# Yubo-Shankui/Bind-Your-Avatar-Implementation

Measured on AMD Instinct MI355X. Metric: denoise-steps/sec, higher is better.
Workload: dtype bf16; 1 GPU; BASELINE.json configs[1]: full transformer.forward, 49x480x720 (13x30x45 latent tokens + 226 text), 2 characters (2 ID + 2 audio), batch 1, random-init 8.6B-param architecture; layers=42, batch=1, launch=eager, parallelism=single GPU

## Files before the change

### bind_your_avatar_implementation_amd/_hip.py

```python
import ctypes
import os

from .build import LIB_PATH as _BUILT_LIB

LIB_PATH = os.environ.get("BYA_HIP_LIB") or _BUILT_LIB

_c = ctypes
_vp, _i32, _i64, _f32 = _c.c_void_p, _c.c_int32, _c.c_int64, _c.c_float


class GemmDesc(_c.Structure):
    _fields_ = [("M", _i32), ("N", _i32), ("K", _i32), ("batch", _i32),
                ("lda", _i32), ("ldw", _i32), ("ldc", _i32), ("ldres", _i32),
                ("a_batch_stride", _i64), ("c_batch_stride", _i64), ("res_batch_stride", _i64),
                ("gate_batch_stride", _i64), ("gate_split", _i32), ("act", _i32),
                ("n_split", _i32), ("c_split_stride", _i64), ("bias_rowscale", _vp), ("alpha", _f32)]


class GemmPlan(_c.Structure):
    _fields_ = [("path", _i32), ("m0", _i32), ("tail", _i32), ("split_k", _i32), ("row_chunks", _i32)]


class QkNormDesc(_c.Structure):
    _fields_ = [("qw", _vp), ("qb", _vp), ("kw", _vp), ("kb", _vp), ("cos", _vp), ("sin", _vp),
                ("text_rows", _i32), ("width", _i32), ("eps", _f32), ("k_scale", _f32)]


class MxGemmCall(_c.Structure):
    _fields_ = [("A", _vp), ("a_scales", _vp), ("W", _vp), ("w_scales", _vp), ("bias", _vp), ("C", _vp),
                ("res", _vp), ("gate0", _vp), ("gate1", _vp), ("q_scales", _vp), ("norm", _c.POINTER(QkNormDesc)),
                ("a_fmt", _i32), ("w_fmt", _i32), ("out_fmt", _i32), ("kernel", _i32)]


class AttnDesc(_c.Structure):
    _fields_ = [("head_dim", _i32), ("heads", _i32), ("nb1", _i32), ("nb2", _i32), ("Sq", _i32), ("Skv", _i32),
                ("q_s1", _i64), ("q_s2", _i64), ("q_row", _i64),
                ("k_s1", _i64), ("k_s2", _i64), ("k_row", _i64),
                ("v_s1", _i64), ("v_s2", _i64), ("v_row", _i64),
                ("o_s1", _i64), ("o_s2", _i64), ("o_row", _i64),
                ("scale", _f32), ("scores_prescaled", _i32), ("score_bound", _f32),
                ("bound_dev", _vp), ("bound_slots", _i32), ("bound_heads", _i32), ("bound_bh0", _i32), ("fallback_flags", _vp)]


class AttnMixDesc(_c.Structure):
    _fields_ = [("head_dim", _i32), ("heads", _i32), ("n_id", _i32), ("n_grp", _i32), ("Sq", _i32), ("Skv", _i32),
                ("q_grp", _i64), ("q_row", _i64), ("k_id", _i64), ("k_grp", _i64), ("k_row", _i64),
                ("v_id", _i64), ("v_grp", _i64), ("v_row", _i64), ("z_grp", _i64), ("z_row", _i64), ("scale", _f32)]


class AttnPlan(_c.Structure):
    _fields_ = [("variant", _i32), ("grid", _i32), ("q_tile", _i32), ("stream_k", _i32), ("sk_rem", _i32), ("sk_cut", _i32),
                ("o_wide", _i32), ("second_launch", _i32)]


class AttnMixPlan(_c.Structure):
    _fields_ = [("form", _i32), ("head_dim", _i32), ("grid", _i32), ("row_chunks", _i32), ("lds_bytes", _i32), ("big_lds", _i32)]


class AttnTinyPlan(_c.Structure):
    _fields_ = [("instance", _i32), ("grid", _i32), ("waves", _i64)]


class RowGemmPlan(_c.Structure):
    _fields_ = [("form", _i32), ("ln", _i32), ("res", _i32), ("act", _i32), ("grid", _i32), ("crosses_row_block", _i32),
                ("work_items", _i64)]


class GroupAttnPlan(_c.Structure):
    _fields_ = [("P", _i32), ("G", _i32), ("wide", _i32), ("blocks", _i32), ("tiles", _i64)]


class LayerNormPlan(_c.Structure):
    _fields_ = [("kernel", _i32), ("vec", _i32), ("nv", _i32), ("modulated", _i32), ("rows_per_wave", _i32), ("grid", _i32),
                ("waves", _i64)]


class QkNormRopePlan(_c.Structure):
    _fields_ = [("stats", _i32), ("only", _i32), ("grid", _i32), ("slots", _i32), ("pairs", _i64), ("waves", _i64)]


class RouterChainPlan(_c.Structure):
    _fields_ = [("tiles", _i32), ("tp0", _i32), ("grid", _i32), ("passes", _i32), ("tiles_last", _i32), ("wgs_last", _i32)]


class SchedCoef(_c.Structure):
    _fields_ = [("guidance", _f32), ("sqrt_alpha", _f32), ("sqrt_beta", _f32), ("k_sample", _f32),
                ("k_denoised", _f32), ("k_noise", _f32), ("k_cur", _f32), ("k_old", _f32)]


SIGNATURES = {
    "bya_abi_version": [],
    "bya_set_option": [_i32, _i32],
    "bya_get_option": [_i32, _c.POINTER(_i32)],
    "bya_mfma_calibration": [_vp, _i64, _vp, _i32, _vp],
    "bya_gemm_bf16": [_vp, _vp, _vp, _vp, _vp, _vp, _vp, _c.POINTER(GemmDesc), _vp],
    "bya_gemm_skinny_bf16": [_vp, _vp, _vp, _vp, _vp, _c.POINTER(GemmDesc), _vp],
    "bya_gemm_qkv_norm_rope": [_vp, _vp, _vp, _vp, _c.POINTER(GemmDesc), _c.POINTER(QkNormDesc), _vp],
    "bya_gemm_bf16_plan": [_vp, _vp, _vp, _vp, _vp, _vp, _vp, _c.POINTER(GemmDesc), _c.POINTER(GemmPlan)],
    "bya_gemm_qkv_norm_rope_plan": [_vp, _vp, _vp, _vp, _c.POINTER(GemmDesc), _c.POINTER(QkNormDesc), _c.POINTER(GemmPlan)],
    "bya_set_gemm_workspace": [_vp, _i64],
    "bya_gemm_workspace_bytes": [_c.POINTER(_i64)],
    "bya_gemm_workspace_status": [_c.POINTER(_i32), _vp],
    "bya_quantize_rows_fp8": [_vp, _vp, _vp, _i32, _i32, _i64, _i64, _vp],
    "bya_gemm_fp8": [_vp, _vp, _vp, _vp, _vp, _vp, _vp, _vp, _vp, _c.POINTER(GemmDesc), _vp],
    "bya_gemm_fp8_plan": [_vp, _vp, _vp, _vp, _vp, _vp, _vp, _vp, _vp, _c.POINTER(GemmDesc), _c.POINTER(GemmPlan)],
    "bya_layernorm_fp8": [_vp, _vp, _vp, _vp, _vp, _vp, _vp, _vp, _vp, _i64, _i32, _i32, _i64, _i64, _i64, _i64, _i64, _i64,
                          _f32, _vp],
    "bya_quantize_mx": [_vp, _vp, _vp, _i32, _i32, _i64, _i32, _vp],
    "bya_layernorm_mx": [_vp, _vp, _vp, _vp, _vp, _vp, _vp, _vp, _vp, _i64, _i32, _i32, _i64, _i64, _i64, _i64, _i64, _i64,
                         _f32, _i32, _vp],
    "bya_gemm_mx": [_vp, _vp, _vp, _vp, _vp, _vp, _vp, _vp, _vp, _c.POINTER(GemmDesc), _i32, _vp],
    "bya_gemm_mx_plan": [_vp, _vp, _vp, _vp, _vp, _vp, _vp, _vp, _vp, _c.POINTER(GemmDesc), _i32, _c.POINTER(GemmPlan)],
    "bya_gemm_mx_mixed": [_vp, _vp, _vp, _vp, _vp, _vp, _vp, _vp, _vp, _c.POINTER(GemmDesc), _i32, _i32, _vp],
    "bya_gemm_mx_mixed_plan": [_vp, _vp, _vp, _vp, _vp, _vp, _vp, _vp, _vp, _c.POINTER(GemmDesc), _i32, _i32,
                               _c.POINTER(GemmPlan)],
    "bya_gemm_mx_quant": [_vp, _vp, _vp, _vp, _vp, _vp, _vp, _c.POINTER(GemmDesc), _i32, _i32, _i32, _vp],
    "bya_gemm_mx_quant_plan": [_vp, _vp, _vp, _vp, _vp, _vp, _vp, _c.POINTER(GemmDesc), _i32, _i32, _i32,
                               _c.POINTER(GemmPlan)],
    "bya_gemm_mx_qkv_norm_rope": [_vp, _vp, _vp, _vp, _vp, _vp, _i32, _i32, _c.POINTER(GemmDesc), _c.POINTER(QkNormDesc), _vp],
    "bya_gemm_mx_qkv_norm_rope_plan": [_vp, _vp, _vp, _vp, _vp, _vp, _i32, _i32, _c.POINTER(GemmDesc), _c.POINTER(QkNormDesc),
                                       _c.POINTER(GemmPlan)],
    "bya_gemm_mx_qkv_norm_rope_on": [_vp, _vp, _vp, _vp, _vp, _vp, _i32, _i32, _c.POINTER(GemmDesc), _c.POINTER(QkNormDesc), _i32,
                                     _vp],
    "bya_gemm_mx_qkv_norm_rope_on_plan": [_vp, _vp, _vp, _vp, _vp, _vp, _i32, _i32, _c.POINTER(GemmDesc), _c.POINTER(QkNormDesc),
                                          _i32, _c.POINTER(GemmPlan)],
    "bya_gemm_mx_call": [_c.POINTER(MxGemmCall), _c.POINTER(GemmDesc), _vp],
    "bya_gemm_mx_call_plan": [_c.POINTER(MxGemmCall), _c.POINTER(GemmDesc), _c.POINTER(GemmPlan)],
    "bya_linear_small_m": [_vp, _vp, _vp, _vp, _i32, _i32, _i32, _i32, _i32, _vp],
    "bya_timestep_features": [_vp, _vp, _i32, _i32, _i32, _f32, _vp],
    "bya_layernorm": [_vp, _vp, _vp, _vp, _vp, _vp, _vp, _vp, _i64, _i32, _i32, _i64, _i64, _i64, _i64, _i64, _i64,
                      _f32, _vp],
    "bya_layernorm_plan": [_vp, _vp, _vp, _vp, _vp, _vp, _vp, _vp, _i64, _i32, _i32, _i64, _i64, _i64, _i64, _i64, _i64,
                           _i32, _c.POINTER(LayerNormPlan)],
    "bya_qknorm_rope_plan": [_vp, _vp, _vp, _vp, _vp, _vp, _vp, _vp, _i32, _i32, _i32, _i64, _i64, _i32, _vp, _i32,
                             _c.POINTER(QkNormRopePlan)],
    "bya_qknorm_rope": [_vp, _vp, _vp, _vp, _vp, _vp, _vp, _vp, _i32, _i32, _i32, _i64, _i64, _i32, _f32, _f32, _vp, _i32, _vp],
    "bya_attn_fwd": [_vp, _vp, _vp, _vp, _c.POINTER(AttnDesc), _vp],
    "bya_attn_variant": [_c.POINTER(AttnDesc)],
    "bya_attn_plan": [_c.POINTER(AttnDesc), _vp, _i32, _c.POINTER(AttnPlan)],
    "bya_attn_fwd_mx": [_vp, _vp, _vp, _vp, _vp, _c.POINTER(AttnDesc), _i32, _i64, _i64, _i64, _i64, _i64, _i64, _vp],
    "bya_attn_mx_plan": [_c.POINTER(AttnDesc), _vp, _vp, _i32, _i64, _i64, _i64, _i64, _i64, _i64, _i32, _c.POINTER(AttnPlan)],
    "bya_set_attn_workspace": [_vp, _i64],
    "bya_attn_workspace_bytes": [_c.POINTER(_i64)],
    "bya_attn_workspace_status": [_c.POINTER(_i32), _vp],
    "bya_attn_kv_mix": [_vp, _vp, _vp, _vp, _vp, _vp, _vp, _c.POINTER(AttnMixDesc), _vp],
    "bya_attn_kv_mix_plan": [_vp, _vp, _c.POINTER(AttnMixDesc), _c.POINTER(AttnMixPlan)],
    "bya_attn_tiny": [_vp, _vp, _vp, _vp, _i32, _i32, _i64, _i64, _i64, _i64, _i64, _i64, _f32, _vp],
    "bya_attn_tiny_plan": [_vp, _vp, _vp, _vp, _i32, _i32, _i64, _i64, _i64, _i64, _c.POINTER(AttnTinyPlan)],
    "bya_router_scores": [_vp, _vp, _vp, _vp, _vp, _vp, _i32, _i64, _i32, _i32, _f32, _vp],
    "bya_router_head": [_vp, _vp, _vp, _vp, _i32, _i64, _i32, _vp],
    "bya_forcing_max_over_frames": [_vp, _vp, _i32, _i64, _i32, _vp],
    "bya_masked_combine": [_vp, _vp, _vp, _vp, _i32, _f32, _i32, _i32, _i64, _i32, _i64, _i64, _i64, _vp],
    "bya_routed_mix": [_vp, _vp, _vp, _vp, _vp, _i32, _i32, _i32, _i64, _i32, _i64, _vp],
    "bya_patchify": [_vp, _vp, _i32, _i32, _i32, _i32, _i32, _vp],
    "bya_unpatchify": [_vp, _vp, _i32, _i32, _i32, _i32, _i32, _vp],
    "bya_act_add": [_vp, _vp, _vp, _i64, _i32, _vp],
    "bya_rowgemm512": [_vp, _vp, _vp, _vp, _vp, _vp, _i32, _i32, _i32, _i32, _i32, _i32, _f32, _i32, _i32, _vp],
    "bya_rowgemm512_plan": [_vp, _vp, _vp, _vp, _vp, _vp, _i32, _i32, _i32, _i32, _i32, _i32, _i32, _c.POINTER(RowGemmPlan)],
    "bya_router_group_attn_plan": [_vp, _vp, _vp, _vp, _vp, _i32, _i32, _i32, _i32, _i64, _i64, _i64, _i64,
                                   _c.POINTER(GroupAttnPlan)],
    "bya_router_mlp_fused_plan": [_vp, _vp, _vp, _vp, _vp, _vp, _vp, _i32, _i32, _i32, _i32, _c.POINTER(RouterChainPlan)],
    "bya_router_group_attn_out_plan": [_vp, _vp, _vp, _vp, _vp, _vp, _vp, _i32, _i32, _i32, _i32, _i64, _i64, _i64, _i64, _i32,
                                       _c.POINTER(RouterChainPlan)],
    "bya_router_group_attn": [_vp, _vp, _vp, _vp, _vp, _i32, _i32, _i32, _i32, _i64, _i64, _i64, _i64, _f32, _f32, _vp],
    "bya_router_mlp_fused": [_vp, _vp, _vp, _vp, _vp, _vp, _vp, _i32, _i32, _i32, _f32, _i32, _vp],
    "bya_router_group_attn_out": [_vp, _vp, _vp, _vp, _vp, _vp, _vp, _i32, _i32, _i32, _i32, _i64, _i64, _i64, _i64, _f32, _f32,
                                  _i32, _vp],
    "bya_masks_to_routing_logits": [_vp, _vp, _i32, _i32, _i32, _i32, _i32, _i32, _i32, _vp],
    "bya_vae_patches": [_vp, _vp, _vp] + [_i32] * 14 + [_vp],
    "bya_vae_groupnorm_stats": [_vp, _vp, _vp, _i64, _i32, _i32, _vp],
    "bya_vae_norm_act": [_vp, _vp, _vp, _vp, _vp, _vp, _vp, _i64, _i32, _i32, _i32, _f32, _i32, _i32, _i32, _i32, _i32, _i32,
                         _i32, _i64, _i32, _vp],
    "bya_vae_conv3d": [_vp, _vp, _vp, _vp, _vp, _i32, _i32, _i32, _i32, _i32, _i32, _i64, _i64, _i64, _vp],
    "bya_vae_upsample_pad": [_vp, _vp, _i32, _i32, _i32, _i32, _i32, _vp],
    "bya_allgather_kv": [_vp, _vp, _vp, _vp, _i64, _i64, _vp, _vp],
    "bya_alltoall_router": [_vp, _vp, _vp, _vp, _i32, _vp, _vp],
    "bya_p2p_push": [_vp, _i32, _i64, _vp, _i32, _i32, _vp, _vp],
    "bya_p2p_wait": [_vp, _i32, _vp, _i64, _vp],
    "bya_p2p_exchange": [_vp, _i32, _i64, _vp, _i32, _i32, _vp, _vp, _i64, _vp],
    "bya_p2p_poison": [_vp, _i32, _vp, _i64, _vp],
    "bya_p2p_alloc": [_i64, _i32, _c.POINTER(_vp)],
    "bya_p2p_free": [_vp],
    "bya_p2p_ipc_export": [_vp, _vp],
    "bya_p2p_ipc_import": [_vp, _c.POINTER(_vp)],
    "bya_p2p_ipc_release": [_vp],
    "bya_cfg_scheduler_step": [_vp, _i32, _i64, _vp, _vp, _vp, _vp, _vp, _i64, _c.POINTER(SchedCoef), _vp],
}

OPTIONS = {"gemm_splitk": 0, "gemm_splitk_min": 1, "gemm_tile": 2, "gemm_variant": 3, "attn_streamk": 4, "fp8_kernel": 5,
           "p2p_groups": 6, "reference_forms": 7, "mx_kernel": 8}
REFERENCE_FORMS = {"rowgemm_chunked": 1, "kv_mix_generic": 2, "ln_generic": 4, "router_scores_wave": 8, "attn_narrow_store": 16}
def _named_value(var, v, table):
    if v not in table:
        raise ValueError(f"{var}={v!r}: expected one of {sorted(table)}")
    return table[v]


ENV_OPTIONS = {
    "BYA_GEMM_SPLITK": ("gemm_splitk", int),
    "BYA_GEMM_SPLITK_MIN": ("gemm_splitk_min", int),
    "BYA_GEMM_TILE": ("gemm_tile", int),
    "BYA_GEMM_VARIANT": ("gemm_variant", lambda v: {"w8": 1, "no128": 2}.get(v, 0)),
    "BYA_ATTN_STREAMK": ("attn_streamk", int),
    "BYA_FP8_KERNEL": ("fp8_kernel", lambda v: 1 if v.startswith("1") else 0),
    "BYA_P2P_GROUPS": ("p2p_groups", int),
    "BYA_MX_KERNEL": ("mx_kernel", lambda v: _named_value("BYA_MX_KERNEL", v, {"0": 0, "1": 1, "p256": 1, "2": 2, "always": 2})),
}

GEMM_PATHS = {0: "t128x64", 1: "t128x128", 2: "t256x128", 3: "t256x256", 4: "p256", 5: "p128", 6: "p128s", 7: "w8_256"}

ATTN_VARIANTS = {0: "d64_running_max", 1: "d64_prescaled_running_max", 2: "d64_static_bound", 3: "d128_running_max",
                 4: "d64_static_bound_w4", 5: "d64_device_bound_w4"}
KV_MIX_FORMS = {0: "mix32", 1: "one_tile"}
TINY_INSTANCES = {0: "tiny8<2>", 1: "tiny8<3>", 2: "tiny8<13>", 3: "tiny8<25>", 4: "generic<2>", 5: "generic<4>",
                  6: "generic<16>", 7: "generic<32>"}

ROWGEMM_FORMS = {0: "chunk_balanced", 1: "w_stationary"}

LN_KERNELS = {0: "generic", 1: "rows"}
LN_OUT_KINDS = {"bf16": 0, "fp8": 1, "mxfp8": 2, "mxfp6": 3}

ERRORS = {-1: "BYA_ERR_SHAPE", -2: "BYA_ERR_ALIGN", -3: "BYA_ERR_LAUNCH", -4: "BYA_ERR_UNSUPPORTED"}

_lib = None


def load():
    global _lib
    if _lib is not None:
        return _lib
    import torch
    if not os.path.exists(LIB_PATH):
        raise RuntimeError(
            f"{LIB_PATH} is missing: the Bind-Your-Avatar MI355X engine has no fallback path. "
            "Build it with `python -m bind_your_avatar_implementation_amd.build`.")
    lib = ctypes.CDLL(LIB_PATH)
    for name, argtypes in SIGNATURES.items():
        fn = getattr(lib, name)
        fn.argtypes = argtypes
        fn.restype = _i32
    _lib = lib
    apply_env_options()
    return lib


def set_option(name, value):
    check(load().bya_set_option(OPTIONS[name], int(value)), f"bya_set_option({name}={value})")


def get_option(name):
    v = _i32(0)
    check(load().bya_get_option(OPTIONS[name], _c.byref(v)), f"bya_get_option({name})")
    return v.value


OPTION_DEFAULTS = {"gemm_splitk": 0, "gemm_splitk_min": 0, "gemm_tile": -1, "gemm_variant": 0, "attn_streamk": 1, "fp8_kernel": 0,
                   "p2p_groups": 0, "reference_forms": 0, "mx_kernel": 0}


def apply_env_options():
    for var, (name, parse) in ENV_OPTIONS.items():
        v = os.environ.get(var)
        set_option(name, parse(v) if v not in (None, "") else OPTION_DEFAULTS[name])


class ByaError(RuntimeError):
    pass


def check(rc, what):
    if rc != 0:
        raise ByaError(f"{what} failed: {ERRORS.get(rc, rc)}")
```

### bind_your_avatar_implementation_amd/csrc/gemm.hip

```cpp
#include "gemm_common.h"
#include <stdlib.h>
#include <string.h>
#include "options.h"

namespace {


template <int ROWS, int NWAVES>
__device__ __forceinline__ void stage_tile(const bf16_t* __restrict__ src, int ld, int row0, int row_max, int k0,
                                           char* lds_tile, int wave, int lane) {
    constexpr int PER_WAVE = ROWS / NWAVES;
#pragma unroll
    for (int q = 0; q < PER_WAVE / 8; ++q) {
        const int rbase = wave * PER_WAVE + q * 8;
        const int rl = rbase + (lane >> 3);
        const int chunk = (lane & 7) ^ ((rl >> 1) & 7);
        int gr = row0 + rl;
        gr = gr < row_max ? gr : row_max;
        const bf16_t* g = src + (long long)gr * ld + k0 + chunk * 8;
        __builtin_amdgcn_global_load_lds(GLOBAL_PTR(g), LDS_PTR(lds_tile + rbase * 128), 16, 0, 0);
    }
}

__device__ __forceinline__ bf16x8 lds_frag(const char* tile, int row, int chunk) {
// ... 79 lines not shown
    ds_read128<(HALF * 64 + 48) * 128>(f.v[3], addr);
}
template <int HALF>
__device__ __forceinline__ void load_frag_b(FragB& f, uint32_t addr) {
    ds_read128<(HALF * 32 + 0) * 128>(f.v[0], addr);
    ds_read128<(HALF * 32 + 16) * 128>(f.v[1], addr);
}
template <int N>
__device__ __forceinline__ void wait_frags(FragA& a, FragB& b) {
    asm volatile("s_waitcnt lgkmcnt(%6)"
                 : "+v"(a.v[0]), "+v"(a.v[1]), "+v"(a.v[2]), "+v"(a.v[3]), "+v"(b.v[0]), "+v"(b.v[1])
                 : "i"(N));
}

template <int HA, int HB>
__device__ __forceinline__ void mfma_quadrant(f32x4 (&acc)[4][8], const FragA& a, const FragB& b) {
    __builtin_amdgcn_s_setprio(1);
#pragma unroll
    for (int ni = 0; ni < 2; ++ni)
#pragma unroll
        for (int mi = 0; mi < 4; ++mi)
            acc[HB * 2 + ni][HA * 4 + mi] =
                __builtin_amdgcn_mfma_f32_16x16x32_bf16(b.v[ni], a.v[mi], acc[HB * 2 + ni][HA * 4 + mi], 0, 0, 0);
    __builtin_amdgcn_s_setprio(0);
}

__global__ __launch_bounds__(512, 2) void gemm256_kernel(GemmArgs p) {
    extern __shared__ __attribute__((aligned(16))) char smem[];
    constexpr int BM = 256, BN = 256, STAGE = (BM + BN) * BK * 2, TILE_A = BM * BK * 2;
    const int tid = threadIdx.x, lane = tid & 63;
    const int wave = __builtin_amdgcn_readfirstlane(tid >> 6);
    const int tiles_m = (p.M + BM - 1) / BM, tiles_n = (p.N + BN - 1) / BN;
    const int nwg = tiles_m * tiles_n;
    const int id = xcd_remap(blockIdx.x, nwg);
    constexpr int GM = 4;
    const int per_group = GM * tiles_n;
    const int group = id / per_group, first_m = group * GM;
    const int gsz = (tiles_m - first_m) < GM ? (tiles_m - first_m) : GM;
    const int in_g = id - group * per_group;
    const int tm = first_m + in_g % gsz, tn = in_g / gsz;
    const int m0 = tm * BM, n0 = tn * BN;
    const int z = blockIdx.z;
    const bf16_t* A = p.A + (long long)z * p.a_bs;
    const int nk = p.K / BK;
    const int wm = wave >> 2, wn = wave & 3;
    const int fr = lane & 15, fq = lane >> 4;

    const int a_row = wm * 128 + fr, w_row = wn * 64 + fr;
    const int a_sw = (a_row >> 1) & 7, w_sw = (w_row >> 1) & 7;
    const int a_off0 = ((fq ^ a_sw) << 4), a_off1 = (((4 + fq) ^ a_sw) << 4);
    const int w_off0 = ((fq ^ w_sw) << 4), w_off1 = (((4 + fq) ^ w_sw) << 4);
    const int a_lane = a_row * 128, w_lane = w_row * 128;

    const __amdgpu_buffer_rsrc_t rsA = __builtin_amdgcn_make_buffer_rsrc(
        (void*)A, 0, (int)(((long long)(p.M - 1) * p.lda + p.K) * 2), 0x00020000);
    const __amdgpu_buffer_rsrc_t rsW = __builtin_amdgcn_make_buffer_rsrc(
        (void*)p.W, 0, (int)(((long long)(p.N - 1) * p.ldw + p.K) * 2), 0x00020000);
    uint32_t voff[8];
#pragma unroll
    for (int q = 0; q < 8; ++q) {
        const int rl = wave * 32 + (q & 3) * 8 + (lane >> 3);
        const int chunk = (lane & 7) ^ ((rl >> 1) & 7);
        voff[q] = (q < 4) ? (uint32_t)(m0 + rl) * (uint32_t)(p.lda * 2) + chunk * 16
                          : (uint32_t)(n0 + rl) * (uint32_t)(p.ldw * 2) + chunk * 16;
    }
    auto piece = [&](int t, int q) {
        char* dst = smem + (t & 1) * STAGE + (q >= 4 ? TILE_A : 0) + (wave * 32 + (q & 3) * 8) * 128;
        __builtin_amdgcn_raw_ptr_buffer_load_lds(q >= 4 ? rsW : rsA, LDS_PTR(dst), 16, voff[q], t * (BK * 2), 0, 0);
    };

    f32x4 acc[4][8];
#pragma unroll
    for (int i = 0; i < 4; ++i)
#pragma unroll
        for (int j = 0; j < 8; ++j) acc[i][j] = f32x4{0.f, 0.f, 0.f, 0.f};

    piece(0, 0); piece(0, 1); piece(0, 2); piece(0, 3); piece(0, 4); piece(0, 5); piece(0, 6); piece(0, 7);
    if (nk > 1) { piece(1, 0); piece(1, 1); }
    asm volatile("s_waitcnt vmcnt(0)" ::: "memory");
    __builtin_amdgcn_s_barrier();

    const uint32_t lds0 = (uint32_t)(uintptr_t)LDS_PTR(smem);
    uint32_t cA0 = lds0 + a_lane + a_off0, cA1 = lds0 + a_lane + a_off1;
    uint32_t cW0 = lds0 + TILE_A + w_lane + w_off0, cW1 = lds0 + TILE_A + w_lane + w_off1;
    static_assert(STAGE == 65536, "stage flip uses one address bit");
    FragA a0, a1;
    FragB bx, by;
    load_frag_a<0>(a0, cA0);
    load_frag_b<0>(bx, cW0);

    for (int t = 0; t < nk; ++t) {
        const bool more = t + 1 < nk;
        load_frag_b<1>(by, cW0);
        if (more) { piece(t + 1, 2); piece(t + 1, 3); }
        __builtin_amdgcn_sched_barrier(0);
        wait_frags<2>(a0, bx);
        mfma_quadrant<0, 0>(acc, a0, bx);
        __builtin_amdgcn_sched_barrier(0);
        load_frag_a<1>(a1, cA0);
        if (more) { piece(t + 1, 4); piece(t + 1, 5); }
        __builtin_amdgcn_sched_barrier(0);
        wait_frags<4>(a0, by);
        mfma_quadrant<0, 1>(acc, a0, by);
        __builtin_amdgcn_sched_barrier(0);
        load_frag_a<0>(a0, cA1);
        if (more) { piece(t + 1, 6); piece(t + 1, 7); }
        __builtin_amdgcn_sched_barrier(0);
        wait_frags<4>(a1, by);
        mfma_quadrant<1, 1>(acc, a1, by);
        __builtin_amdgcn_sched_barrier(0);
        load_frag_b<0>(by, cW1);
        __builtin_amdgcn_sched_barrier(0);
        mfma_quadrant<1, 0>(acc, a1, bx);
        __builtin_amdgcn_sched_barrier(0);
        load_frag_b<1>(bx, cW1);
        __builtin_amdgcn_sched_barrier(0);
        wait_frags<2>(a0, by);
        mfma_quadrant<0, 0>(acc, a0, by);
        __builtin_amdgcn_sched_barrier(0);
        load_frag_a<1>(a1, cA1);
        __builtin_amdgcn_sched_barrier(0);
        wait_frags<4>(a0, bx);
        mfma_quadrant<0, 1>(acc, a0, bx);
        __builtin_amdgcn_sched_barrier(0);
        wait_frags<0>(a1, bx);
        mfma_quadrant<1, 1>(acc, a1, bx);
        __builtin_amdgcn_sched_barrier(0);
        asm volatile("s_waitcnt vmcnt(0)" ::: "memory");
        __builtin_amdgcn_s_barrier();
        cA0 ^= STAGE; cA1 ^= STAGE; cW0 ^= STAGE; cW1 ^= STAGE;
        if (more) {
            load_frag_a<0>(a0, cA0);
            load_frag_b<0>(bx, cW0);
            if (t + 2 < nk) { piece(t + 2, 0); piece(t + 2, 1); }
        }
        __builtin_amdgcn_sched_barrier(0);
        mfma_quadrant<1, 0>(acc, a1, by);
        __builtin_amdgcn_sched_barrier(0);
    }
    asm volatile("s_waitcnt lgkmcnt(0)" ::: "memory");

    auto run = [&](auto act_tag) {
        epilogue_block<decltype(act_tag)::value, 4, 8, 2>(p, z, m0 + wm * 128 + fr, n0 + wn * 64 + fq * 4, acc);
    };
    dispatch_act_big(p.act, run);
}

inline bool v4_eligible(const GemmArgs& a) {
    return a.K >= 3 * BK && a.N % 8 == 0 && a.n_split % 8 == 0 && a.ldc % 8 == 0 && (!a.res || a.ldres % 8 == 0) &&
        !(((uintptr_t)a.C | (uintptr_t)a.res | (uintptr_t)a.bias | (uintptr_t)a.gate0 | (uintptr_t)a.gate1) & 15) &&
        a.c_bs % 8 == 0 && a.res_bs % 8 == 0 && a.gate_bs % 8 == 0 && a.c_split_stride % 8 == 0;
}

inline bool p128_eligible(const GemmArgs& a) { return v4_eligible(a) && a.K >= 4 * BK && a.conv_cpg_log2 < 0 && bya_opt(BYA_OPT_GEMM_VARIANT) == 0; }

inline int path256(const GemmArgs& a) {
    return v4_eligible(a) && bya_opt(BYA_OPT_GEMM_VARIANT) != 1 ? BYA_GEMM_PATH_P256 : BYA_GEMM_PATH_W8_256;
}

int launch_w8_256(const GemmArgs& a, int batch, hipStream_t s) {
    const int tiles_m = (a.M + 255) / 256, tiles_n = (a.N + 255) / 256;
    dim3 grid(tiles_m * tiles_n, 1, batch);
    const size_t lds = 2 * 512 * BK * 2;
    static std::atomic<unsigned long long> attr_done{0};
    if (bya_allow_big_lds(reinterpret_cast<const void*>(gemm256_kernel), (int)lds, attr_done) != BYA_OK) return BYA_ERR_LAUNCH;
    BYA_LAUNCH(gemm256_kernel, grid, dim3(512), lds, s, a);
    return hipGetLastError() == hipSuccess ? BYA_OK : BYA_ERR_LAUNCH;
}

template <int BM, int BN, int WAVES_M, int WAVES_N>
int launch(const GemmArgs& a, int batch, hipStream_t s) {
    const int tiles_m = (a.M + BM - 1) / BM, tiles_n = (a.N + BN - 1) / BN;
    dim3 grid(tiles_m * tiles_n, 1, batch);
    const size_t lds = 2 * (BM + BN) * BK * 2;
    static std::atomic<unsigned long long> attr_done{0};
    if (bya_allow_big_lds(reinterpret_cast<const void*>(gemm_bf16_kernel<BM, BN, WAVES_M, WAVES_N>), (int)lds, attr_done) != BYA_OK)
        return BYA_ERR_LAUNCH;
    BYA_LAUNCH((gemm_bf16_kernel<BM, BN, WAVES_M, WAVES_N>), grid, dim3(64 * WAVES_M * WAVES_N), lds, s, a);
    return hipGetLastError() == hipSuccess ? BYA_OK : BYA_ERR_LAUNCH;
}

constexpr double REL_128S = 0.85, REL_128P = 0.80;
inline double rounds_128(int M, int N, int batch, double rel) {
    const long long t = (long long)((M + 127) / 128) * ((N + 255) / 256) * batch;
    return 0.5 * (double)((t + 255) / 256) / rel;
}
inline double rounds_256_split(int M, int N, int K, int batch) {
    const long long tiles = (long long)((M + 255) / 256) * ((N + 255) / 256) * batch, full = tiles / 256, rem = tiles % 256;
    if (rem == 0) return (double)full;
    const int R = (int)((rem + 7) / 8);
    int parts = 32 / R;
    const int by_k = (K / BK) / bya_gemm_split_min_ktiles();
    if (parts > by_k) parts = by_k;
    return (double)full + (parts > 1 ? 1.0 / parts + 0.3 : 1.0);
}
inline int hybrid_rows(int M, int N, int batch, double rel, double* cost) {
    const long long tn = (N + 255) / 256, tiles = (long long)((M + 255) / 256) * tn, full = tiles / 256;
    if (batch != 1 || full < 1 || tiles % 256 == 0) return 0;
    const int main_tm = (int)(full * 256 / tn), m0 = main_tm * 256;
    if (m0 <= 0 || m0 >= M) return 0;
    *cost = (double)(((long long)main_tm * tn + 255) / 256) + rounds_128(M - m0, N, 1, rel) + 0.05;
    return m0;
}
inline int plan_rows_qkn(int M, int N, int batch, int* m0) {
    const int forced = bya_opt(BYA_OPT_GEMM_TILE);
    if (forced >= 0) return forced == 5 || forced == 6 ? 1 : 0;
    const long long t256 = (long long)((M + 255) / 256) * ((N + 255) / 256) * batch;
    const double r256 = (double)((t256 + 255) / 256), r128 = rounds_128(M, N, batch, REL_128P);
    double best = r256, hc = 0.0;
    int plan = 0;
    if (r128 < 0.97 * best) { best = r128; plan = 1; }
    const int hm = hybrid_rows(M, N, batch, REL_128P, &hc);
    if (hm > 0 && hc < (plan == 0 ? r256 - 0.15 : 0.97 * best)) { *m0 = hm; plan = 2; }
    return plan;
}

inline int pick_tile(int M, int N, int K, int batch, int forced, int act, bool splitk, bool p128_ok) {
    if (forced >= 0) return (forced >= 4 && !act_on_big_tiles(act)) ? 1 : forced;
    if (N <= 64) return 0;
    auto rounds = [&](int bm, int bn, int per_cu) {
        const long long blocks = (long long)((M + bm - 1) / bm) * ((N + bn - 1) / bn) * batch;
        const long long slots = 256LL * per_cu;
        return (double)((blocks + slots - 1) / slots) * (bm * bn) * (double)per_cu;
    };
    const double t128 = rounds(128, 128, 2) / 0.80;
    const double t256x128 = rounds(256, 128, 1) / 0.95;
    const double frac_rounds = (double)((M + 255) / 256) * ((N + 255) / 256) * batch / 256.0;
    const double t256 = splitk ? (frac_rounds + 0.12) * 65536.0 : rounds(256, 256, 1) / 1.00;
    (void)t256x128;
#ifdef BYA_GEMM_NO_DEEP_GRID
    const bool deep_grid = false;
#else
    const bool deep_grid = frac_rounds >= 4.0 && M >= 512 && K >= 512;
#endif
    if (((M < 1024 || K < 1024) && !deep_grid) || N < 512 || !act_on_big_tiles(act)) return 1;
    if (p128_ok) {
        const double t256s = (splitk ? rounds_256_split(M, N, K, batch) * 65536.0 : t256) / 1.2;
        const double best = t256s <= t128 ? t256s : t128, r128 = rounds_128(M, N, batch, REL_128S);
        if (r128 * 65536.0 / 1.2 < 0.97 * best) {
            double hc = 0.0;
            if (!splitk && hybrid_rows(M, N, batch, REL_128S, &hc) > 0 && hc < 0.97 * r128 && t256 / 1.2 <= t128) return 4;
            return 6;
        }
    }
    return (t256 / 1.2 <= t128) ? 4 : 1;
}

}

namespace {
constexpr int MAX_DEVICES = 64;
std::atomic<void*> g_gemm_ws[MAX_DEVICES];
inline int current_device() {
    int dev = 0;
    return hipGetDevice(&dev) == hipSuccess && dev >= 0 && dev < MAX_DEVICES ? dev : -1;
}
}

extern "C" int bya_set_gemm_workspace(void* ws, int64_t bytes) {
    if (ws && (bytes < (int64_t)GEMM_WS_BYTES || ((uintptr_t)ws & 255))) return BYA_ERR_SHAPE;
    const int dev = current_device();
    if (dev < 0) return BYA_ERR_UNSUPPORTED;
    g_gemm_ws[dev].store(ws);
    return BYA_OK;
}

extern "C" int bya_gemm_workspace_status(int32_t* timeouts, hipStream_t stream) {
    if (!timeouts) return BYA_ERR_SHAPE;
    *timeouts = 0;
    const int dev = current_device();
    char* const ws = dev < 0 ? nullptr : static_cast<char*>(g_gemm_ws[dev].load());
    if (!ws) return BYA_OK;
    unsigned word = 0;
    if (hipMemcpyAsync(&word, ws + 1023 * 4, 4, hipMemcpyDeviceToHost, stream) != hipSuccess) return BYA_ERR_LAUNCH;
    if (hipStreamSynchronize(stream) != hipSuccess) return BYA_ERR_LAUNCH;
    *timeouts = (int32_t)word;
    return BYA_OK;
}

extern "C" int bya_gemm_workspace_bytes(int64_t* bytes) {
    if (!bytes) return BYA_ERR_SHAPE;
    *bytes = (int64_t)GEMM_WS_BYTES;
    return BYA_OK;
}

namespace {
int dispatch_gemm(const GemmArgs& a, int nbatch, hipStream_t stream);
void plan_gemm(const GemmArgs& a, int nbatch, bya_gemm_plan* p);

int bf16_args(const void* A, const void* W, const void* bias, const void* C, const void* res, const void* gate0,
              const void* gate1, const bya_gemm_desc* d, GemmArgs* out) {
    if (!A || !W || !C || !d) return BYA_ERR_SHAPE;
    if (d->M <= 0 || d->N <= 0 || d->K <= 0 || d->batch <= 0) return BYA_ERR_SHAPE;
    if (d->K % BK != 0 || d->N % 4 != 0) return BYA_ERR_SHAPE;
    if (d->lda % 8 || d->ldw % 8 || d->ldc % 4 || (res && d->ldres % 4)) return BYA_ERR_ALIGN;
    if (((uintptr_t)A | (uintptr_t)W) & 15) return BYA_ERR_ALIGN;
    if (((uintptr_t)C | (uintptr_t)res | (uintptr_t)bias | (uintptr_t)gate0 | (uintptr_t)gate1) & 7) return BYA_ERR_ALIGN;
    if (d->act < 0 || d->act > 6) return BYA_ERR_UNSUPPORTED;
    GemmArgs& a = *out;
    a.A = (const bf16_t*)A; a.W = (const bf16_t*)W; a.bias = (const bf16_t*)bias; a.C = (bf16_t*)C;
    a.res = (const bf16_t*)res; a.gate0 = (const bf16_t*)gate0; a.gate1 = (const bf16_t*)(gate1 ? gate1 : gate0);
    a.M = d->M; a.N = d->N; a.K = d->K;
    a.lda = d->lda; a.ldw = d->ldw; a.ldc = d->ldc; a.ldres = d->ldres;
    a.a_bs = d->a_batch_stride; a.c_bs = d->c_batch_stride; a.res_bs = d->res_batch_stride;
    a.gate_bs = d->gate_batch_stride; a.gate_split = d->gate_split; a.act = d->act; a.leaky = 0.01f;
    a.n_split = d->n_split; a.c_split_stride = d->c_split_stride;
    a.bias_rowscale = d->bias_rowscale; a.alpha = d->alpha == 0.0f ? 1.0f : d->alpha;
    const int dev = current_device();
    char* const ws = dev < 0 ? nullptr : static_cast<char*>(g_gemm_ws[dev].load());
    a.ws_counters = reinterpret_cast<unsigned*>(ws);
    a.ws_slabs = ws ? reinterpret_cast<float*>(ws + GEMM_WS_COUNTER_BYTES) : nullptr;
    if (d->n_split < 0 || (d->n_split > 0 && (d->n_split % 4 || d->c_split_stride % 4 || res))) return BYA_ERR_SHAPE;
    return BYA_OK;
}

int qkn_args(const void* A, const void* W, const void* bias, const void* C, const bya_gemm_desc* d, const bya_qknorm_desc* n,
             GemmArgs* out) {
    if (!A || !W || !C || !d || !n) return BYA_ERR_SHAPE;
    if (d->M <= 0 || d->N <= 0 || d->K <= 0 || d->batch <= 0 || d->K % BK != 0) return BYA_ERR_SHAPE;
    if (!n->qw || !n->qb || !n->kw || !n->kb || n->width <= 0 || n->text_rows < 0) return BYA_ERR_SHAPE;
    if (n->text_rows < d->M && (!n->cos || !n->sin)) return BYA_ERR_SHAPE;
    if ((d->N != 3 * n->width && d->N != 2 * n->width) || n->width % 128 != 0 || d->n_split <= 0 || d->act != 0 || d->bias_rowscale || (d->alpha != 0.0f && d->alpha != 1.0f))
        return BYA_ERR_UNSUPPORTED;
    if (d->lda % 8 || d->ldw % 8) return BYA_ERR_ALIGN;
    if (((uintptr_t)A | (uintptr_t)W | (uintptr_t)C | (uintptr_t)bias | (uintptr_t)n->qw | (uintptr_t)n->qb | (uintptr_t)n->kw |
         (uintptr_t)n->kb | (uintptr_t)n->cos | (uintptr_t)n->sin) & 15) return BYA_ERR_ALIGN;
    GemmArgs& a = *out;
    a.A = (const bf16_t*)A; a.W = (const bf16_t*)W; a.bias = (const bf16_t*)bias; a.C = (bf16_t*)C;
    a.res = nullptr; a.gate0 = nullptr; a.gate1 = nullptr;
    a.M = d->M; a.N = d->N; a.K = d->K;
    a.lda = d->lda; a.ldw = d->ldw; a.ldc = d->ldc; a.ldres = 0;
    a.a_bs = d->a_batch_stride; a.c_bs = d->c_batch_stride; a.res_bs = 0; a.gate_bs = 0; a.gate_split = 0; a.act = 0; a.leaky = 0.01f;
    a.n_split = d->n_split; a.c_split_stride = d->c_split_stride;
    a.bias_rowscale = nullptr; a.alpha = 1.0f;
    a.ws_counters = nullptr; a.ws_slabs = nullptr;
    a.qkn_w[0] = (const bf16_t*)n->qw; a.qkn_b[0] = (const bf16_t*)n->qb; a.qkn_w[1] = (const bf16_t*)n->kw; a.qkn_b[1] = (const bf16_t*)n->kb;
    a.qkn_cos = n->cos; a.qkn_sin = n->sin; a.qkn_text_rows = n->text_rows; a.qkn_width = n->width;
    a.qkn_eps = n->eps; a.qkn_kscale = n->k_scale == 0.0f ? 1.0f : n->k_scale;
    if (!v4_eligible(a) || !gemm_rows_reachable(a, a.M)) return BYA_ERR_UNSUPPORTED;
    return BYA_OK;
}

inline int qkn_plan(const GemmArgs& a, int batch, int* m0) {
    *m0 = 0;
    return p128_eligible(a) ? plan_rows_qkn(a.M, a.N, batch, m0) : 0;
}
}

extern "C" int bya_gemm_bf16(const void* A, const void* W, const void* bias, void* C, const void* res,
                             const void* gate0, const void* gate1, const bya_gemm_desc* d, hipStream_t stream) {
    GemmArgs a;
    const int rc = bf16_args(A, W, bias, C, res, gate0, gate1, d, &a);
    if (rc != BYA_OK) return rc;
    return gemm_row_chunks(a, d->batch, 2, [&](const GemmArgs& piece, int batch, long long) {
        return dispatch_gemm(piece, batch, stream);
    });
}

extern "C" int bya_gemm_bf16_plan(const void* A, const void* W, const void* bias, const void* C, const void* res,
                                  const void* gate0, const void* gate1, const bya_gemm_desc* d, bya_gemm_plan* plan) {
    if (!plan) return BYA_ERR_SHAPE;
    GemmArgs a, piece;
    int rc = bf16_args(A, W, bias, C, res, gate0, gate1, d, &a), nb = 0;
    if (rc != BYA_OK) return rc;
    const int chunks = gemm_first_chunk(a, d->batch, &piece, &nb);
    if (!chunks) return BYA_ERR_UNSUPPORTED;
    plan_gemm(piece, nb, plan);
    plan->row_chunks = chunks;
    return BYA_OK;
}

extern "C" int bya_gemm_qkv_norm_rope(const void* A, const void* W, const void* bias, void* C, const bya_gemm_desc* d,
                                      const bya_qknorm_desc* n, hipStream_t stream) {
    GemmArgs a;
    const int rc0 = qkn_args(A, W, bias, C, d, n, &a);
    if (rc0 != BYA_OK) return rc0;
    int m0 = 0;
    const int plan = qkn_plan(a, d->batch, &m0);
    if (plan == 1) return bya_launch_gemm128p_qkn(&a, d->batch, stream);
    if (plan == 2) {
        GemmArgs lo = a, hi = a;
        lo.M = m0;
        hi.M = a.M - m0;
        hi.A += (long long)m0 * a.lda;
        hi.C += (long long)m0 * a.ldc;
        hi.qkn_text_rows = a.qkn_text_rows > m0 ? a.qkn_text_rows - m0 : 0;
        if (a.qkn_cos && m0 > a.qkn_text_rows) {
            hi.qkn_cos = a.qkn_cos + (long long)(m0 - a.qkn_text_rows) * 64;
            hi.qkn_sin = a.qkn_sin + (long long)(m0 - a.qkn_text_rows) * 64;
        }
        const int rc = bya_launch_gemm256p_qkn(&lo, 1, stream);
        return rc != BYA_OK ? rc : bya_launch_gemm128p_qkn(&hi, 1, stream);
    }
    return bya_launch_gemm256p_qkn(&a, d->batch, stream);
}

extern "C" int bya_gemm_qkv_norm_rope_plan(const void* A, const void* W, const void* bias, const void* C, const bya_gemm_desc* d,
                                           const bya_qknorm_desc* n, bya_gemm_plan* p) {
    if (!p) return BYA_ERR_SHAPE;
    GemmArgs a;
    const int rc = qkn_args(A, W, bias, C, d, n, &a);
    if (rc != BYA_OK) return rc;
    int m0 = 0;
    const int plan = qkn_plan(a, d->batch, &m0);
    p->path = plan == 1 ? BYA_GEMM_PATH_P128 : BYA_GEMM_PATH_P256;
    p->m0 = plan == 2 ? m0 : 0;
    p->tail = plan == 2 ? BYA_GEMM_PATH_P128 : -1;
    p->split_k = 0;
    p->row_chunks = 1;
    return BYA_OK;
}

namespace {
template <int MT>
__global__ __launch_bounds__(1024) void gemm_skinny_kernel(GemmArgs p) {
    extern __shared__ __attribute__((aligned(16))) char smem[];
    float* red = reinterpret_cast<float*>(smem);
    const int tid = threadIdx.x, lane = tid & 63, c = lane & 15, g = lane >> 4;
    const int wave = __builtin_amdgcn_readfirstlane(tid >> 6);
    const int n0 = blockIdx.x * 16, zb = blockIdx.y, fold = p.gate_split, rows = fold > 0 ? fold * p.M : p.M;
    const int ksteps = p.K / 32;
    const int k_lo = (int)((long long)ksteps * wave / 16), k_hi = (int)((long long)ksteps * (wave + 1) / 16);
    const bf16_t* wrow = p.W + (long long)(n0 + c) * p.ldw + 8 * g;
    const bf16_t* xrow[MT];
#pragma unroll
    for (int mt = 0; mt < MT; ++mt) {
        int r = mt * 16 + c;
        r = r < rows ? r : rows - 1;
        const int z = fold > 0 ? r / p.M : zb, m = fold > 0 ? r % p.M : r;
        xrow[mt] = p.A + (long long)z * p.a_bs + (long long)m * p.lda + 8 * g;
    }
    f32x4 acc[MT];
#pragma unroll
    for (int mt = 0; mt < MT; ++mt) acc[mt] = f32x4{0.f, 0.f, 0.f, 0.f};
    int ks = k_lo;
    for (; ks + 4 <= k_hi; ks += 4) {
        bf16x8 wf[4];
#pragma unroll
        for (int u = 0; u < 4; ++u) wf[u] = *reinterpret_cast<const bf16x8*>(wrow + (ks + u) * 32);
#pragma unroll
        for (int u = 0; u < 4; ++u)
#pragma unroll
            for (int mt = 0; mt < MT; ++mt) {
                const bf16x8 xf = *reinterpret_cast<const bf16x8*>(xrow[mt] + (ks + u) * 32);
                acc[mt] = __builtin_amdgcn_mfma_f32_16x16x32_bf16(wf[u], xf, acc[mt], 0, 0, 0);
            }
    }
    for (; ks < k_hi; ++ks) {
        const bf16x8 wf = *reinterpret_cast<const bf16x8*>(wrow + ks * 32);
#pragma unroll
        for (int mt = 0; mt < MT; ++mt) {
            const bf16x8 xf = *reinterpret_cast<const bf16x8*>(xrow[mt] + ks * 32);
            acc[mt] = __builtin_amdgcn_mfma_f32_16x16x32_bf16(wf, xf, acc[mt], 0, 0, 0);
        }
    }
#pragma unroll
    for (int mt = 0; mt < MT; ++mt)
        *reinterpret_cast<f32x4*>(red + ((wave * MT * 16 + mt * 16 + c) * 16 + 4 * g)) = acc[mt];
    __syncthreads();
    for (int t = tid; t < MT * 256; t += 1024) {
        const int r = t >> 4, n = t & 15;
        float v = 0.f;
#pragma unroll
        for (int w = 0; w < 16; ++w) v += red[(w * MT * 16 + r) * 16 + n];
        if (r < rows) {
            const int z = fold > 0 ? r / p.M : zb, m = fold > 0 ? r % p.M : r;
            if (p.bias) v += bf2f(p.bias[n0 + n]);
            switch (p.act) {
                case 1: v = gelu_tanh(v); break;
                case 2: v = gelu_erf(v); break;
                case 3: v = v > 0.f ? v : 0.f; break;
                case 4: v = silu(v); break;
                case 5: v = v > 0.f ? v : v * p.leaky; break;
                case 6: v = gelu_tanh_ieee(v); break;
                default: break;
            }
            v *= p.alpha;
            if (p.res) v += bf2f(p.res[(long long)z * p.res_bs + (long long)m * p.ldres + n0 + n]);
            p.C[(long long)z * p.c_bs + (long long)m * p.ldc + n0 + n] = f2bf(v);
        }
    }
}

inline bool skinny_eligible(const GemmArgs& a) {
    return a.M <= 64 && a.N <= 8192 && a.K >= 256 && a.K % 32 == 0 && a.N % 16 == 0 && a.lda % 8 == 0 && a.ldw % 8 == 0 && a.a_bs % 8 == 0 &&
        !a.gate0 && !a.bias_rowscale && a.n_split == 0 && a.conv_cpg_log2 < 0 && !(((uintptr_t)a.A | (uintptr_t)a.W) & 15);
}

template <int MT>
int launch_skinny_mt(const GemmArgs& a, dim3 grid, hipStream_t stream) {
    const size_t lds = (size_t)16 * MT * 16 * 16 * 4;
    static std::atomic<unsigned long long> big{0};
    if (lds > 64 * 1024 && bya_allow_big_lds(reinterpret_cast<const void*>(gemm_skinny_kernel<MT>), 160 * 1024, big) != BYA_OK)
        return BYA_ERR_LAUNCH;
    BYA_LAUNCH(gemm_skinny_kernel<MT>, grid, dim3(1024), lds, stream, a);
    return hipGetLastError() == hipSuccess ? BYA_OK : BYA_ERR_LAUNCH;
}

int launch_skinny(const GemmArgs& a0, int nbatch, hipStream_t stream) {
    GemmArgs a = a0;
    const bool fold = nbatch > 1 && (long long)nbatch * a.M <= 64;
    a.gate_split = fold ? nbatch : 0;
    const int rows = fold ? nbatch * a.M : a.M, mt = (rows + 15) / 16;
    const dim3 grid((unsigned)(a.N / 16), (unsigned)(fold ? 1 : nbatch));
    switch (mt) {
        case 1: return launch_skinny_mt<1>(a, grid, stream);
        case 2: return launch_skinny_mt<2>(a, grid, stream);
        case 3: return launch_skinny_mt<3>(a, grid, stream);
        case 4: return launch_skinny_mt<4>(a, grid, stream);
        case 5: return launch_skinny_mt<5>(a, grid, stream);
        case 6: return launch_skinny_mt<6>(a, grid, stream);
        case 7: return launch_skinny_mt<7>(a, grid, stream);
        default: return launch_skinny_mt<8>(a, grid, stream);
    }
}

void plan_gemm(const GemmArgs& a, int nbatch, bya_gemm_plan* p) {
    p->path = -1; p->m0 = 0; p->tail = -1; p->split_k = 0; p->row_chunks = 1;
    const bool ws = a.ws_counters != nullptr;
    const int forced = bya_opt(BYA_OPT_GEMM_TILE);
    const bool splitk = ws && bya_opt(BYA_OPT_GEMM_SPLITK) != 0 && a.K / BK >= 2 * bya_gemm_split_min_ktiles() && v4_eligible(a) &&
        bya_opt(BYA_OPT_GEMM_VARIANT) != 1;
    const int tile = pick_tile(a.M, a.N, a.K, nbatch, forced, a.act, splitk, p128_eligible(a));
    if (tile >= 0 && tile <= 3) { p->path = tile; return; }
    if ((tile == 5 || tile == 6) && p128_eligible(a)) { p->path = tile; return; }
    p->path = path256(a);
    const int tn = (a.N + 255) / 256, tm = (a.M + 255) / 256;
    const long long tiles = (long long)tm * tn;
    const long long full = tiles / 256;
    if (!splitk && nbatch == 1 && full >= 1 && tiles % 256 != 0) {
        const int main_tm = (int)(full * 256 / tn);
        const int m0 = main_tm * 256;
        if (m0 > 0 && m0 < a.M) {
            const long long tail_blocks = (long long)((a.M - m0 + 127) / 128) * ((a.N + 127) / 128);
            double tail_cost = 0.9 * (double)((tail_blocks + 511) / 512);
#ifdef BYA_GEMM_NO_P128_TAIL
            const bool tail_128p = false;
#else
            const bool tail_128p = p128_eligible(a) && act_on_big_tiles(a.act) && rounds_128(a.M - m0, a.N, 1, REL_128S) + 0.05 < tail_cost;
#endif
            if (tail_128p) tail_cost = rounds_128(a.M - m0, a.N, 1, REL_128S) + 0.05;
            const double main_cost = (double)(((long long)main_tm * tn + 255) / 256);
            if (main_cost + tail_cost < (double)((tiles + 255) / 256) - 0.15) {
                p->m0 = m0;
                p->tail = tail_128p ? BYA_GEMM_PATH_P128S : BYA_GEMM_PATH_T128X128;
                return;
            }
        }
    }
    if (p->path == BYA_GEMM_PATH_P256) p->split_k = bya_gemm256p_split(&a, nbatch);
}

int launch_path(int path, const GemmArgs& a, int batch, hipStream_t stream) {
    switch (path) {
        case BYA_GEMM_PATH_T128X64: return launch<128, 64, 2, 2>(a, batch, stream);
        case BYA_GEMM_PATH_T128X128: return launch<128, 128, 2, 2>(a, batch, stream);
        case BYA_GEMM_PATH_T256X128: return launch<256, 128, 4, 2>(a, batch, stream);
        case BYA_GEMM_PATH_T256X256: return launch<256, 256, 2, 4>(a, batch, stream);
        case BYA_GEMM_PATH_P256: return bya_launch_gemm256p(&a, batch, stream);
        case BYA_GEMM_PATH_P128: return bya_launch_gemm128p(&a, batch, stream);
        case BYA_GEMM_PATH_P128S: return bya_launch_gemm128s(&a, batch, stream);
        case BYA_GEMM_PATH_W8_256: return launch_w8_256(a, batch, stream);
        default: return BYA_ERR_UNSUPPORTED;
    }
}

int dispatch_gemm(const GemmArgs& a, int nbatch, hipStream_t stream) {
    bya_gemm_plan p;
    plan_gemm(a, nbatch, &p);
    if (p.m0 > 0) {
        GemmArgs lo = a, hi = a;
        lo.M = p.m0;
        hi.M = a.M - p.m0;
        hi.A += (long long)p.m0 * a.lda;
        hi.C += (long long)p.m0 * a.ldc;
        if (hi.res) hi.res += (long long)p.m0 * a.ldres;
        if (hi.bias_rowscale) hi.bias_rowscale += p.m0;
        hi.gate_split = a.gate_split > p.m0 ? a.gate_split - p.m0 : 0;
        const int rc = launch_path(p.path, lo, 1, stream);
        return rc != BYA_OK ? rc : launch_path(p.tail, hi, 1, stream);
    }
    return launch_path(p.path, a, nbatch, stream);
}
}


extern "C" int bya_gemm_skinny_bf16(const void* A, const void* W, const void* bias, void* C, const void* res,
                                    const bya_gemm_desc* d, hipStream_t stream) {
    if (!A || !W || !C || !d) return BYA_ERR_SHAPE;
    if (d->M <= 0 || d->N <= 0 || d->K <= 0 || d->batch <= 0) return BYA_ERR_SHAPE;
    if (d->act < 0 || d->act > 6) return BYA_ERR_UNSUPPORTED;
    GemmArgs a;
    a.A = (const bf16_t*)A; a.W = (const bf16_t*)W; a.bias = (const bf16_t*)bias; a.C = (bf16_t*)C;
    a.res = (const bf16_t*)res; a.gate0 = nullptr; a.gate1 = nullptr;
    a.M = d->M; a.N = d->N; a.K = d->K;
    a.lda = d->lda; a.ldw = d->ldw; a.ldc = d->ldc; a.ldres = d->ldres;
    a.a_bs = d->a_batch_stride; a.c_bs = d->c_batch_stride; a.res_bs = d->res_batch_stride;
    a.gate_bs = 0; a.gate_split = 0; a.act = d->act; a.leaky = 0.01f;
    a.n_split = d->n_split; a.c_split_stride = d->c_split_stride;
    a.bias_rowscale = d->bias_rowscale; a.alpha = d->alpha == 0.0f ? 1.0f : d->alpha;
    a.ws_counters = nullptr; a.ws_slabs = nullptr;
    if (!skinny_eligible(a)) return BYA_ERR_UNSUPPORTED;
    return launch_skinny(a, d->batch, stream);
}
```

### bind_your_avatar_implementation_amd/csrc/gemm_common.h

```cpp
#pragma once
#include "bya_common.h"
#include "../../include/bya.h"

namespace {

struct GemmArgs {
    const bf16_t* A; const bf16_t* W; const bf16_t* bias; bf16_t* C; const bf16_t* res;
    const bf16_t* gate0; const bf16_t* gate1;
    int M, N, K;
    int lda, ldw, ldc, ldres;
    long long a_bs, c_bs, res_bs, gate_bs;
    int gate_split;
    int act;
    float leaky;
    int n_split;
    long long c_split_stride;
    const float* bias_rowscale;
    float alpha;
    float* ws_slabs;
    unsigned* ws_counters;
    int gm = 4;
    const bf16_t* qkn_w[2] = {nullptr, nullptr};
    const bf16_t* qkn_b[2] = {nullptr, nullptr};
    const float* qkn_cos = nullptr; const float* qkn_sin = nullptr;
// ... 39 lines not shown
        case 1: f(IntTag<1>{}); break;
        case 2: f(IntTag<2>{}); break;
        case 3: f(IntTag<3>{}); break;
        case 4: f(IntTag<4>{}); break;
        case 5: f(IntTag<5>{}); break;
        case 6: f(IntTag<6>{}); break;
        default: f(IntTag<0>{}); break;
    }
}

template <int ACT, int NI, int NJ, int IB = NI>
__device__ __forceinline__ void epilogue_block(const GemmArgs& p, int z, int m_base, int n_base, const f32x4 (&acc)[NI][NJ]) {
    static_assert(NI % IB == 0, "burst size must divide the tile");
    const bool has_res = p.res != nullptr, has_gate = p.gate0 != nullptr, has_bias = p.bias != nullptr;
    const bool has_rs = p.bias_rowscale != nullptr;
    const __amdgpu_buffer_rsrc_t rsR = __builtin_amdgcn_make_buffer_rsrc(
        (void*)((has_res ? p.res : p.C) + (long long)z * p.res_bs), 0, 0x7fffffff, 0x00020000);
    const __amdgpu_buffer_rsrc_t rsC = __builtin_amdgcn_make_buffer_rsrc(
        (void*)(p.C + (long long)z * p.c_bs), 0, 0x7fffffff, 0x00020000);
    const char* g0base = reinterpret_cast<const char*>(p.gate0 + (long long)z * p.gate_bs);
    const char* g1base = reinterpret_cast<const char*>(p.gate1 + (long long)z * p.gate_bs);
    float rs[NJ];
    bool mok[NJ];
    uint32_t roff[NJ], coff[NJ];
#pragma unroll
    for (int j = 0; j < NJ; ++j) {
        const int m = m_base + 16 * j;
        mok[j] = m < p.M;
        const uint32_t mc = mok[j] ? (uint32_t)m : 0u;
        rs[j] = has_rs ? p.bias_rowscale[(long long)z * p.M + mc] : 1.0f;
        roff[j] = mok[j] ? mc * (uint32_t)(p.ldres * 2) : 0xffffffffu;
        coff[j] = mok[j] ? mc * (uint32_t)(p.ldc * 2) : 0xffffffffu;
    }
#pragma unroll
    for (int ib = 0; ib < NI; ib += IB) {
        u32x2 bv[IB], g0[IB], g1[IB], rv[IB][NJ];
        bool nok[IB];
        uint32_t ncb[IB];
#pragma unroll
        for (int ii = 0; ii < IB; ++ii) {
            const int n4 = n_base + 16 * (ib + ii);
            nok[ii] = n4 < p.N;
            ncb[ii] = nok[ii] ? (uint32_t)n4 * 2u : 0u;
            bv[ii] = has_bias ? *reinterpret_cast<const u32x2*>(reinterpret_cast<const char*>(p.bias) + ncb[ii]) : u32x2{0u, 0u};
            if (has_gate) {
                g0[ii] = *reinterpret_cast<const u32x2*>(g0base + ncb[ii]);
                g1[ii] = *reinterpret_cast<const u32x2*>(g1base + ncb[ii]);
            }
            if (has_res) {
#pragma unroll
                for (int j = 0; j < NJ; ++j)
                    rv[ii][j] = __builtin_bit_cast(u32x2, __builtin_amdgcn_raw_buffer_load_b64(
                        rsR, mok[j] ? roff[j] + ncb[ii] : 0xffffffffu, 0, 0));
            }
        }
#pragma unroll
        for (int ii = 0; ii < IB; ++ii) {
            const int n4 = n_base + 16 * (ib + ii);
            uint32_t colb = (uint32_t)n4 * 2u;
            if (p.n_split > 0) colb = ((uint32_t)(n4 / p.n_split) * (uint32_t)p.c_split_stride + (uint32_t)(n4 % p.n_split)) * 2u;
            const float b4[4] = {bflo(bv[ii][0]), bfhi(bv[ii][0]), bflo(bv[ii][1]), bfhi(bv[ii][1])};
#pragma unroll
            for (int j = 0; j < NJ; ++j) {
                const int m = m_base + 16 * j;
                float v[4];
#pragma unroll
                for (int e = 0; e < 4; ++e)
                    v[e] = p.alpha * apply_act<ACT>(fmaf(rs[j], b4[e], acc[ib + ii][j][e]), p.leaky);
                if (has_gate) {
                    const u32x2 gv = m < p.gate_split ? g0[ii] : g1[ii];
                    v[0] *= bflo(gv[0]); v[1] *= bfhi(gv[0]); v[2] *= bflo(gv[1]); v[3] *= bfhi(gv[1]);
                }
                if (has_res) {
                    v[0] += bflo(rv[ii][j][0]); v[1] += bfhi(rv[ii][j][0]);
                    v[2] += bflo(rv[ii][j][1]); v[3] += bfhi(rv[ii][j][1]);
                }
                u32x2 o;
                o[0] = pack2bf(v[0], v[1]);
                o[1] = pack2bf(v[2], v[3]);
                __builtin_amdgcn_raw_buffer_store_b64(o, rsC, (mok[j] && nok[ii]) ? coff[j] + colb : 0xffffffffu, 0, 0);
            }
        }
    }
}

template <int OFF, typename T>
__device__ __forceinline__ void ds_read128(T& dst, uint32_t addr) {
    static_assert(sizeof(T) == 16, "one ds_read_b128");
    asm volatile("ds_read_b128 %0, %1 offset:%2" : "=v"(dst) : "v"(addr), "i"(OFF));
}

inline long long gemm_span_bytes(const GemmArgs& a, int M, bool res) {
    const long long ld = res ? a.ldres : a.ldc;
    const long long col = (!res && a.n_split > 0) ? (long long)(a.N / a.n_split - 1) * a.c_split_stride + a.n_split - 1
                                                  : (long long)a.N - 1;
    return ((long long)(M - 1) * ld + col) * 2 + 16;
}

inline bool gemm_rows_reachable(const GemmArgs& a, int M) {
    constexpr long long REACH = 0x7fffffffLL;
    return gemm_span_bytes(a, M, false) < REACH && (!a.res || gemm_span_bytes(a, M, true) < REACH);
}

inline int gemm_chunk_rows(const GemmArgs& a) {
    if (gemm_rows_reachable(a, a.M)) return a.M;
    int chunk = a.M;
    while (chunk > 256 && !gemm_rows_reachable(a, chunk)) chunk = ((chunk / 2 + 255) / 256) * 256;
    return gemm_rows_reachable(a, chunk) ? chunk : 0;
}

inline int gemm_first_chunk(const GemmArgs& a, int batch, GemmArgs* piece, int* piece_batch) {
    const int chunk = gemm_chunk_rows(a);
    *piece = a;
    *piece_batch = batch;
    if (chunk == a.M || chunk == 0) return chunk == 0 ? 0 : 1;
    piece->M = chunk;
    *piece_batch = 1;
    return batch * ((a.M + chunk - 1) / chunk);
}

template <typename F>
int gemm_row_chunks(const GemmArgs& a, int batch, int a_elem_bytes, F&& run) {
    const int chunk = gemm_chunk_rows(a);
    if (chunk == a.M) return run(a, batch, 0LL);
    if (chunk == 0) return BYA_ERR_UNSUPPORTED;
    for (int z = 0; z < batch; ++z)
        for (int m0 = 0; m0 < a.M; m0 += chunk) {
            GemmArgs s = a;
            s.M = a.M - m0 < chunk ? a.M - m0 : chunk;
            s.A = reinterpret_cast<const bf16_t*>(reinterpret_cast<const char*>(a.A) +
                                                  ((long long)z * a.a_bs + (long long)m0 * a.lda) * a_elem_bytes);
            s.C = a.C + (long long)z * a.c_bs + (long long)m0 * a.ldc;
            if (a.res) s.res = a.res + (long long)z * a.res_bs + (long long)m0 * a.ldres;
            if (a.gate0) s.gate0 = a.gate0 + (long long)z * a.gate_bs;
            if (a.gate1) s.gate1 = a.gate1 + (long long)z * a.gate_bs;
            if (a.bias_rowscale) s.bias_rowscale = a.bias_rowscale + (long long)z * a.M + m0;
            s.gate_split = a.gate_split > m0 ? a.gate_split - m0 : 0;
            const int rc = run(s, 1, (long long)z * a.M + m0);
            if (rc != BYA_OK) return rc;
        }
    return BYA_OK;
}
inline int gemm_group_m(const GemmArgs& a) { return a.K >= 8192 ? 2 : (a.N >= 8192 ? 8 : 4); }

}

int bya_launch_gemm256p(const void* args, int batch, hipStream_t stream);
int bya_launch_gemm256p_qkn(const void* args, int batch, hipStream_t stream);
int bya_gemm_split_min_ktiles();
int bya_gemm256p_split(const void* args, int batch);
int bya_launch_gemm128p(const void* args, int batch, hipStream_t stream);
int bya_launch_gemm128p_qkn(const void* args, int batch, hipStream_t stream);
int bya_launch_gemm128s(const void* args, int batch, hipStream_t stream);
```

### bind_your_avatar_implementation_amd/csrc/gemm_persistent.h

```cpp
#pragma once
#include "gemm_common.h"

namespace {

typedef int i32x4 __attribute__((ext_vector_type(4)));

struct XcdRange { int base, end; };
__host__ __device__ __forceinline__ XcdRange xcd_range(int total, int xcd) {
    const int cq = total >> 3, cr = total & 7;
    const int base = (xcd < cr) ? xcd * (cq + 1) : cr * (cq + 1) + (xcd - cr) * cq;
    return {base, base + cq + (xcd < cr ? 1 : 0)};
}

struct PersistentTile { int z, m0, n0; bool valid; };

template <int BM, int BN>
struct TileWalk {
    int tiles_m, tiles_n, per_z, gm;
    int base, end, slot, slots;
    __device__ __forceinline__ TileWalk(int tiles_m_, int tiles_n_, int batch, int gm_)
        : tiles_m(tiles_m_), tiles_n(tiles_n_), per_z(tiles_m_ * tiles_n_), gm(gm_) {
        const int total = per_z * batch, xcd = blockIdx.x & 7;
        slot = blockIdx.x >> 3;
        slots = gridDim.x >> 3;
        const XcdRange r = xcd_range(total, xcd);
        base = r.base;
        end = r.end;
    }
    __device__ __forceinline__ PersistentTile coord(int seq) const {
        PersistentTile c;
        const int id = base + slot + seq * slots;
        c.valid = id < end;
        const int idz = c.valid ? id : base;
        c.z = idz / per_z;
        const int idt = idz - c.z * per_z;
        const int per_group = gm * tiles_n;
        const int group = idt / per_group, first_m = group * gm;
        const int gsz = (tiles_m - first_m) < gm ? (tiles_m - first_m) : gm;
        const int in_g = idt - group * per_group;
        c.m0 = (first_m + in_g % gsz) * BM;
        c.n0 = (in_g / gsz) * BN;
        return c;
    }
};

__device__ __forceinline__ int w_slot_col(int s) {
    const int r = s & 15, i = (s >> 4) & 7;
    return (s & 128) + (((r & 3) << 2) | (r >> 2)) * 8 + i;
}
__device__ __forceinline__ uint32_t stage_off(int lane, int rl, int src_row, uint32_t pitch) {
    return (uint32_t)src_row * pitch + ((lane & 7) ^ ((rl >> 1) & 7)) * 16;
}

__device__ __forceinline__ uint32_t stage_off64(int lane, int rl, int src_row, uint32_t pitch) {
    return (uint32_t)src_row * pitch + ((lane & 3) ^ (((rl >> 2) & 1) << 1)) * 16;
}

__device__ __forceinline__ i32x4 raw_rsrc(const void* base, uint32_t bytes) {
    const unsigned long long b = (unsigned long long)base;
    i32x4 r;
    r.x = __builtin_amdgcn_readfirstlane((int)(b & 0xffffffffu));
    r.y = __builtin_amdgcn_readfirstlane((int)((b >> 32) & 0xffffu));
    r.z = __builtin_amdgcn_readfirstlane((int)bytes);
    r.w = 0x00020000;
    return r;
}

template <int LDS_OFF = 0>
__device__ __forceinline__ void dma_piece(uint32_t lds_base, uint32_t voff, const i32x4& rsrc, uint32_t soff) {
    asm volatile("s_mov_b32 m0, %0\n\ts_nop 0\n\tbuffer_load_dwordx4 %1, %2, %3 offen lds"
                 :
                 : "s"(lds_base + LDS_OFF), "v"(voff), "s"(rsrc), "s"(soff)
                 : "memory");
}

template <typename T>
__device__ __forceinline__ i32x4 tile_rsrc_a(const GemmArgs& p, const T* A, const PersistentTile& c) {
    const long long left = ((long long)(p.M - 1 - c.m0) * p.lda + p.K) * (long long)sizeof(T);
    return raw_rsrc(A + (long long)c.z * p.a_bs + (long long)c.m0 * p.lda, c.valid && left > 0 ? (uint32_t)left : 0u);
}
template <typename T>
__device__ __forceinline__ i32x4 tile_rsrc_w(const GemmArgs& p, const T* W, const PersistentTile& c, int row_elems = 0) {
    const long long left = ((long long)(p.N - 1 - c.n0) * p.ldw + (row_elems ? row_elems : p.K)) * (long long)sizeof(T);
    return raw_rsrc(W + (long long)c.n0 * p.ldw, c.valid && left > 0 ? (uint32_t)left : 0u);
}

__device__ __forceinline__ uint32_t frag_addr(uint32_t tile, int row, int chunk) {
    return tile + row * 128 + ((chunk ^ ((row >> 1) & 7)) << 4);
}

__device__ __forceinline__ uint32_t frag_addr64(uint32_t tile, int row, int chunk) {
    return tile + row * 64 + ((chunk ^ (((row >> 2) & 1) << 1)) << 4);
}

#define DMA_PIECE(Q, BASE, VO, RS, SOFF) dma_piece<(Q) * 1024>(BASE, VO[Q], RS, SOFF)
#define ALL4(M, ...) M(0, __VA_ARGS__); M(1, __VA_ARGS__); M(2, __VA_ARGS__); M(3, __VA_ARGS__)
#define ALL8(M, ...) ALL4(M, __VA_ARGS__); M(4, __VA_ARGS__); M(5, __VA_ARGS__); M(6, __VA_ARGS__); M(7, __VA_ARGS__)
#define KEEP4(F) asm volatile("" :: "v"(F[0]), "v"(F[1]), "v"(F[2]), "v"(F[3]))
#define KEEP8(F) asm volatile("" :: "v"(F[0]), "v"(F[1]), "v"(F[2]), "v"(F[3]), "v"(F[4]), "v"(F[5]), "v"(F[6]), "v"(F[7]))

inline int persistent_grid(long long total) { return (int)(total < 256 ? (total + 7) / 8 * 8 : 256); }

template <auto KERNEL, typename... Args>
int launch_persistent(int blocks, int threads, size_t lds, hipStream_t s, const Args&... args) {
    static std::atomic<unsigned long long> attr_done{0};
    if (bya_allow_big_lds(reinterpret_cast<const void*>(KERNEL), (int)lds, attr_done) != BYA_OK) return BYA_ERR_LAUNCH;
    BYA_LAUNCH(KERNEL, dim3(blocks), dim3(threads), lds, s, args...);
    return hipGetLastError() == hipSuccess ? BYA_OK : BYA_ERR_LAUNCH;
}

}
```

### bind_your_avatar_implementation_amd/csrc/gemm_v6.hip

```cpp
#include "gemm_wide_epilogue.h"
#include "options.h"

#ifndef BYA_GEMM6_ABLATE
#define BYA_GEMM6_ABLATE 0
#endif

namespace {

__global__ __launch_bounds__(512, 1) void gemm128s_kernel(GemmArgs p, int tiles_m, int tiles_n, int batch) {
    extern __shared__ __attribute__((aligned(16))) char smem[];
    constexpr int BM = 128, BN = 256, TILE_A = BM * BK * 2, STAGE = (BM + BN) * BK * 2;
    static_assert(TILE_A == 16384 && STAGE == 49152, "three stages fill 144 KiB");
    const int tid = threadIdx.x, lane = tid & 63;
    const int wave = __builtin_amdgcn_readfirstlane(tid >> 6);
    const int nk = p.K / BK;

    const TileWalk<BM, BN> walk(tiles_m, tiles_n, batch, p.gm);
    int seq = 0;
    PersistentTile cur = walk.coord(seq);
    if (!cur.valid) return;
    const uint32_t lds0 = (uint32_t)(uintptr_t)LDS_PTR(smem);

    if (wave >= 4) {
        const int lw = wave - 4;
        uint32_t voA[4], voW[8];
#pragma unroll
        for (int q = 0; q < 4; ++q) {
            const int rl = lw * 32 + q * 8 + (lane >> 3);
            voA[q] = stage_off(lane, rl, rl, (uint32_t)(p.lda * 2));
        }
#pragma unroll
        for (int q = 0; q < 8; ++q) {
            const int rl = lw * 64 + q * 8 + (lane >> 3);
            voW[q] = stage_off(lane, rl, w_slot_col(rl), (uint32_t)(p.ldw * 2));
        }
        uint32_t fillA = __builtin_amdgcn_readfirstlane(lds0 + lw * 32 * 128);
        uint32_t fillW = __builtin_amdgcn_readfirstlane(lds0 + TILE_A + lw * 64 * 128);
        int st = 0;
        i32x4 rsA = tile_rsrc_a(p, p.A, cur), rsW = tile_rsrc_w(p, p.W, cur);
#define DMA_A(Q, BASE, RS, SOFF) DMA_PIECE(Q, BASE, voA, RS, SOFF)
#define DMA_W(Q, BASE, RS, SOFF) DMA_PIECE(Q, BASE, voW, RS, SOFF)
        ALL4(DMA_A, fillA, rsA, 0u);
        ALL8(DMA_W, fillW, rsW, 0u);
        ALL4(DMA_A, fillA + STAGE, rsA, (uint32_t)(BK * 2));
        ALL8(DMA_W, fillW + STAGE, rsW, (uint32_t)(BK * 2));
        ALL4(DMA_A, fillA + 2 * STAGE, rsA, (uint32_t)(2 * BK * 2));
        ALL8(DMA_W, fillW + 2 * STAGE, rsW, (uint32_t)(2 * BK * 2));
        asm volatile("s_waitcnt vmcnt(24)\n\ts_barrier" ::: "memory");
        auto refill = [&](const i32x4& dA, const i32x4& dW, uint32_t soff) {
            asm volatile("s_waitcnt vmcnt(12)\n\ts_barrier" ::: "memory");
            if (!(BYA_GEMM6_ABLATE & 2)) {
                ALL4(DMA_A, fillA, dA, (BYA_GEMM6_ABLATE & 16) ? 0u : soff);
                ALL8(DMA_W, fillW, dW, (BYA_GEMM6_ABLATE & 16) ? 0u : soff);
            }
            const uint32_t d = st == 2 ? (uint32_t)(-2 * STAGE) : (uint32_t)STAGE;
            fillA += d;
            fillW += d;
            st = st == 2 ? 0 : st + 1;
        };
        for (;;) {
            const PersistentTile nxt = walk.coord(seq + 1);
            const i32x4 rsAn = tile_rsrc_a(p, p.A, nxt), rsWn = tile_rsrc_w(p, p.W, nxt);
            for (int t = 0; t + 3 < nk; ++t) refill(rsA, rsW, (uint32_t)((t + 3) * (BK * 2)));
            refill(rsAn, rsWn, 0u);
            refill(rsAn, rsWn, (uint32_t)(BK * 2));
            refill(rsAn, rsWn, (uint32_t)(2 * BK * 2));
            if (!nxt.valid) break;
            ++seq;
            rsA = rsAn;
            rsW = rsWn;
        }
#undef DMA_A
#undef DMA_W
        asm volatile("s_waitcnt vmcnt(0)" ::: "memory");
        return;
    }

    const int wm = wave >> 1, wn = wave & 1;
    const int fr = lane & 15, fq = lane >> 4;
    const int a_row = wm * 64 + fr, w_row = wn * 128 + fr;
    const uint32_t bA0 = frag_addr(lds0, a_row, fq), bA1 = frag_addr(lds0, a_row, 4 + fq);
    const uint32_t bW0 = frag_addr(lds0 + TILE_A, w_row, fq);
    const uint32_t bW1 = frag_addr(lds0 + TILE_A, w_row, 4 + fq);
    uint32_t off1 = 0u, off0 = (uint32_t)STAGE;
    uint32_t rA1 = bA1, rW1 = bW1, rA0 = bA0 + STAGE, rW0 = bW0 + STAGE;

    f32x4 acc[8][4];
    bf16x8 fa[2][4], fw[2][8];
    asm volatile("s_barrier" ::: "memory");

#define RA(S, J) ds_read128<(J) * 2048>(fa[S][J], (S) ? rA1 : rA0)
#define RW(S, I) ds_read128<(I) * 2048>(fw[S][I], (S) ? rW1 : rW0)
    for (;;) {
        const PersistentTile nxt = walk.coord(seq + 1);
        {
            const uint32_t tA = bA0 + off1, tW = bW0 + off1;
            ds_read128<0 * 2048>(fa[0][0], tA); ds_read128<1 * 2048>(fa[0][1], tA); ds_read128<2 * 2048>(fa[0][2], tA); ds_read128<3 * 2048>(fa[0][3], tA);
            ds_read128<0 * 2048>(fw[0][0], tW); ds_read128<1 * 2048>(fw[0][1], tW); ds_read128<2 * 2048>(fw[0][2], tW); ds_read128<3 * 2048>(fw[0][3], tW);
            ds_read128<4 * 2048>(fw[0][4], tW); ds_read128<5 * 2048>(fw[0][5], tW); ds_read128<6 * 2048>(fw[0][6], tW); ds_read128<7 * 2048>(fw[0][7], tW);
            asm volatile("s_waitcnt lgkmcnt(0)" ::: "memory");
        }
        auto ktile = [&](auto v_c) {
            constexpr char V = decltype(v_c)::value;
#define MF(S, I, J) \
            asm volatile("v_mfma_f32_16x16x32_bf16 %0, %1, %2, %0" : "+a"(acc[I][J]) : "v"(fw[S][I]), "v"(fa[S][J]))
#define MFZ(S, I, J) \
            asm volatile("v_mfma_f32_16x16x32_bf16 %0, %1, %2, 0" : "=a"(acc[I][J]) : "v"(fw[S][I]), "v"(fa[S][J]))
#define SYNC() asm volatile("s_waitcnt lgkmcnt(0)\n\ts_barrier" ::: "memory")
#define NEXT() do { \
                asm volatile("s_waitcnt lgkmcnt(0)" ::: "memory"); \
                off1 = off0; \
                off0 = off0 == (uint32_t)(2 * STAGE) ? 0u : off0 + (uint32_t)STAGE; \
                rA1 = bA1 + off1; rW1 = bW1 + off1; rA0 = bA0 + off0; rW0 = bW0 + off0; \
            } while (0)
        if constexpr (V == 'A') {
            MFZ(0, 0, 0);  RA(1, 0);
            MFZ(0, 0, 1);  RA(1, 1);
            MFZ(0, 0, 2);  RA(1, 2);
            MFZ(0, 0, 3);  RA(1, 3);
            MFZ(0, 1, 0);  RW(1, 0);
            MFZ(0, 1, 1);
            MFZ(0, 1, 2);  RW(1, 1);
            MFZ(0, 1, 3);
            MFZ(0, 2, 0);  RW(1, 2);
            MFZ(0, 2, 1);
            MFZ(0, 2, 2);  RW(1, 3);
            MFZ(0, 2, 3);
            MFZ(0, 3, 0);  RW(1, 4);
            MFZ(0, 3, 1);
            MFZ(0, 3, 2);  RW(1, 5);
            MFZ(0, 3, 3);
            MFZ(0, 4, 0);  RW(1, 6);
            MFZ(0, 4, 1);
            MFZ(0, 4, 2);  RW(1, 7);
            MFZ(0, 4, 3);
            MFZ(0, 5, 0);
            MFZ(0, 5, 1);
            MFZ(0, 5, 2);
            MFZ(0, 5, 3);
            MFZ(0, 6, 0);
            MFZ(0, 6, 1);
            MFZ(0, 6, 2);
            MFZ(0, 6, 3);  SYNC();
            MFZ(0, 7, 0);
            MFZ(0, 7, 1);  RW(0, 0);
            MFZ(0, 7, 2);
            MFZ(0, 7, 3);  RW(0, 1);
            MF(1, 0, 0);
            MF(1, 0, 1);  RW(0, 2);
            MF(1, 0, 2);
            MF(1, 0, 3);  RW(0, 3);
            MF(1, 1, 0);
            MF(1, 1, 1);  RW(0, 4);
            MF(1, 1, 2);
            MF(1, 1, 3);  RA(0, 0);
            MF(1, 2, 0);
            MF(1, 2, 1);  RA(0, 1);
            MF(1, 2, 2);
            MF(1, 2, 3);  RA(0, 2);
            MF(1, 3, 0);
            MF(1, 3, 1);  RA(0, 3);
            MF(1, 3, 2);
            MF(1, 3, 3);  RW(0, 5);
            MF(1, 4, 0);
            MF(1, 4, 1);  RW(0, 6);
            MF(1, 4, 2);
            MF(1, 4, 3);  RW(0, 7);
            MF(1, 5, 0);
            MF(1, 5, 1);
            MF(1, 5, 2);
            MF(1, 5, 3);
            MF(1, 6, 0);
            MF(1, 6, 1);
            MF(1, 6, 2);
            MF(1, 6, 3);
            MF(1, 7, 0);
            MF(1, 7, 1);
            MF(1, 7, 2);
            MF(1, 7, 3);  NEXT();
        } else if constexpr (V == 'B') {
            MF(0, 0, 0);  RA(1, 0);
            MF(0, 0, 1);  RA(1, 1);
            MF(0, 0, 2);  RA(1, 2);
            MF(0, 0, 3);  RA(1, 3);
            MF(0, 1, 0);  RW(1, 0);
            MF(0, 1, 1);
            MF(0, 1, 2);  RW(1, 1);
            MF(0, 1, 3);
            MF(0, 2, 0);  RW(1, 2);
            MF(0, 2, 1);
            MF(0, 2, 2);  RW(1, 3);
            MF(0, 2, 3);
            MF(0, 3, 0);  RW(1, 4);
            MF(0, 3, 1);
            MF(0, 3, 2);  RW(1, 5);
            MF(0, 3, 3);
            MF(0, 4, 0);  RW(1, 6);
            MF(0, 4, 1);
            MF(0, 4, 2);  RW(1, 7);
            MF(0, 4, 3);
            MF(0, 5, 0);
            MF(0, 5, 1);
            MF(0, 5, 2);
            MF(0, 5, 3);
            MF(0, 6, 0);
            MF(0, 6, 1);
            MF(0, 6, 2);
            MF(0, 6, 3);  SYNC();
            MF(0, 7, 0);
            MF(0, 7, 1);  RW(0, 0);
            MF(0, 7, 2);
            MF(0, 7, 3);  RW(0, 1);
            MF(1, 0, 0);
            MF(1, 0, 1);  RW(0, 2);
            MF(1, 0, 2);
            MF(1, 0, 3);  RW(0, 3);
            MF(1, 1, 0);
            MF(1, 1, 1);  RW(0, 4);
            MF(1, 1, 2);
            MF(1, 1, 3);  RA(0, 0);
            MF(1, 2, 0);
            MF(1, 2, 1);  RA(0, 1);
            MF(1, 2, 2);
            MF(1, 2, 3);  RA(0, 2);
            MF(1, 3, 0);
            MF(1, 3, 1);  RA(0, 3);
            MF(1, 3, 2);
            MF(1, 3, 3);  RW(0, 5);
            MF(1, 4, 0);
            MF(1, 4, 1);  RW(0, 6);
            MF(1, 4, 2);
            MF(1, 4, 3);  RW(0, 7);
            MF(1, 5, 0);
            MF(1, 5, 1);
            MF(1, 5, 2);
            MF(1, 5, 3);
            MF(1, 6, 0);
            MF(1, 6, 1);
            MF(1, 6, 2);
            MF(1, 6, 3);
            MF(1, 7, 0);
            MF(1, 7, 1);
            MF(1, 7, 2);
            MF(1, 7, 3);  NEXT();
        } else if constexpr (V == 'L') {
            MF(0, 0, 0);  RA(1, 0);
            MF(0, 0, 1);  RA(1, 1);
            MF(0, 0, 2);  RA(1, 2);
            MF(0, 0, 3);  RA(1, 3);
            MF(0, 1, 0);  RW(1, 0);
            MF(0, 1, 1);
            MF(0, 1, 2);  RW(1, 1);
            MF(0, 1, 3);
            MF(0, 2, 0);  RW(1, 2);
            MF(0, 2, 1);
            MF(0, 2, 2);  RW(1, 3);
            MF(0, 2, 3);
            MF(0, 3, 0);  RW(1, 4);
            MF(0, 3, 1);
            MF(0, 3, 2);  RW(1, 5);
            MF(0, 3, 3);
            MF(0, 4, 0);  RW(1, 6);
            MF(0, 4, 1);
            MF(0, 4, 2);  RW(1, 7);
            MF(0, 4, 3);
            MF(0, 5, 0);
            MF(0, 5, 1);
            MF(0, 5, 2);
            MF(0, 5, 3);
            MF(0, 6, 0);
            MF(0, 6, 1);
            MF(0, 6, 2);
            MF(0, 6, 3);  SYNC();
            MF(0, 7, 0);
            MF(0, 7, 1);
            MF(0, 7, 2);
            MF(0, 7, 3);
            MF(1, 0, 0);
            MF(1, 0, 1);
            MF(1, 0, 2);
            MF(1, 0, 3);
            MF(1, 1, 0);
            MF(1, 1, 1);
            MF(1, 1, 2);
            MF(1, 1, 3);
            MF(1, 2, 0);
            MF(1, 2, 1);
            MF(1, 2, 2);
            MF(1, 2, 3);
            MF(1, 3, 0);
            MF(1, 3, 1);
            MF(1, 3, 2);
            MF(1, 3, 3);
            MF(1, 4, 0);
            MF(1, 4, 1);
            MF(1, 4, 2);
            MF(1, 4, 3);
            MF(1, 5, 0);
            MF(1, 5, 1);
            MF(1, 5, 2);
            MF(1, 5, 3);
            MF(1, 6, 0);
            MF(1, 6, 1);
            MF(1, 6, 2);
            MF(1, 6, 3);
            MF(1, 7, 0);
            MF(1, 7, 1);
            MF(1, 7, 2);
            MF(1, 7, 3);  NEXT();
        }
            KEEP4(fa[0]); KEEP8(fw[0]); KEEP4(fa[1]); KEEP8(fw[1]);
#undef MF
#undef MFZ
#undef SYNC
#undef NEXT
        };
        ktile(IntTag<'A'>{});
        for (int t = 1; t + 1 < nk; ++t) ktile(IntTag<'B'>{});
        ktile(IntTag<'L'>{});
        asm volatile("s_nop 15\n\ts_nop 15" ::: "memory");

        if constexpr (BYA_GEMM6_ABLATE & 1) {
#pragma unroll
            for (int i = 0; i < 8; ++i) asm volatile("" :: "a"(acc[i][0]), "a"(acc[i][1]), "a"(acc[i][2]), "a"(acc[i][3]));
        } else {
            auto run = [&](auto act_tag) {
                epilogue_wide<decltype(act_tag)::value, 1, false, false, 4>(p, cur.z, cur.m0 + wm * 64, cur.n0 + wn * 128, fr, fq, acc, wave, lane);
            };
            dispatch_act_big(p.act, run);
        }

        if (!nxt.valid) break;
        ++seq;
        cur = nxt;
    }
#undef RA
#undef RW
}

}

int bya_launch_gemm128s(const void* args, int batch, hipStream_t s) {
    GemmArgs a = *static_cast<const GemmArgs*>(args);
#ifdef BYA_GEMM6_GM
    a.gm = BYA_GEMM6_GM;
#else
    a.gm = 2 * gemm_group_m(a);
#endif
    const int tiles_m = (a.M + 127) / 128, tiles_n = (a.N + 255) / 256;
    const size_t lds = 3 * (128 + 256) * BK * 2;
    return launch_persistent<gemm128s_kernel>(persistent_grid((long long)tiles_m * tiles_n * batch), 512, lds, s, a, tiles_m, tiles_n, batch);
}
```

### bind_your_avatar_implementation_amd/csrc/misc.hip

```cpp
#include "bya_common.h"
#include "../../include/bya.h"
#include "options.h"
#include "routing_weights.h"

namespace {

template <int MAXM>
__global__ __launch_bounds__(256) void linear_small_m_kernel(const bf16_t* __restrict__ x, const bf16_t* __restrict__ W,
                                                             const bf16_t* __restrict__ bias, bf16_t* __restrict__ out,
                                                             int M, int N, int K, int silu_in, int act_out) {
    const int lane = threadIdx.x & 63;
    const long long n = (long long)blockIdx.x * 4 + (threadIdx.x >> 6);
    if (n >= N) return;
    float acc[MAXM];
#pragma unroll
    for (int m = 0; m < MAXM; ++m) acc[m] = 0.f;
    const bf16_t* wrow = W + n * K;
    for (int k0 = lane * 8; k0 < K; k0 += 512) {
        float wv[8];
        unpack8(*reinterpret_cast<const u32x4*>(wrow + k0), wv);
#pragma unroll
        for (int m = 0; m < MAXM; ++m) {
            if (m < M) {
                float xv[8];
// ... 144 lines not shown
    const long long n = ((long long)t * Ht + h) * Wt + w;
    u32x2 o; o[0] = top; o[1] = bot;
    *reinterpret_cast<u32x2*>(cols + (((long long)b * frames * Ht * Wt + n) * C + c) * 4) = o;
}

__global__ void unpatchify_kernel(const bf16_t* __restrict__ y, bf16_t* __restrict__ out, int batch, int frames, int C,
                                  int H, int W) {
    const int Ht = H / 2, Wt = W / 2;
    const long long idx = (long long)blockIdx.x * blockDim.x + threadIdx.x;
    const long long total = (long long)batch * frames * C * Ht * Wt;
    if (idx >= total) return;
    const int w = (int)(idx % Wt); long long rest = idx / Wt;
    const int h = (int)(rest % Ht); rest /= Ht;
    const int c = (int)(rest % C); rest /= C;
    const int t = (int)(rest % frames);
    const int b = (int)(rest / frames);
    const long long n = ((long long)t * Ht + h) * Wt + w;
    const u32x2 v = *reinterpret_cast<const u32x2*>(y + (((long long)b * frames * Ht * Wt + n) * C + c) * 4);
    bf16_t* dst = out + ((((long long)b * frames + t) * C + c) * H + 2 * h) * W + 2 * w;
    *reinterpret_cast<uint32_t*>(dst) = v[0];
    *reinterpret_cast<uint32_t*>(dst + W) = v[1];
}

__global__ __launch_bounds__(256) void act_add_kernel(const bf16_t* __restrict__ x, const bf16_t* __restrict__ r,
                                                      bf16_t* __restrict__ y, long long nvec, int act) {
    for (long long i = (long long)blockIdx.x * 256 + threadIdx.x; i < nvec; i += (long long)gridDim.x * 256) {
        float v[8];
        unpack8(*reinterpret_cast<const u32x4*>(x + i * 8), v);
#pragma unroll
        for (int e = 0; e < 8; ++e) {
            float t = v[e];
            switch (act) {
                case BYA_ACT_GELU_TANH: t = gelu_tanh(t); break;
                case BYA_ACT_GELU_ERF: t = gelu_erf(t); break;
                case BYA_ACT_RELU: t = t > 0.f ? t : 0.f; break;
                case BYA_ACT_SILU: t = silu(t); break;
                case BYA_ACT_LEAKY_RELU: t = t > 0.f ? t : 0.01f * t; break;
                default: break;
            }
            v[e] = t;
        }
        if (r) {
            float rv[8];
            unpack8(*reinterpret_cast<const u32x4*>(r + i * 8), rv);
#pragma unroll
            for (int e = 0; e < 8; ++e) v[e] = bf2f(f2bf(v[e])) + rv[e];
        }
        *reinterpret_cast<u32x4*>(y + i * 8) = pack8(v);
    }
}

inline int ok() { const hipError_t e = hipGetLastError(); return e == hipSuccess ? BYA_OK : -(1000 + (int)e); }


#pragma clang fp contract(off)
__global__ void __launch_bounds__(256)
cfg_sched_kernel(const bf16_t* __restrict__ pred, long long pred_stride, int n_pred, const bf16_t* __restrict__ x,
                 const float* __restrict__ old_x0, const bf16_t* __restrict__ noise, bf16_t* __restrict__ prev,
                 float* __restrict__ x0_out, long long n, bya_sched_coef c) {
    for (long long i = (long long)blockIdx.x * blockDim.x + threadIdx.x; i < n; i += (long long)gridDim.x * blockDim.x) {
        float v = bf2f(pred[i]);
        if (n_pred == 2) {
            const float cond = bf2f(pred[pred_stride + i]);
            const float diff = cond - v;
            const float scaled = c.guidance * diff;
            v = v + scaled;
        }
        const float xs = bf2f(x[i]);
        const float t1 = bf2f(f2bf(c.sqrt_alpha * xs));
        const float t2 = c.sqrt_beta * v;
        const float x0 = t1 - t2;
        float d = x0;
        if (old_x0) {
            const float cur = c.k_cur * x0;
            const float old = c.k_old * old_x0[i];
            d = cur - old;
        }
        const float t3 = bf2f(f2bf(c.k_sample * xs));
        const float t4 = c.k_denoised * d;
        float r = t3 - t4;
        if (noise) {
            const float tn = bf2f(f2bf(c.k_noise * bf2f(noise[i])));
            r = r + tn;
        }
        prev[i] = f2bf(r);
        if (x0_out) x0_out[i] = x0;
    }
}


struct Lin1 { int i0, i1; float w0, w1; };
__device__ __forceinline__ Lin1 lin_index(int dst, int in_size, int out_size) {
    Lin1 r;
    if (in_size == out_size) { r.i0 = r.i1 = dst; r.w0 = 1.0f; r.w1 = 0.0f; return r; }
    const float scale = (float)in_size / (float)out_size;
    float src = scale * ((float)dst + 0.5f) - 0.5f;
    if (src < 0.0f) src = 0.0f;
    r.i0 = (int)src;
    r.i1 = r.i0 + (r.i0 < in_size - 1 ? 1 : 0);
    float l1 = src - (float)r.i0;
    l1 = fminf(fmaxf(l1, 0.0f), 1.0f);
    r.w1 = l1;
    r.w0 = 1.0f - l1;
    return r;
}

__global__ void __launch_bounds__(256)
masks_to_logits_kernel(const uint8_t* __restrict__ masks, bf16_t* __restrict__ out, int n_id, int Ti, int Hi, int Wi,
                       int To, int Ho, int Wo) {
    const long long n = (long long)To * Ho * Wo;
    const long long tok = (long long)blockIdx.x * blockDim.x + threadIdx.x;
    if (tok >= n) return;
    const int w = (int)(tok % Wo), h = (int)((tok / Wo) % Ho), t = (int)(tok / ((long long)Wo * Ho));
    const Lin1 lt = lin_index(t, Ti, To), lh = lin_index(h, Hi, Ho), lw = lin_index(w, Wi, Wo);
    int label = -1;
    for (int id = 0; id < n_id; ++id) {
        const uint8_t* m = masks + (long long)id * Ti * Hi * Wi;
        auto px = [&](int tt, int hh, int ww) -> float { return m[((long long)tt * Hi + hh) * Wi + ww] > 0 ? 1.0f : 0.0f; };
        auto row = [&](int tt, int hh) -> float {
            float o = px(tt, hh, lw.i0) * lw.w0;
            o += px(tt, hh, lw.i1) * lw.w1;
            return o;
        };
        auto plane = [&](int tt) -> float {
            float o = row(tt, lh.i0) * lh.w0;
            o += row(tt, lh.i1) * lh.w1;
            return o;
        };
        float v = plane(lt.i0) * lt.w0;
        v += plane(lt.i1) * lt.w1;
        if (v > 0.5f) label = id;
    }
    for (int id = 0; id < n_id; ++id) out[tok * n_id + id] = (id == label) ? (bf16_t)0x3F80 : (bf16_t)0;
}

}

extern "C" int bya_abi_version(void) { return 2; }

std::atomic<int32_t> g_bya_options[BYA_OPT_COUNT] = {
    {0},
    {0},
    {-1},
    {0},
    {1},
    {0},
    {0},
    {0},
    {0},
};

extern "C" int bya_set_option(int32_t key, int32_t value) {
    static const int32_t lo[BYA_OPT_COUNT] = {0, 0, -1, 0, 0, 0, 0, 0, 0};
    static const int32_t hi[BYA_OPT_COUNT] = {2, 1 << 20, 6, 2, 1, 1, 1024, 31, 2};
    if (key < 0 || key >= BYA_OPT_COUNT || value < lo[key] || value > hi[key]) return BYA_ERR_SHAPE;
    if (key == BYA_OPT_P2P_GROUPS && value != 0 && value < 16) return BYA_ERR_SHAPE;
    g_bya_options[key].store(value, std::memory_order_relaxed);
    return BYA_OK;
}

extern "C" int bya_get_option(int32_t key, int32_t* value) {
    if (key < 0 || key >= BYA_OPT_COUNT || !value) return BYA_ERR_SHAPE;
    *value = g_bya_options[key].load(std::memory_order_relaxed);
    return BYA_OK;
}

extern "C" int bya_linear_small_m(const void* x, const void* W, const void* bias, void* out, int32_t M, int32_t N,
                                  int32_t K, int32_t silu_in, int32_t act_out, hipStream_t stream) {
    if (!x || !W || !out || M <= 0 || M > 8 || N <= 0 || K <= 0) return BYA_ERR_SHAPE;
    if (K % 8) return BYA_ERR_SHAPE;
    if (((uintptr_t)x | (uintptr_t)W) & 15) return BYA_ERR_ALIGN;
    if (act_out != BYA_ACT_NONE && act_out != BYA_ACT_SILU) return BYA_ERR_UNSUPPORTED;
    dim3 grid((unsigned)((N + 3) / 4));
    if (M <= 2)
        BYA_LAUNCH((linear_small_m_kernel<2>), grid, dim3(256), 0, stream, (const bf16_t*)x, (const bf16_t*)W,
                           (const bf16_t*)bias, (bf16_t*)out, M, N, K, silu_in, act_out);
    else
        BYA_LAUNCH((linear_small_m_kernel<8>), grid, dim3(256), 0, stream, (const bf16_t*)x, (const bf16_t*)W,
                           (const bf16_t*)bias, (bf16_t*)out, M, N, K, silu_in, act_out);
    return ok();
}

extern "C" int bya_timestep_features(const int64_t* timesteps, void* out, int32_t batch, int32_t dim,
                                     int32_t flip_sin_to_cos, float freq_shift, hipStream_t stream) {
    if (!timesteps || !out || batch <= 0 || dim <= 0 || dim % 2) return BYA_ERR_SHAPE;
    const int total = batch * (dim / 2);
    BYA_LAUNCH(timestep_features_kernel, dim3((total + 255) / 256), dim3(256), 0, stream, timesteps,
                       (bf16_t*)out, batch, dim, flip_sin_to_cos, freq_shift);
    return ok();
}

extern "C" int bya_masked_combine(void* x, const void* feat, const void* r, const void* af, int32_t mode, float alpha,
                                  int32_t batch, int32_t n_id, int64_t N, int32_t D, int64_t x_row,
                                  int64_t x_batch_stride, int64_t r_batch_stride, hipStream_t stream) {
    if (!x || !feat || !r || batch <= 0 || N <= 0 || D <= 0) return BYA_ERR_SHAPE;
    if (mode != 0 && mode != 1) return BYA_ERR_UNSUPPORTED;
    if (n_id < 1 || n_id > 4 || (mode == 1 && !af)) return BYA_ERR_UNSUPPORTED;
    if (D % 8 || x_row % 8 || x_batch_stride % 8) return BYA_ERR_ALIGN;
    if (((uintptr_t)x | (uintptr_t)feat) & 15) return BYA_ERR_ALIGN;
    CombArgs a;
    a.x = (bf16_t*)x; a.feat = (const bf16_t*)feat; a.r = (const bf16_t*)r; a.af = (const bf16_t*)af;
    a.mode = mode; a.batch = batch; a.n_id = n_id; a.D = D; a.N = N; a.x_row = x_row; a.x_bs = x_batch_stride;
    a.r_bs = r_batch_stride; a.alpha = alpha;
    const long long total = (long long)batch * N * (D / 8);
    BYA_LAUNCH(masked_combine_kernel, dim3((unsigned)((total + 255) / 256)), dim3(256), 0, stream, a);
    return ok();
}

extern "C" int bya_routed_mix(const void* feat, const void* r, const void* af, void* z, float* wsum, int32_t mode,
                              int32_t batch, int32_t n_id, int64_t N, int32_t D, int64_t r_batch_stride,
                              hipStream_t stream) {
    if (!feat || !r || !z || batch <= 0 || N <= 0 || D <= 0) return BYA_ERR_SHAPE;
    if (mode != 0 && mode != 1) return BYA_ERR_UNSUPPORTED;
    if (n_id < 1 || n_id > 4 || (mode == 1 && !af)) return BYA_ERR_UNSUPPORTED;
    if (D % 8) return BYA_ERR_ALIGN;
    if (((uintptr_t)z | (uintptr_t)feat) & 15) return BYA_ERR_ALIGN;
    CombArgs a;
    a.x = nullptr; a.feat = (const bf16_t*)feat; a.r = (const bf16_t*)r; a.af = (const bf16_t*)af;
    a.mode = mode; a.batch = batch; a.n_id = n_id; a.D = D; a.N = N; a.x_row = 0; a.x_bs = 0;
    a.r_bs = r_batch_stride; a.alpha = 1.0f;
    const long long total = (long long)batch * N * (D / 8);
    BYA_LAUNCH(routed_mix_kernel, dim3((unsigned)((total + 255) / 256)), dim3(256), 0, stream, a, (bf16_t*)z, wsum);
    return ok();
}

extern "C" int bya_forcing_max_over_frames(const void* forcing, void* out, int32_t frames, int64_t per_frame,
                                           int32_t n_id, hipStream_t stream) {
    if (!forcing || !out || frames <= 0 || per_frame <= 0 || n_id <= 0) return BYA_ERR_SHAPE;
    const long long inner = per_frame * n_id;
    BYA_LAUNCH(forcing_max_kernel, dim3((unsigned)((inner + 255) / 256)), dim3(256), 0, stream,
                       (const bf16_t*)forcing, (bf16_t*)out, frames, (long long)per_frame, n_id);
    return ok();
}

extern "C" int bya_patchify(const void* x, void* cols, int32_t batch, int32_t frames, int32_t channels, int32_t H,
                            int32_t W, hipStream_t stream) {
    if (!x || !cols || batch <= 0 || frames <= 0 || channels <= 0 || H <= 0 || W <= 0) return BYA_ERR_SHAPE;
    if (H % 2 || W % 2) return BYA_ERR_SHAPE;
    if (((uintptr_t)x & 3) || ((uintptr_t)cols & 7)) return BYA_ERR_ALIGN;
    const long long total = (long long)batch * frames * channels * (H / 2) * (W / 2);
    BYA_LAUNCH(patchify_kernel, dim3((unsigned)((total + 255) / 256)), dim3(256), 0, stream, (const bf16_t*)x,
                       (bf16_t*)cols, batch, frames, channels, H, W);
    return ok();
}

extern "C" int bya_unpatchify(const void* y, void* out, int32_t batch, int32_t frames, int32_t channels, int32_t H,
                              int32_t W, hipStream_t stream) {
    if (!y || !out || batch <= 0 || frames <= 0 || channels <= 0 || H <= 0 || W <= 0) return BYA_ERR_SHAPE;
    if (H % 2 || W % 2) return BYA_ERR_SHAPE;
    if (((uintptr_t)out & 3) || ((uintptr_t)y & 7)) return BYA_ERR_ALIGN;
    const long long total = (long long)batch * frames * channels * (H / 2) * (W / 2);
    BYA_LAUNCH(unpatchify_kernel, dim3((unsigned)((total + 255) / 256)), dim3(256), 0, stream,
                       (const bf16_t*)y, (bf16_t*)out, batch, frames, channels, H, W);
    return ok();
}

extern "C" int bya_act_add(const void* x, const void* r, void* y, int64_t n, int32_t act, hipStream_t stream) {
    if (!x || !y || n <= 0 || n % 8) return BYA_ERR_SHAPE;
    if (((uintptr_t)x | (uintptr_t)y | (uintptr_t)r) & 15) return BYA_ERR_ALIGN;
    if (act < 0 || act > 5) return BYA_ERR_UNSUPPORTED;
    const long long nvec = n / 8;
    long long blocks = (nvec + 255) / 256;
    if (blocks > 4096) blocks = 4096;
    BYA_LAUNCH(act_add_kernel, dim3((unsigned)blocks), dim3(256), 0, stream, (const bf16_t*)x,
                       (const bf16_t*)r, (bf16_t*)y, nvec, act);
    return ok();
}

extern "C" int bya_cfg_scheduler_step(const void* pred, int32_t n_pred, int64_t pred_stride, const void* sample,
                                      const float* old_x0, const void* noise, void* prev_sample, float* x0_out,
                                      int64_t n, const bya_sched_coef* coef, hipStream_t stream) {
    if (!pred || !sample || !prev_sample || !coef || n <= 0) return BYA_ERR_SHAPE;
    if (n_pred != 1 && n_pred != 2) return BYA_ERR_SHAPE;
    if (n_pred == 2 && pred_stride < n) return BYA_ERR_SHAPE;
    long long blocks = (n + 255) / 256;
    if (blocks > 8192) blocks = 8192;
    BYA_LAUNCH(cfg_sched_kernel, dim3((unsigned)blocks), dim3(256), 0, stream, (const bf16_t*)pred,
               (long long)pred_stride, n_pred, (const bf16_t*)sample, old_x0, (const bf16_t*)noise,
               (bf16_t*)prev_sample, x0_out, (long long)n, *coef);
    return ok();
}

extern "C" int bya_masks_to_routing_logits(const void* masks, void* logits, int32_t n_id, int32_t in_frames,
                                           int32_t in_h, int32_t in_w, int32_t frames, int32_t h, int32_t w,
                                           hipStream_t stream) {
    if (!masks || !logits || n_id <= 0 || in_frames <= 0 || in_h <= 0 || in_w <= 0 || frames <= 0 || h <= 0 || w <= 0)
        return BYA_ERR_SHAPE;
    const long long n = (long long)frames * h * w;
    BYA_LAUNCH(masks_to_logits_kernel, dim3((unsigned)((n + 255) / 256)), dim3(256), 0, stream, (const uint8_t*)masks,
               (bf16_t*)logits, n_id, in_frames, in_h, in_w, frames, h, w);
    return ok();
}
```

### bind_your_avatar_implementation_amd/engine.py

```python
import contextlib
import os

import torch

from . import ops
from .parallel import RouterPartition, SeqShard


def _key(tensors):
    return tuple((t.data_ptr(), t._version, tuple(t.shape)) for t in tensors)


FP8_LINEARS = ("qkv", "out", "ff1", "ff2", "pq", "aq")
FP8_DEFAULT = ("qkv", "out", "ff1", "ff2")


def mx_call_kernel(fmt, w_fmt, persistent_gemm):
    if not persistent_gemm or (fmt, w_fmt) != ("mxfp8", "mxfp4"):
        return 0
    return 2 if persistent_gemm == "always" else 1


class DenoiseEngine:
    MAX_ID = 4
    n_id = None

    def _count_ids(self, id_cond, audio_embeds):
        if self.m.is_train_face and id_cond is not None:
            n = len(id_cond)
        elif audio_embeds is not None and audio_embeds.ndim == 5:
            n = audio_embeds.shape[1]
        else:
            n = 2
        if not 2 <= n <= self.MAX_ID:
            raise ValueError(f"{n} identities: the engine runs 2..{self.MAX_ID} (the reference itself exactly 2)")
        return n

    def __init__(self, model):
        p = model.proj_out.weight
        if not p.is_cuda:
            raise RuntimeError("the Bind-Your-Avatar MI355X engine needs its parameters on a GPU "
                               "(there is no CPU fallback); call model.to('cuda')")
        if p.dtype != torch.bfloat16:
            raise RuntimeError(f"engine computes in bf16 (MFMA, fp32 accumulate); parameters are {p.dtype}")
        ops._hip.load()
        ops.ensure_gemm_workspace(p.device)
        self.m = model
        self.cfg = model.config
        self.dev = p.device
        self.D = model.inner_dim
        self.H = self.cfg.num_attention_heads
        self.L = len(model.transformer_blocks)
        self.Tt_max = self.cfg.max_text_seq_length
        self.cache_invariants = False
        self.k_scale = (self.cfg.attention_head_dim ** -0.5) * 1.4426950408889634
        self.mix_before_projection = os.environ.get("BYA_MIX_BEFORE_PROJECTION", "1") != "0"
        self.fused_attn_mix = self.mix_before_projection and os.environ.get("BYA_FUSED_ATTN_MIX", "1") != "0"
        self.fp8_weights = bool(getattr(model, "_fp8_weights", False)) or os.environ.get("BYA_FP8_WEIGHTS") == "1"
        self.fuse_ln_quant = os.environ.get("BYA_FP8_FUSED_LN", "1") != "0"
        self.mx_fmt = getattr(model, "_mx_weights", None)
        self.mx_wfmt = None
        if self.mx_fmt is not None:
            self.mx_wfmt = getattr(model, "_mx_weight_format", None) or self.mx_fmt
            ops.mx_fmt_pair(self.mx_fmt, self.mx_wfmt)
            if self.fp8_weights:
                raise ValueError("fp8 weights (enable_fp8_weights / BYA_FP8_WEIGHTS) and MX weights (enable_mx_weights) "
                                 "are both requested: enable one of them")
        self.mx_fuse_quant = self.mx_fmt is not None and bool(getattr(model, "_mx_fuse_activation_quant", True))
        self.mx_fuse_attn_quant = self.mx_fmt is not None and bool(getattr(model, "_mx_fuse_attention_quant", False))
        self.mx_fuse_qk_norm = self.mx_fmt is not None and bool(getattr(model, "_mx_fuse_qk_norm", False))
        pg = getattr(model, "_mx_persistent_gemm", False)
        mx8 = self.mx_fmt == "mxfp8" and self.mx_wfmt == "mxfp8"
        self.mx_kernel = (2 if pg == "always" else 1) if (pg and mx8) else 0
        self.mx_call_kernel = mx_call_kernel(self.mx_fmt, self.mx_wfmt, pg)
        self.side_stream_conditioning = os.environ.get("BYA_INVARIANTS_SIDE_STREAM", "1") != "0"
        self.sp_allgather = os.environ.get("BYA_SP_ALLGATHER", "0") == "1"
        self.router_fused_attn = os.environ.get("BYA_ROUTER_FUSED_ATTN", "1") != "0"
        self.router_chain = os.environ.get("BYA_ROUTER_CHAIN", "1")
        self.verify_exchanges = os.environ.get("BYA_SP_VERIFY", "0") == "1"
        self.sp_overlap_v = os.environ.get("BYA_SP_OVERLAP_V", "1") != "0"
        self.sp_shard_mods = os.environ.get("BYA_SP_SHARD_MODS", "1") != "0"
        if os.environ.get("BYA_SP_OVERLAP_V") == "all":
            self.SP_OVERLAP_V_MIN_ROWS = 0
        self.router_replicated = os.environ.get("BYA_ROUTER_REPLICATED", "0") == "1"
        self.qkn_epilogue = os.environ.get("BYA_QKN_EPILOGUE", "1") != "0"
        self._inv_cache = {}
        self._side = None
        self._ws_key, self._ws = None, None
        self._parts = {}
        if model.is_train_audio and not model.is_train_face:
            raise RuntimeError("audio injection needs the face router's logits (models/transformer.py:860)")
        self._pack()

    def _fingerprint(self):
        ptrs = vers = n = 0
        for group in (self.m.parameters(), self.m.buffers()):
            for t in group:
                n += 1
                ptrs += t.data_ptr()
                if not t.is_inference():
                    vers += t._version
        return (n, ptrs, vers)

    def refresh_if_stale(self):
        if self._fingerprint() == self._fp:
            return False
        self._pack()
        self._inv_cache = {}
        self.m._graphs = {}
        return True

    def _pack(self):
        m, D = self.m, self.D
        cat = torch.cat
        self._fp = self._fingerprint()
        self.score_bound = []
        for blk in m.transformer_blocks:
            nq, nk = blk.attn1.norm_q, blk.attn1.norm_k
            bq = 8.0 * nq.weight.float().abs().max().item() + nq.bias.float().norm().item()
            bk = 8.0 * nk.weight.float().abs().max().item() + nk.bias.float().norm().item()
            self.score_bound.append(1.02 * bq * bk * self.k_scale if os.environ.get("BYA_ATTN_BOUNDED", "1") != "0" else 0.0)
        self.device_bound = os.environ.get("BYA_ATTN_DEVICE_BOUND", "1") != "0"
        mods_w, mods_b = [], []
        for blk in m.transformer_blocks:
            for nz in (blk.norm1, blk.norm2):
                mods_w.append(nz.linear.weight)
                mods_b.append(nz.linear.bias)
        mods_w.append(m.norm_out.linear.weight)
        mods_b.append(m.norm_out.linear.bias)
        self.mod_w = cat(mods_w).contiguous()
        self.mod_b = cat(mods_b).contiguous()
        self.patch_w = m.patch_embed.proj.weight.reshape(D, -1)
        self.qkv_w = [cat([b.attn1.to_q.weight, b.attn1.to_k.weight, b.attn1.to_v.weight]).contiguous()
                      for b in m.transformer_blocks]
        self.qkv_b = [cat([b.attn1.to_q.bias, b.attn1.to_k.bias, b.attn1.to_v.bias]).contiguous()
                      for b in m.transformer_blocks]
        self.w8 = None
        blocks = m.transformer_blocks
        source = {"qkv": lambda: self.qkv_w,
                  "out": lambda: [b.attn1.to_out[0].weight for b in blocks],
                  "ff1": lambda: [b.ff.net[0].proj.weight for b in blocks],
                  "ff2": lambda: [b.ff.net[2].weight for b in blocks],
                  "pq": lambda: [pc.to_q.weight for pc in m.perceiver_cross_attention] if m.is_train_face else None,
                  "aq": lambda: [al["attn"].to_q.weight for al in m.audio_model.layers] if m.is_train_audio else None}
        if self.fp8_weights:
            keep = getattr(m, "_fp8_linears", None) or os.environ.get("BYA_FP8_LINEARS") or FP8_DEFAULT
            keep = set(FP8_LINEARS if keep == "all" else keep.split(",")) if isinstance(keep, str) else set(keep)
            unknown = keep - set(FP8_LINEARS)
            if unknown:
                raise ValueError(f"fp8 linears {sorted(unknown)}: expected a subset of {FP8_LINEARS}")
            self.w8 = {}
            for k in FP8_LINEARS:
                ws = source[k]() if k in keep else None
                if ws is not None:
                    self.w8[k] = [ops.quantize_rows_fp8(w) for w in ws]
        self.wmx = None
        if self.mx_fmt is not None:
            keep = getattr(m, "_mx_linears", None) or FP8_DEFAULT
            keep = set(FP8_LINEARS if keep == "all" else keep.split(",")) if isinstance(keep, str) else set(keep)
            unknown = keep - set(FP8_LINEARS)
            if unknown:
                raise ValueError(f"MX linears {sorted(unknown)}: expected a subset of {FP8_LINEARS}")
            self.wmx = {}
            for k in FP8_LINEARS:
                ws = source[k]() if k in keep else None
                if ws is not None:
                    self.wmx[k] = [ops.quantize_mx(w.contiguous(), self.mx_wfmt) for w in ws]
        pe = getattr(m.patch_embed, "pos_embedding", None)
        use_pe = (not self.cfg.use_rotary_positional_embeddings) or self.cfg.use_learned_positional_embeddings
        self.pos_embedding = pe[0] if (pe is not None and use_pe) else None
        if m.is_train_face:
            r = m.router
            qk = r.norm_q.weight.numel()
            hd = qk // r.heads
            j = torch.arange(qk, device=self.dev)
            perm = (j % hd) * r.heads + j // hd
            self.r_nq_w, self.r_nq_b = r.norm_q.weight[perm].contiguous(), r.norm_q.bias[perm].contiguous()
            self.r_nk_w, self.r_nk_b = r.norm_k.weight[perm].contiguous(), r.norm_k.bias[perm].contiguous()
            self.r_to_q = [l.weight[:, perm].contiguous() for l in r.to_q]
            self.r_to_k = [l.weight[:, perm].contiguous() for l in r.to_k]
            self.r_pos = r.pos_emb.reshape(-1, r.feat_dim).contiguous()
            self.r_qkv = []
            for st in r.spatial_temporal_layers:
                packed = {}
                for name in ("spatial_attn", "temporal_attn", "multi_id_attn"):
                    a = getattr(st, name)
                    packed[name] = (cat([a.to_q.weight, a.to_k.weight, a.to_v.weight]).contiguous(),
                                    cat([a.to_q.bias, a.to_k.bias, a.to_v.bias]).contiguous())
                if r.feat_dim == 512 and os.environ.get("BYA_ROUTER_ROWGEMM", "1") != "0":
                    for name, ln in (("spatial_attn", st.norm1), ("temporal_attn", st.norm2), ("multi_id_attn", st.norm3)):
                        a = getattr(st, name)
                        w, b = packed[name]
                        if name == "spatial_attn":
                            c = (64 ** -0.5) * 1.4426950408889634
                            F_ = r.feat_dim
                            w, b = w.float().clone(), b.float().clone()
                            w[F_:2 * F_] *= c
                            b[F_:2 * F_] *= c
                        packed["rg_" + name] = (ops.pack_rowgemm512(w, b, ln.weight, ln.bias), ln.eps,
                                                ops.pack_rowgemm512(a.to_out[0].weight, a.to_out[0].bias))
                    packed["rg_mlp"] = (ops.pack_rowgemm512(st.mlp[0].weight, st.mlp[0].bias, st.norm4.weight, st.norm4.bias),
                                        st.norm4.eps, ops.pack_rowgemm512(st.mlp[2].weight, st.mlp[2].bias))
                self.r_qkv.append(packed)
            self.lfe_proj_t = m.local_facial_extractor.proj_out.t().contiguous()
        if m.is_train_audio:
            cw = m.audio_model.audio_proj_model.conv1.weight
            self.conv_w = cw.permute(0, 2, 1).reshape(cw.shape[0], -1).contiguous()
            att = [l["attn"] for l in m.audio_model.layers]
            self.audio_kv_w = cat([w for a in att for w in (a.to_k.weight, a.to_v.weight)]).contiguous()
            self.audio_kv_b = cat([b for a in att for b in (a.to_k.bias, a.to_v.bias)]).contiguous()

    def _shard(self, rank, world, S, Tt, group):
        key = ("seq", rank, world, S, Tt, id(group))
        sh = self._parts.get(key)
        if sh is None:
            sh = self._parts[key] = SeqShard(rank, world, S, Tt, group, getattr(self.m, "_seq_p2p", None) if group is not None else None)
        return sh

    def _router_partition(self, sh, pairs, per_frame):
        key = ("router", sh.rank, sh.world, pairs, per_frame, id(sh.group))
        rp = self._parts.get(key)
        if rp is None:
            rp = self._parts[key] = RouterPartition(sh.rank, sh.world, pairs, per_frame, sh.group, sh.p2p)
        return rp

    def _buf(self, name, *shape):
        t = self._ws.get(name)
        if t is None or tuple(t.shape) != tuple(shape):
            t = torch.empty(*shape, dtype=torch.bfloat16, device=self.dev)
            self._ws[name] = t
# ... 138 lines not shown
        idc = self._bf(torch.cat([id_cond[i] for i in range(n_id)], 0))
        vit = [self._bf(torch.cat([id_vit_hidden[i][k] for i in range(n_id)], 0)) for k in range(5)]
        n_vit = vit[0].shape[1]
        E = lambda *s: torch.empty(*s, dtype=torch.bfloat16, device=self.dev)

        def mapper(seq, x, out_last):
            h = x
            for a, b in ((0, 1), (3, 4)):
                t = E(*h.shape[:-1], seq[a].weight.shape[0])
                self._linear(h, seq[a].weight, seq[a].bias, t)
                self._ln(t, t, seq[b])
                ops.act_add(t, t, act="leaky_relu")
                h = t
            return self._linear(h, seq[6].weight, seq[6].bias, out_last)

        x_tok = mapper(lfe.id_embedding_mapping, idc, E(G, nt * dim)).view(G, nt, dim)
        lat = E(G, nq + nt, dim)
        lat[:, :nq] = lfe.latents.to(torch.bfloat16)
        lat[:, nq:] = x_tok
        n_ctx, n_lat = nt + n_vit, nq + nt
        ctx = E(G, n_ctx, dim)
        ctx[:, :nt] = x_tok
        kvin = E(G, n_ctx + n_lat, dim)
        inner = lfe.heads * lfe.dim_head
        q, kv = E(G, n_lat, inner), E(G, n_ctx + n_lat, 2 * inner)
        ao, f = E(G, n_lat, inner), E(G, n_lat, dim)
        hid = E(G, n_lat, lfe.layers[0][1][1].weight.shape[0])
        for lvl in range(5):
            mapper(getattr(lfe, f"mapping_{lvl}"), vit[lvl], ctx[:, nt:])
            for attn, ff in lfe.layers[lvl * lfe.depth:(lvl + 1) * lfe.depth]:
                self._ln(ctx, kvin[:, :n_ctx], attn.norm1)
                self._ln(lat, kvin[:, n_ctx:], attn.norm2)
                ops.gemm(kvin[:, n_ctx:], attn.to_q.weight, q)
                ops.gemm(kvin, attn.to_kv.weight, kv)
                ops.self_attention(q, kv[:, :, :inner], kv[:, :, inner:], ao, heads=lfe.heads,
                                   head_dim=lfe.dim_head)
                ops.gemm(ao, attn.to_out.weight, lat, res=lat)
                self._ln(lat, f, ff[0])
                ops.gemm(f, ff[1].weight, hid, act="gelu_erf")
                ops.gemm(hid, ff[3].weight, lat, res=lat)
        face_all = E(G, nq, self.lfe_proj_t.shape[0])
        ops.gemm(lat[:, :nq], self.lfe_proj_t, face_all)
        face = face_all.view(n_id, B, nq, -1).transpose(0, 1).contiguous()
        self.last_face_emb = face

        kvs, krs = [], []
        face2d = face.view(B * n_id * nq, -1)
        fn = E(*face2d.shape)
        for l, pc in enumerate(m.perceiver_cross_attention):
            self._ln(face2d, fn, pc.norm1)
            kv_l = E(B * n_id * nq, pc.to_kv.weight.shape[0])
            ops.gemm(fn.view(B * n_id, nq, -1), pc.to_kv.weight, kv_l.view(B * n_id, nq, -1))
            inner_p = pc.to_q.weight.shape[0]
            kn = E(B * n_id * nq, inner_p)
            ops.layernorm(kv_l[:, :inner_p], kn, self.r_nk_w, self.r_nk_b, eps=m.router.norm_k.eps)
            kr_l = E(B * n_id * nq, inner_p)
            ops.gemm(kn.view(B * n_id, nq, -1), self.r_to_k[l], kr_l.view(B * n_id, nq, -1))
            kvs.append(kv_l.view(B, n_id, nq, -1))
            krs.append(kr_l.view(B, n_id, nq, -1))
            if after_layer is not None:
                after_layer(l)
        return kvs, krs

    def _audio_invariants(self, audio_embeds, T, B, n_id):
        with ops.weight_streaming():
            return self._audio_invariants_body(audio_embeds, T, B, n_id)

    def _audio_invariants_body(self, audio_embeds, T, B, n_id):
        am = self.m.audio_model
        ap = am.audio_proj_model
        mono = audio_embeds.dim() == 4
        if mono:
            mute = am.mute_audio_embeds
            if mute is None:
                mute = torch.load("tests/input/ae_mute.pt")
            mute = self._bf(mute[:T * 4 + 1].to(self.dev))
            if mute.shape != audio_embeds.shape[1:]:
                raise AssertionError(f"cur_audio_context_tokens.shape: {tuple(audio_embeds.shape[1:])} frames x blocks x "
                                     f"channels, mute_context_tokens.shape: {tuple(mute.shape)}")
            audio_embeds = torch.stack([self._bf(audio_embeds), mute.unsqueeze(0).expand_as(audio_embeds)], dim=1)
        a = self._bf(audio_embeds).contiguous()
        bs, ni, F, blk, ch = a.shape
        assert bs == B and ni == n_id
        assert 1 + (T - 1) * 4 + (am.window_size - am.window_stride) == F, \
            f"hidden_states_num_frames: {T}, window_size: {am.window_size}, window_stride: {am.window_stride}, " \
            f"audio_embeds.shape[1]: {F}"
        G, per = B * n_id, blk * ch
        nwin = F - am.window_size + 1
        E = lambda *s: torch.empty(*s, dtype=torch.bfloat16, device=self.dev)
        win = torch.as_strided(a, (G, nwin, am.window_size * per), (F * per, per, 1))
        h1, h2 = E(G, nwin, ap.proj1.weight.shape[0]), E(G, nwin, ap.proj2.weight.shape[0])
        ops.gemm(win, ap.proj1.weight, h1, bias=ap.proj1.bias, act="relu")
        ops.gemm(h1, ap.proj2.weight, h2, bias=ap.proj2.bias, act="relu")
        C = ap.proj3.weight.shape[0]
        cur = E(G, nwin, C)
        ops.gemm(h2, ap.proj3.weight, cur, bias=ap.proj3.bias)
        for _ in range(2):
            n = cur.shape[1]
            keep = n % 2
            n_out = (n - keep) // 2
            nxt = E(G, keep + n_out, C)
            if keep:
                nxt[:, 0] = cur[:, 0]
            if n_out > 0:
                pairs = torch.as_strided(cur, (G, n_out, 2 * C), (n * C, 2 * C, 1), cur.storage_offset() + keep * C)
                ops.gemm(pairs, self.conv_w, nxt[:, keep:], bias=ap.conv1.bias)
            cur = nxt
        assert cur.shape[1] == T
        tok = ap.context_tokens
        ctx = E(G * T * tok, ap.output_dim)
        self._ln(cur.view(G * T * tok, ap.output_dim), ctx, ap.norm)
        if mono:
            ctx.view(B, n_id, T, tok, ap.output_dim)[:, 1] += am.mute_learnable_tokens.view(1, 1, tok, ap.output_dim)
        self.last_audio_ctx = ctx.view(B, n_id, T, tok, ap.output_dim)
        rows, inner = G * T * tok, am.layers[0]["attn"].to_k.weight.shape[0]
        kv = E(2 * len(am.layers), rows, inner)
        ops.gemm(ctx, self.audio_kv_w, kv[0], bias=self.audio_kv_b, split=(inner, rows * inner))
        ks = [kv[2 * l].view(B, n_id, T, tok, -1) for l in range(len(am.layers))]
        vs = [kv[2 * l + 1].view(B, n_id, T, tok, -1) for l in range(len(am.layers))]
        return ks, vs

    def _cached(self, name, tensors, fn):
        if not self.cache_invariants:
            return fn()
        key = _key(tensors)
        hit = self._inv_cache.get(name)
        if hit is not None and hit[0] == key:
            return hit[2]
        val = fn()
        self._inv_cache[name] = (key, list(tensors), val)
        return val

    @torch.no_grad()
    def precompute(self, id_cond=None, id_vit_hidden=None, audio_embeds=None, latent_frames=13):
        self.cache_invariants = True
        self._inv_cache = {}
        n_id = self._count_ids(id_cond, audio_embeds)
        if self.m.is_train_face and id_cond is not None:
            B = id_cond[0].shape[0]
            flat = list(id_cond[:n_id]) + [t for i in range(n_id) for t in id_vit_hidden[i]]
            self._cached("face", flat, lambda: self._face_invariants(id_cond, id_vit_hidden, B, n_id))
        if self.m.is_train_audio and audio_embeds is not None:
            self._cached("audio", [audio_embeds],
                         lambda: self._audio_invariants(audio_embeds, latent_frames, audio_embeds.shape[0], n_id))
        return self

    def release(self):
        self.cache_invariants = False
        self._inv_cache = {}

    @torch.no_grad()
    def step(self, *args, **kwargs):
        self.refresh_if_stale()
        with ops.pinned_stream():
            return self._step(*args, **kwargs)

    def _step(self, hidden_states, encoder_hidden_states, timestep, image_rotary_emb, id_cond, id_vit_hidden,
              audio_embeds, af_matrix, routing_logits_forcing, taps=None):
        n_id = self.n_id = self._count_ids(id_cond, audio_embeds)
        m, cfg, D, H = self.m, self.cfg, self.D, self.H
        B, T, C, Hh, Ww = hidden_states.shape
        ht, wt = Hh // 2, Ww // 2
        per_frame, N = ht * wt, T * ht * wt
        Tt = encoder_hidden_states.shape[1]
        S = Tt + N
        sh = self._shard(getattr(m, "_seq_rank", 0), getattr(m, "_seq_world", 1), S, Tt, getattr(m, "_seq_group", None))
        if sh.active and B != 1:
            raise NotImplementedError("sequence-parallel execution shards ONE sample; split a CFG batch over rank groups")
        S_loc, Tt_loc, N_loc, v0, v1 = sh.S_loc, sh.Tt_loc, sh.N_loc, sh.v0, sh.v1
        key = (B, T, C, Hh, Ww, Tt, sh.rank, sh.world, n_id)
        if self._ws_key != key:
            self._ws_key, self._ws = key, {}
            if sh.p2p is not None:
                sh.p2p.drop_tables()
        sh.begin_step()
        buf = self._buf
        hs = self._bf(hidden_states)
        enc_in = self._bf(encoder_hidden_states)
        if not torch.is_tensor(timestep):
            timestep = torch.tensor([timestep] * B)
        ts = timestep.to(device=self.dev, dtype=torch.int64).reshape(-1)
        if ts.numel() == 1 and B > 1:
            ts = ts.expand(B)
        ts = ts.contiguous()
        use_face = m.is_train_face
        use_audio = m.is_train_audio and audio_embeds is not None
        if use_face and m.router.frames * m.router.height * m.router.width != N:
            raise ValueError(f"router positional table is {m.router.frames}x{m.router.height}x{m.router.width} "
                             f"but the latents give {T}x{wt}x{ht} tokens")
        cos = sin = None
        if image_rotary_emb is not None:
            cos = image_rotary_emb[0].to(device=self.dev, dtype=torch.float32)[v0:v1].contiguous()
            sin = image_rotary_emb[1].to(device=self.dev, dtype=torch.float32)[v0:v1].contiguous()

        inv_side, face_marks, audio_mark = None, {}, [None]
        if (use_face or use_audio) and ops._TIMERS is None and self.side_stream_conditioning:
            if self._side is None:
                self._side = torch.cuda.Stream(self.dev)
            inv_side = ops.on_stream(self._side)
        with (inv_side if inv_side is not None else contextlib.nullcontext()):
            audio_res = []

            def audio_now():
                if use_audio and not audio_res:
                    audio_res.append(self._cached("audio", [audio_embeds], lambda: self._audio_invariants(audio_embeds, T, B, n_id)))
                    if inv_side is not None:
                        audio_mark[0] = inv_side.mark()

            def after_face_layer(l):
                if inv_side is not None:
                    face_marks[l] = inv_side.mark()
                if l == 0:
                    audio_now()
            if use_face:
                flat_face = list(id_cond[:n_id]) + [t for i in range(n_id) for t in id_vit_hidden[i]]
                face_kv, router_k = self._cached("face", flat_face,
                                                 lambda: self._face_invariants(id_cond, id_vit_hidden, B, n_id, after_face_layer))
            audio_now()
            if use_audio:
                audio_k, audio_v = audio_res[0]
        if use_audio:
            af = self._bf(af_matrix)
        forced = None
        if routing_logits_forcing is not None and use_face:
            f_in = self._bf(routing_logits_forcing).reshape(T, per_frame, n_id)
            forced = ops.forcing_max_over_frames(f_in, buf("forced", 1, N, n_id).view(T, per_frame, n_id), T, per_frame,
                                                 n_id).view(1, N, n_id)[:, v0:v1].contiguous()

        tfeat = ops.timestep_features(ts, buf("tfeat", B, D), cfg.flip_sin_to_cos, float(cfg.freq_shift))
        te = m.time_embedding
        e1 = ops.linear_small_m(tfeat, te.linear_1.weight, te.linear_1.bias, buf("e1", B, te.linear_1.weight.shape[0]),
                                act_out="silu")
        emb = ops.linear_small_m(e1, te.linear_2.weight, te.linear_2.bias, buf("emb", B, te.linear_2.weight.shape[0]))
        Nm = self.mod_w.shape[0]
        if sh.active and sh.p2p is not None and B == 1 and self.sp_shard_mods:
            W, r = sh.world, sh.rank
            cut = [(Nm * j // W) // 8 * 8 for j in range(W)] + [Nm]
            part = buf("mods_part", 1, cut[r + 1] - cut[r])
            ops.linear_small_m(emb, self.mod_w[cut[r]:cut[r + 1]], self.mod_b[cut[r]:cut[r + 1]], part, silu_in=True)
            mods = sh.p2p.symmetric(f"mods:{(1, Nm)}", (1, Nm), torch.bfloat16)
            sh._exchange(("mods", Nm), [(part[0], j, f"mods:{(1, Nm)}", cut[r]) for j in range(W)])
        else:
            mods = ops.linear_small_m(emb, self.mod_w, self.mod_b, buf("mods", B, Nm), silu_in=True)
        mbs = mods.stride(0)

        x = buf("x", B, S_loc, D)
        xv = x[:, Tt_loc:]
        pe = self.pos_embedding
        if pe is not None and pe.shape[0] != S:
            raise ValueError("learned positional embeddings need the configured sample height/width/frames")
        if Tt_loc:
            tp = m.patch_embed.text_proj
            ops.gemm(enc_in[:, sh.r0:sh.r0 + Tt_loc], tp.weight, x[:, :Tt_loc], bias=tp.bias,
                     res=None if pe is None else pe[sh.r0:sh.r0 + Tt_loc])
        cols = ops.patchify(hs, buf("cols", B, N, C * 4))
        ops.gemm(cols[:, v0:v1], self.patch_w, xv, bias=m.patch_embed.proj.bias,
                 res=None if pe is None else pe[Tt + v0:Tt + v1])
        if taps is not None:
            taps["emb"], taps["embed"] = emb.clone(), x.clone()

        xn = buf("xn", B, S_loc, D)
        qkv = buf("qkv", 3, B, S_loc, D)
        q, k, v = qkv[0], qkv[1], qkv[2]
        ff = buf("ff", B, S_loc, 4 * D)
        head_parallel = sh.active and H % sh.world == 0 and not self.sp_allgather
        if head_parallel:
            W = sh.world
            Dl = D // W
            qkvb = buf("qkv_blocks", 3 * W, S_loc, Dl)
            qh, kh, vh = buf("q_heads", S, Dl), buf("k_heads", S, Dl), buf("v_heads", S, Dl)
            oh = buf("o_heads", S, Dl)
        elif sh.active:
            k_full, v_full = buf("k_full", 1, S, D), buf("v_full", 1, S, D)
        r_logits = None
        for i, blk in enumerate(m.transformer_blocks):
            for half, nz in enumerate((blk.norm1, blk.norm2)):
                mo = mods[:, (2 * i + half) * 6 * D:]
                ln_kw = dict(eps=nz.norm.eps, shift0=mo[:, 3 * D:], scale0=mo[:, 4 * D:], shift1=mo, scale1=mo[:, D:],
                             split=Tt_loc, mod_batch_stride=mbs)
                xq = None
                if self._quantised(("qkv", "ff1")[half]) and self.fuse_ln_quant:
                    xq = self._layernorm_quant(("qkv", "ff1")[half], x, xn.shape, nz.norm.weight, nz.norm.bias, **ln_kw)
                else:
                    ops.layernorm(x, xn, nz.norm.weight, nz.norm.bias, **ln_kw)
                if half == 0:
                    at = blk.attn1
                    if head_parallel:
                        if sh.p2p is None:
                            self._dit_linear("qkv", i, xn[0], self.qkv_w[i], qkvb[0], bias=self.qkv_b[i], split=(Dl, S_loc * Dl),
                                             quantised=None if xq is None else (xq[0][0], xq[1][0]))
                        qk_kw = dict(heads=H // W, text_rows=Tt_loc if cos is not None else S_loc, eps=at.norm_q.eps,
                                     k_scale=self.k_scale)
                        if sh.p2p is not None:
                            sb, st = self._attn_bound(i, H, slots=max(1, 64 // W))
                            if (self.sp_overlap_v and st is None and xq is None and not self._quantised("qkv")
                                    and S_loc >= self.SP_OVERLAP_V_MIN_ROWS):
                                ops.gemm(xn[0], self.qkv_w[i][2 * D:], qkvb[2 * W], bias=self.qkv_b[i][2 * D:], split=(Dl, S_loc * Dl))
                                sh.push_v_heads(qkvb[2 * W:])
                                if not (self.qkn_epilogue and ops.gemm_qkv_norm_rope(
                                        xn[0], self.qkv_w[i][:2 * D], qkvb[0], self.qkv_b[i][:2 * D], (Dl, S_loc * Dl), at.norm_q.weight,
                                        at.norm_q.bias, at.norm_k.weight, at.norm_k.bias, cos, sin, qk_kw["text_rows"], eps=at.norm_q.eps,
                                        k_scale=self.k_scale, tensors=2)):
                                    ops.gemm(xn[0], self.qkv_w[i][:2 * D], qkvb[0], bias=self.qkv_b[i][:2 * D], split=(Dl, S_loc * Dl))
                                    ops.qknorm_rope(qkvb[:W], qkvb[W:2 * W], at.norm_q.weight, at.norm_q.bias, at.norm_k.weight,
                                                    at.norm_k.bias, cos, sin, heads=H // W, text_rows=qk_kw["text_rows"],
                                                    eps=at.norm_q.eps, k_scale=self.k_scale)
                                qh_, kh_, vh_ = sh.rows_to_heads_qk(qkvb[:2 * W])
# ... 322 lines not shown
```

### bind_your_avatar_implementation_amd/ops.py

```python
import ctypes
import os

import torch

from . import _hip
from ._hip import AttnDesc, AttnMixDesc, GemmDesc, check

ACT = {None: 0, "none": 0, "gelu_tanh": 1, "gelu_erf": 2, "relu": 3, "silu": 4, "leaky_relu": 5,
       "gelu_tanh_ieee": 6}


_PINNED_STREAM = None


def _stream():
    if _PINNED_STREAM is not None:
        return _PINNED_STREAM
    return torch.cuda.current_stream().cuda_stream


class pinned_stream:

    def __enter__(self):
        global _PINNED_STREAM
# ... 206 lines not shown

def gemm_workspace_status(device=None):
    lib = _hip.load()
    idx = torch.cuda.current_device() if device is None else torch.device(device).index
    n = ctypes.c_int32(0)
    with torch.cuda.device(idx):
        check(lib.bya_gemm_workspace_status(ctypes.byref(n), _stream()), "bya_gemm_workspace_status")
    return n.value


_HEALED = {}
HANDOFF_MODE = {}


def _handoff_counts(device=None):
    idx = None if device is None else torch.device(device).index
    if idx is None:
        idx = torch.cuda.current_device()
    g = gemm_workspace_status(idx) if idx in _GEMM_WS else 0
    a = attn_workspace_status(idx) if idx in _ATTN_WS else 0
    seen = _HEALED.get(idx, [0, 0])
    return idx, g - seen[0], a - seen[1], g, a


def heal_handoffs(device=None):
    idx, g_new, a_new, g, a = _handoff_counts(device)
    if not (g_new or a_new):
        return False
    _HEALED[idx] = [g, a]
    set_option("gemm_splitk", 0)
    set_option("attn_streamk", 0)
    HANDOFF_MODE[idx] = (f"unsplit (self-healed: {g_new} split-K and {a_new} stream-K hand-off(s) timed out -- the launch's grid was "
                         f"not co-resident, the GPU is shared; gemm_splitk = attn_streamk = 0 from here on)")
    import warnings
    warnings.warn("bind_your_avatar_implementation_amd: " + HANDOFF_MODE[idx] + "; the step is re-run")
    return True


def check_gemm_workspace(device=None):
    idx, g_new, a_new, _, _ = _handoff_counts(device)
    if g_new:
        raise _hip.ByaError(f"{g_new} split-K tile(s) of bya_gemm_bf16 were finished without all their partial sums (a hand-off "
                            f"between workgroups timed out): results of this run are not to be trusted")
    if a_new:
        raise _hip.ByaError(f"{a_new} stream-K hand-off(s) of the joint attention timed out: results of this run are not to be trusted")
    import sys
    p2p = sys.modules.get(__package__ + ".p2p")
    if p2p is not None:
        for g in list(p2p.LIVE_GROUPS):
            g.check()


_ATTN_WS = {}


def ensure_attn_workspace(device):
    device = torch.device(device)
    idx = device.index if device.index is not None else torch.cuda.current_device()
    ws = _ATTN_WS.get(idx)
    if ws is not None:
        return ws
    lib = _hip.load()
    n = ctypes.c_int64(0)
    check(lib.bya_attn_workspace_bytes(ctypes.byref(n)), "bya_attn_workspace_bytes")
    with torch.cuda.device(idx):
        ws = torch.zeros(n.value, dtype=torch.uint8, device=torch.device("cuda", idx))
        torch.cuda.synchronize(idx)
        check(lib.bya_set_attn_workspace(ws.data_ptr(), n.value), "bya_set_attn_workspace")
    _ATTN_WS[idx] = ws
    return ws


def attn_workspace_status(device=None):
    lib = _hip.load()
    idx = torch.cuda.current_device() if device is None else torch.device(device).index
    n = ctypes.c_int32(0)
    with torch.cuda.device(idx):
        check(lib.bya_attn_workspace_status(ctypes.byref(n), _stream()), "bya_attn_workspace_status")
    return n.value


def _gemm_desc(a, w, out, res, gate_split, gate_batch_stride, act, split, bias_rowscale, alpha, plan=False):
    ab, M, K, a_bs, lda = _mat(a, "a", plan)
    ob, Mo, N, c_bs, ldc = _mat(out, "out", plan)
    if split is not None:
        N = w.shape[0]
    if w.dim() != 2 or w.shape[1] != K or w.shape[0] != N or w.stride(1) != 1 or w.dtype != torch.bfloat16:
        raise ValueError(f"w: expected bf16 [{N}, {K}], got {tuple(w.shape)} {w.dtype}")
    if (ab, M) != (ob, Mo):
        raise ValueError("a/out row mismatch")
    d = GemmDesc()
    d.M, d.N, d.K, d.batch = M, N, K, ab
    d.lda, d.ldw, d.ldc = lda, w.stride(0), ldc
    d.a_batch_stride, d.c_batch_stride = a_bs, c_bs
    d.ldres, d.res_batch_stride = 0, 0
    if res is not None:
        rb, Mr, Nr, r_bs, ldres = _mat(res, "res", plan)
        if (Mr, Nr) != (M, N) or rb not in (1, ab):
            raise ValueError("res shape mismatch")
        d.ldres, d.res_batch_stride = ldres, (r_bs if rb == ab else 0)
    d.gate_batch_stride, d.gate_split, d.act = gate_batch_stride, gate_split, ACT[act]
    d.n_split, d.c_split_stride = (0, 0) if split is None else split
    d.bias_rowscale, d.alpha = (_plan_p if plan else _p)(bias_rowscale), float(alpha)
    if bias_rowscale is not None:
        assert bias_rowscale.dtype == torch.float32 and bias_rowscale.is_contiguous() and bias_rowscale.numel() == ab * M
    return d


def _takes_skinny(d, gate0, bias_rowscale, split):
    return (_WEIGHT_STREAMING and d.M <= 64 and d.N <= 8192 and d.N % 16 == 0 and d.K % 32 == 0 and d.K >= 256 and gate0 is None
            and bias_rowscale is None and split is None and d.a_batch_stride % 8 == 0)


def gemm(a, w, out, bias=None, res=None, gate0=None, gate1=None, gate_split=0, gate_batch_stride=0, act=None,
         split=None, bias_rowscale=None, alpha=1.0):
    lib = _hip.load()
    d = _gemm_desc(a, w, out, res, gate_split, gate_batch_stride, act, split, bias_rowscale, alpha)
    if a.device.index not in _GEMM_WS:
        ensure_gemm_workspace(a.device)
    ab, M, N, K = d.batch, d.M, d.N, d.K
    name = "bya_gemm_bf16" if M >= 1024 else "bya_gemm_bf16_small_m"
    if _SHAPE_LABELS:
        name += f":{ab}x{M}x{N}x{K}:{act or 'none'}{'+gate' if gate0 is not None else ''}{'+res' if res is not None else ''}"
    tok = _begin(name, 2.0 * ab * M * N * K)
    if _takes_skinny(d, gate0, bias_rowscale, split):
        check(lib.bya_gemm_skinny_bf16(_p(a), _p(w), _p(bias), _p(out), _p(res), ctypes.byref(d), _stream()),
              "bya_gemm_skinny_bf16")
    else:
        check(lib.bya_gemm_bf16(_p(a), _p(w), _p(bias), _p(out), _p(res), _p(gate0), _p(gate1), ctypes.byref(d),
                                _stream()), "bya_gemm_bf16")
    _end(tok)
    return out


GEMM_PATHS = _hip.GEMM_PATHS


def _plan_dict(p):
    return {"path": GEMM_PATHS[p.path], "m0": p.m0, "tail": GEMM_PATHS.get(p.tail) if p.m0 > 0 else None,
            "split_k": p.split_k, "row_chunks": p.row_chunks}


def plan_key(plan):
    return plan["path"] + (f"|{plan['tail']}" if plan["tail"] else "") + ("+splitk" if plan["split_k"] else "")


def gemm_plan(a, w, out, bias=None, res=None, gate0=None, gate1=None, gate_split=0, gate_batch_stride=0, act=None,
              split=None, bias_rowscale=None, alpha=1.0):
    lib = _hip.load()
    d = _gemm_desc(a, w, out, res, gate_split, gate_batch_stride, act, split, bias_rowscale, alpha, plan=True)
    if a.is_cuda and a.device.index not in _GEMM_WS:
        ensure_gemm_workspace(a.device)
    if _takes_skinny(d, gate0, bias_rowscale, split):
        return {"path": "skinny", "m0": 0, "tail": None, "split_k": 0, "row_chunks": 1}
    p, q = _hip.GemmPlan(), _plan_p
    check(lib.bya_gemm_bf16_plan(q(a), q(w), q(bias), q(out), q(res), q(gate0), q(gate1), ctypes.byref(d),
                                 ctypes.byref(p)), "bya_gemm_bf16_plan")
    return _plan_dict(p)


def _qkn_descs(a, w, out, split, qw, qb, kw, kb, cos, sin, text_rows, eps, k_scale, tensors, plan=False):
    ab, M, K, a_bs, lda = _mat(a, "a", plan)
    ob, Mo, _, c_bs, ldc = _mat(out, "out", plan)
    N = w.shape[0]
    if w.dim() != 2 or w.shape[1] != K or w.stride(1) != 1 or w.dtype != torch.bfloat16 or tensors not in (2, 3) or N % tensors \
            or (ab, M) != (ob, Mo):
        raise ValueError("gemm_qkv_norm_rope: a [(B,) M, K], w [3 * width, K] (or [2 * width, K]: q | k alone, tensors=2), "
                         "out = the first of the split outputs")
    d = GemmDesc()
    d.M, d.N, d.K, d.batch = M, N, K, ab
    d.lda, d.ldw, d.ldc = lda, w.stride(0), ldc
    d.a_batch_stride, d.c_batch_stride = a_bs, c_bs
    d.n_split, d.c_split_stride = split
    d.alpha = 1.0
    n = _hip.QkNormDesc()
    ptr = _plan_p if plan else _p
    n.qw, n.qb, n.kw, n.kb, n.cos, n.sin = ptr(qw), ptr(qb), ptr(kw), ptr(kb), ptr(cos), ptr(sin)
    n.text_rows, n.width, n.eps, n.k_scale = int(text_rows), N // tensors, float(eps), float(k_scale)
    if cos is not None:
        assert cos.dtype == torch.float32 and sin.dtype == torch.float32 and cos.is_contiguous() and sin.is_contiguous()
        assert cos.shape == (M - text_rows, 64)
    return d, n


def gemm_qkv_norm_rope(a, w, out, bias, split, qw, qb, kw, kb, cos, sin, text_rows, eps=1e-6, k_scale=1.0, tensors=3):
    lib = _hip.load()
    d, n = _qkn_descs(a, w, out, split, qw, qb, kw, kb, cos, sin, text_rows, eps, k_scale, tensors)
    ab, M, N, K = d.batch, d.M, d.N, d.K
    tok = _begin("bya_gemm_bf16" if M >= 1024 else "bya_gemm_bf16_small_m")
    rc = lib.bya_gemm_qkv_norm_rope(_p(a), _p(w), _p(bias), _p(out), ctypes.byref(d), ctypes.byref(n), _stream())
    if rc == -4:
        return False
    check(rc, "bya_gemm_qkv_norm_rope")
    if tok is not None:
        _FLOPS[tok[0]] = _FLOPS.get(tok[0], 0.0) + 2.0 * ab * M * N * K
    _end(tok)
    return True


def gemm_qkv_norm_rope_plan(a, w, out, bias, split, qw, qb, kw, kb, cos, sin, text_rows, eps=1e-6, k_scale=1.0, tensors=3):
    lib = _hip.load()
    d, n = _qkn_descs(a, w, out, split, qw, qb, kw, kb, cos, sin, text_rows, eps, k_scale, tensors, plan=True)
    p, q = _hip.GemmPlan(), _plan_p
    rc = lib.bya_gemm_qkv_norm_rope_plan(q(a), q(w), q(bias), q(out), ctypes.byref(d), ctypes.byref(n), ctypes.byref(p))
    if rc == -4:
        return None
    check(rc, "bya_gemm_qkv_norm_rope_plan")
    return _plan_dict(p)


def quantize_rows_fp8(x, q=None, scale=None):
    lib = _hip.load()
    b, M, K, bs, ldx = _mat(x, "x")
    if b > 1 and bs != M * ldx:
        raise ValueError("quantize_rows_fp8: batch entries must be evenly stacked rows")
    if q is None:
        q = torch.empty(*x.shape, dtype=torch.uint8, device=x.device)
    if scale is None:
        scale = torch.empty(*x.shape[:-1], dtype=torch.float32, device=x.device)
    assert q.dtype == torch.uint8 and q.is_contiguous() and scale.dtype == torch.float32 and scale.is_contiguous()
    assert q.numel() == b * M * K and scale.numel() == b * M
    tok = _begin("bya_quantize_rows_fp8")
    check(lib.bya_quantize_rows_fp8(_p(x), _p(q), _p(scale), b * M, K, ldx, K, _stream()), "bya_quantize_rows_fp8")
    _end(tok)
    return q, scale


def _fp8_desc(a8, a_scale, w8, w_scale, out, res, gate_split, gate_batch_stride, act, split, alpha, plan=False):
    if a8.dim() == 2:
        ab, (M, K) = 1, a8.shape
    else:
        ab, M, K = a8.shape
    ob, Mo, N, c_bs, ldc = _mat(out, "out", plan)
    if split is not None:
        N = w8.shape[0]
    assert a8.dtype == torch.uint8 and w8.dtype == torch.uint8 and a8.is_contiguous() and w8.is_contiguous()
    assert w8.shape == (N, K) and (ab, M) == (ob, Mo)
    assert a_scale.dtype == torch.float32 and a_scale.numel() == ab * M and a_scale.is_contiguous()
    assert w_scale.dtype == torch.float32 and w_scale.numel() == N and w_scale.is_contiguous()
    d = GemmDesc()
    d.M, d.N, d.K, d.batch = M, N, K, ab
    d.lda, d.ldw, d.ldc = K, K, ldc
    d.a_batch_stride, d.c_batch_stride = M * K, c_bs
    d.ldres, d.res_batch_stride = 0, 0
    if res is not None:
        rb, Mr, Nr, r_bs, ldres = _mat(res, "res", plan)
        if (Mr, Nr) != (M, N) or rb not in (1, ab):
            raise ValueError("res shape mismatch")
        d.ldres, d.res_batch_stride = ldres, (r_bs if rb == ab else 0)
    d.gate_batch_stride, d.gate_split, d.act = gate_batch_stride, gate_split, ACT[act]
    d.n_split, d.c_split_stride = (0, 0) if split is None else split
    d.bias_rowscale, d.alpha = None, float(alpha)
    return d


def gemm_fp8(a8, a_scale, w8, w_scale, out, bias=None, res=None, gate0=None, gate1=None, gate_split=0,
             gate_batch_stride=0, act=None, split=None, alpha=1.0):
    lib = _hip.load()
    d = _fp8_desc(a8, a_scale, w8, w_scale, out, res, gate_split, gate_batch_stride, act, split, alpha)
    ab, M, N, K = d.batch, d.M, d.N, d.K
    name = "bya_gemm_fp8"
    if _SHAPE_LABELS:
        name += f":{ab}x{M}x{N}x{K}:{act or 'none'}{'+gate' if gate0 is not None else ''}{'+res' if res is not None else ''}"
    tok = _begin(name, 2.0 * ab * M * N * K)
    check(lib.bya_gemm_fp8(_p(a8), _p(a_scale), _p(w8), _p(w_scale), _p(bias), _p(out), _p(res), _p(gate0), _p(gate1),
                           ctypes.byref(d), _stream()), "bya_gemm_fp8")
    _end(tok)
    return out


def gemm_fp8_plan(a8, a_scale, w8, w_scale, out, bias=None, res=None, gate0=None, gate1=None, gate_split=0,
                  gate_batch_stride=0, act=None, split=None, alpha=1.0):
    lib = _hip.load()
    d = _fp8_desc(a8, a_scale, w8, w_scale, out, res, gate_split, gate_batch_stride, act, split, alpha, plan=True)
    p, q = _hip.GemmPlan(), _plan_p
    check(lib.bya_gemm_fp8_plan(q(a8), q(a_scale), q(w8), q(w_scale), q(bias), q(out), q(res), q(gate0), q(gate1),
                                ctypes.byref(d), ctypes.byref(p)), "bya_gemm_fp8_plan")
    return _plan_dict(p)



MX_FORMATS = {"mxfp8": 0, "mxfp6": 2}
MX_WEIGHT_FORMATS = {**MX_FORMATS, "mxfp4": 4}
MX_BITS = {"mxfp8": 8, "mxfp6": 6, "mxfp4": 4}


def mx_fmt_code(fmt):
    if fmt not in MX_FORMATS:
        raise ValueError(f"MX format {fmt!r}: expected one of {sorted(MX_FORMATS)}")
    return MX_FORMATS[fmt]


def mx_weight_fmt_code(fmt):
    if fmt not in MX_WEIGHT_FORMATS:
        raise ValueError(f"MX weight format {fmt!r}: expected one of {sorted(MX_WEIGHT_FORMATS)}")
    return MX_WEIGHT_FORMATS[fmt]


def mx_fmt_pair(fmt, w_fmt):
    a = mx_fmt_code(fmt)
    w = a if w_fmt is None else mx_weight_fmt_code(w_fmt)
    if w not in (a, MX_WEIGHT_FORMATS["mxfp4"]):
        raise ValueError(f"MX weight format {w_fmt!r} under {fmt!r} activations: expected {fmt!r} or 'mxfp4'")
    return a, w


def mx_code_bytes(K, fmt):
    mx_weight_fmt_code(fmt)
    return K * MX_BITS[fmt] // 8


# ... 896 lines not shown
```

### include/bya.h

```cpp
#ifndef BYA_H
#define BYA_H

#include <stdint.h>

#ifdef __cplusplus
extern "C" {
#endif
#if defined(__GNUC__) || defined(__clang__)
#pragma GCC visibility push(default)
#endif

#ifndef __HIP_PLATFORM_AMD__
typedef struct ihipStream_t* hipStream_t;
#endif

enum { BYA_ACT_NONE = 0, BYA_ACT_GELU_TANH = 1, BYA_ACT_GELU_ERF = 2, BYA_ACT_RELU = 3, BYA_ACT_SILU = 4,
       BYA_ACT_LEAKY_RELU = 5,
       BYA_ACT_GELU_TANH_IEEE = 6  };

int bya_abi_version(void);

enum bya_option {
    BYA_OPT_GEMM_SPLITK = 0,
    BYA_OPT_GEMM_SPLITK_MIN = 1,
    BYA_OPT_GEMM_TILE = 2,
    BYA_OPT_GEMM_VARIANT = 3,
    BYA_OPT_ATTN_STREAMK = 4,
    BYA_OPT_FP8_KERNEL = 5,
    BYA_OPT_P2P_GROUPS = 6,
    BYA_OPT_REFERENCE_FORMS = 7,
    BYA_OPT_MX_KERNEL = 8,
    BYA_OPT_COUNT = 9
};
enum { BYA_REF_ROWGEMM_CHUNKED = 1,
       BYA_REF_KV_MIX_GENERIC = 2,
       BYA_REF_LN_GENERIC = 4,
       BYA_REF_ROUTER_SCORES_WAVE = 8,
       BYA_REF_ATTN_NARROW_STORE = 16   };
int bya_set_option(int32_t key, int32_t value);
int bya_get_option(int32_t key, int32_t* value);

#define BYA_CALIBRATION_OPERAND_BYTES (256LL * 256 * 16 * 16)
#define BYA_CALIBRATION_FLOP_PER_ITER (256.0 * 4 * 2.0 * 128 * 128 * 32)
int bya_mfma_calibration(const void* operands, int64_t operand_bytes, void* sink, int32_t iters, hipStream_t stream);

typedef struct bya_gemm_desc {
    int32_t M, N, K;
    int32_t batch;
    int32_t lda, ldw, ldc, ldres;
    int64_t a_batch_stride, c_batch_stride, res_batch_stride, gate_batch_stride;
    int32_t gate_split;
    int32_t act;
    int32_t n_split;
    int64_t c_split_stride;
    const float* bias_rowscale;
    float alpha;
} bya_gemm_desc;

int bya_gemm_bf16(const void* A, const void* W, const void* bias, void* C, const void* res,
                  const void* gate0, const void* gate1, const bya_gemm_desc* desc, hipStream_t stream);

typedef struct bya_qknorm_desc {
    const void* qw; const void* qb; const void* kw; const void* kb;
    const float* cos; const float* sin;
    int32_t text_rows;
    int32_t width;
    float eps, k_scale;
} bya_qknorm_desc;
int bya_gemm_qkv_norm_rope(const void* A, const void* W, const void* bias, void* C, const bya_gemm_desc* desc,
                           const bya_qknorm_desc* norm, hipStream_t stream);

int bya_gemm_skinny_bf16(const void* A, const void* W, const void* bias, void* C, const void* res,
                         const bya_gemm_desc* desc, hipStream_t stream);

int bya_set_gemm_workspace(void* ws, int64_t bytes);
int bya_gemm_workspace_bytes(int64_t* bytes);
int bya_gemm_workspace_status(int32_t* timeouts, hipStream_t stream);

#define BYA_GEMM_PATH_T128X64 0
#define BYA_GEMM_PATH_T128X128 1
#define BYA_GEMM_PATH_T256X128 2
#define BYA_GEMM_PATH_T256X256 3
#define BYA_GEMM_PATH_P256 4
#define BYA_GEMM_PATH_P128 5
#define BYA_GEMM_PATH_P128S 6
#define BYA_GEMM_PATH_W8_256 7
#define BYA_GEMM_PATH_COUNT 8
typedef struct bya_gemm_plan {
    int32_t path;
    int32_t m0;
    int32_t tail;
    int32_t split_k;
    int32_t row_chunks;
} bya_gemm_plan;
int bya_gemm_bf16_plan(const void* A, const void* W, const void* bias, const void* C, const void* res,
                       const void* gate0, const void* gate1, const bya_gemm_desc* desc, bya_gemm_plan* plan);
int bya_gemm_qkv_norm_rope_plan(const void* A, const void* W, const void* bias, const void* C, const bya_gemm_desc* desc,
                                const bya_qknorm_desc* norm, bya_gemm_plan* plan);

int bya_quantize_rows_fp8(const void* x, void* q, float* scale, int32_t M, int32_t K, int64_t ldx, int64_t ldq,
                          hipStream_t stream);
int bya_gemm_fp8(const void* A8, const float* a_scale, const void* W8, const float* w_scale, const void* bias, void* C,
                 const void* res, const void* gate0, const void* gate1, const bya_gemm_desc* desc, hipStream_t stream);
int bya_gemm_fp8_plan(const void* A8, const float* a_scale, const void* W8, const float* w_scale, const void* bias,
                      const void* C, const void* res, const void* gate0, const void* gate1, const bya_gemm_desc* desc,
                      bya_gemm_plan* plan);
int bya_layernorm_fp8(const void* x, void* q, float* q_scale, const void* w, const void* b, const void* shift0,
                      const void* scale0, const void* shift1, const void* scale1, int64_t rows_per_batch, int32_t batch,
                      int32_t D, int64_t ldx, int64_t ldq, int64_t x_batch_stride, int64_t q_batch_stride,
                      int64_t mod_batch_stride, int64_t split, float eps, hipStream_t stream);

enum { BYA_MX_E4M3 = 0, BYA_MX_E2M3 = 2, BYA_MX_E2M1 = 4 };
int bya_quantize_mx(const void* x, void* codes, void* scales, int32_t M, int32_t K, int64_t ldx, int32_t fmt,
                    hipStream_t stream);
int bya_layernorm_mx(const void* x, void* q, void* q_scales, const void* w, const void* b, const void* shift0,
                     const void* scale0, const void* shift1, const void* scale1, int64_t rows_per_batch, int32_t batch,
                     int32_t D, int64_t ldx, int64_t ldq, int64_t x_batch_stride, int64_t q_batch_stride,
                     int64_t mod_batch_stride, int64_t split, float eps, int32_t fmt, hipStream_t stream);
int bya_gemm_mx(const void* A, const void* a_scales, const void* W, const void* w_scales, const void* bias, void* C,
                const void* res, const void* gate0, const void* gate1, const bya_gemm_desc* desc, int32_t fmt,
                hipStream_t stream);
int bya_gemm_mx_plan(const void* A, const void* a_scales, const void* W, const void* w_scales, const void* bias,
                     const void* C, const void* res, const void* gate0, const void* gate1, const bya_gemm_desc* desc,
                     int32_t fmt, bya_gemm_plan* plan);
int bya_gemm_mx_mixed(const void* A, const void* a_scales, const void* W, const void* w_scales, const void* bias, void* C,
                      const void* res, const void* gate0, const void* gate1, const bya_gemm_desc* desc, int32_t a_fmt,
                      int32_t w_fmt, hipStream_t stream);
int bya_gemm_mx_mixed_plan(const void* A, const void* a_scales, const void* W, const void* w_scales, const void* bias,
                           const void* C, const void* res, const void* gate0, const void* gate1,
                           const bya_gemm_desc* desc, int32_t a_fmt, int32_t w_fmt, bya_gemm_plan* plan);
int bya_gemm_mx_quant(const void* A, const void* a_scales, const void* W, const void* w_scales, const void* bias,
                      void* q_codes, void* q_scales, const bya_gemm_desc* desc, int32_t a_fmt, int32_t w_fmt,
                      int32_t out_fmt, hipStream_t stream);
int bya_gemm_mx_quant_plan(const void* A, const void* a_scales, const void* W, const void* w_scales, const void* bias,
                           const void* q_codes, const void* q_scales, const bya_gemm_desc* desc, int32_t a_fmt,
                           int32_t w_fmt, int32_t out_fmt, bya_gemm_plan* plan);
int bya_gemm_mx_qkv_norm_rope(const void* A, const void* a_scales, const void* W, const void* w_scales, const void* bias,
                              void* C, int32_t fmt, int32_t w_fmt, const bya_gemm_desc* desc, const bya_qknorm_desc* norm,
                              hipStream_t stream);
int bya_gemm_mx_qkv_norm_rope_plan(const void* A, const void* a_scales, const void* W, const void* w_scales,
                                   const void* bias, const void* C, int32_t fmt, int32_t w_fmt, const bya_gemm_desc* desc,
                                   const bya_qknorm_desc* norm, bya_gemm_plan* plan);
int bya_gemm_mx_qkv_norm_rope_on(const void* A, const void* a_scales, const void* W, const void* w_scales, const void* bias,
                                 void* C, int32_t fmt, int32_t w_fmt, const bya_gemm_desc* desc, const bya_qknorm_desc* norm,
                                 int32_t kernel, hipStream_t stream);
int bya_gemm_mx_qkv_norm_rope_on_plan(const void* A, const void* a_scales, const void* W, const void* w_scales,
                                      const void* bias, const void* C, int32_t fmt, int32_t w_fmt, const bya_gemm_desc* desc,
                                      const bya_qknorm_desc* norm, int32_t kernel, bya_gemm_plan* plan);
typedef struct bya_mx_gemm_call {
    const void *A, *a_scales, *W, *w_scales, *bias;
    void* C;
    const void *res, *gate0, *gate1;
    void* q_scales;
    const bya_qknorm_desc* norm;
    int32_t a_fmt, w_fmt, out_fmt, kernel;
} bya_mx_gemm_call;
int bya_gemm_mx_call(const bya_mx_gemm_call* call, const bya_gemm_desc* desc, hipStream_t stream);
int bya_gemm_mx_call_plan(const bya_mx_gemm_call* call, const bya_gemm_desc* desc, bya_gemm_plan* plan);

int bya_linear_small_m(const void* x, const void* W, const void* bias, void* out, int32_t M, int32_t N,
                       int32_t K, int32_t silu_in, int32_t act_out, hipStream_t stream);

int bya_timestep_features(const int64_t* timesteps, void* out, int32_t batch, int32_t dim,
                          int32_t flip_sin_to_cos, float freq_shift, hipStream_t stream);

int bya_layernorm(const void* x, void* y, const void* w, const void* b, const void* shift0, const void* scale0,
                  const void* shift1, const void* scale1, int64_t rows_per_batch, int32_t batch, int32_t D,
                  int64_t ldx, int64_t ldy, int64_t x_batch_stride, int64_t y_batch_stride,
                  int64_t mod_batch_stride, int64_t split, float eps, hipStream_t stream);
#define BYA_LN_OUT_BF16 0
#define BYA_LN_OUT_FP8 1
#define BYA_LN_OUT_MX_E4M3 2
#define BYA_LN_OUT_MX_E2M3 3
#define BYA_LN_KERNEL_GENERIC 0
#define BYA_LN_KERNEL_ROWS 1
typedef struct bya_layernorm_plan_info {
    int32_t kernel;
    int32_t vec, nv;
    int32_t modulated;
    int32_t rows_per_wave;
    int32_t grid;
    int64_t waves;
} bya_layernorm_plan_info;
int bya_layernorm_plan(const void* x, const void* y, const void* w, const void* b, const void* shift0, const void* scale0,
                       const void* shift1, const void* scale1, int64_t rows_per_batch, int32_t batch, int32_t D, int64_t ldx,
                       int64_t ldy, int64_t x_batch_stride, int64_t y_batch_stride, int64_t mod_batch_stride, int64_t split,
                       int32_t out_kind, bya_layernorm_plan_info* plan);

int bya_qknorm_rope(void* q, void* k, const void* qw, const void* qb, const void* kw, const void* kb,
                    const float* cos, const float* sin, int32_t batch, int32_t S, int32_t heads, int64_t ld,
                    int64_t batch_stride, int32_t text_rows, float eps, float k_scale, float* stats, int32_t stats_slots,
                    hipStream_t stream);
typedef struct bya_qknorm_rope_plan_info {
    int32_t stats;
    int32_t only;
    int32_t grid;
    int32_t slots;
    int64_t pairs;
    int64_t waves;
} bya_qknorm_rope_plan_info;
int bya_qknorm_rope_plan(const void* q, const void* k, const void* qw, const void* qb, const void* kw, const void* kb,
                         const float* cos, const float* sin, int32_t batch, int32_t S, int32_t heads, int64_t ld,
                         int64_t batch_stride, int32_t text_rows, const float* stats, int32_t stats_slots,
                         bya_qknorm_rope_plan_info* plan);

typedef struct bya_attn_desc {
    int32_t head_dim;
    int32_t heads;
    int32_t nb1, nb2;
    int32_t Sq, Skv;
    int64_t q_s1, q_s2, q_row;
    int64_t k_s1, k_s2, k_row;
    int64_t v_s1, v_s2, v_row;
    int64_t o_s1, o_s2, o_row;
    float scale;
    int32_t scores_prescaled;
    float score_bound;
    const float* bound_dev;
    int32_t bound_slots, bound_heads, bound_bh0;
    int32_t* fallback_flags;
} bya_attn_desc;
#define BYA_ATTN_BOUND_LIMIT 90.0f

int bya_attn_fwd(const void* q, const void* k, const void* v, void* o, const bya_attn_desc* desc,
                 hipStream_t stream);

#define BYA_ATTN_D64_RUNNING_MAX 0
#define BYA_ATTN_D64_PRESCALED 1
#define BYA_ATTN_D64_STATIC_BOUND 2
#define BYA_ATTN_D128 3
#define BYA_ATTN_D64_STATIC_BOUND_W4 4
#define BYA_ATTN_D64_DEVICE_BOUND_W4 5
int bya_attn_variant(const bya_attn_desc* desc);

typedef struct bya_attn_plan_info {
    int32_t variant;
    int32_t grid;
    int32_t q_tile;
    int32_t stream_k;
    int32_t sk_rem;
    int32_t sk_cut;
    int32_t o_wide;
    int32_t second_launch;
} bya_attn_plan_info;
int bya_attn_plan(const bya_attn_desc* desc, const void* o, int32_t workspace_assumed, bya_attn_plan_info* plan);

int bya_attn_fwd_mx(const void* q, const void* k, const void* v, void* codes, void* scales, const bya_attn_desc* desc,
                    int32_t out_fmt, int64_t c_s1, int64_t c_s2, int64_t c_row, int64_t sc_s1, int64_t sc_s2, int64_t sc_row,
                    hipStream_t stream);
// ... 177 lines not shown
```

Baseline: 2.881 steps/s.

## Add 96-row persistent GEMM tile variant for tail pieces to cut wave quantization

Templates the persistent 128x256 streaming GEMM kernel on the number of 32-row A fragments and adds a 96x256 instance with its own hand-written MFMA/LDS schedule. A cost model picks 96-row tiles for the tail piece of a split GEMM when fewer tiles fit the 256-CU rounds better, derating 96-row tiles by a relative-efficiency factor. The engine turns this variant on by default during each step. In exchange, the smaller tile has lower arithmetic intensity per tile, and the cost-model constant is a guess.

```diff
diff --git a/bind_your_avatar_implementation_amd/_hip.py b/bind_your_avatar_implementation_amd/_hip.py
--- a/bind_your_avatar_implementation_amd/_hip.py
+++ b/bind_your_avatar_implementation_amd/_hip.py
@@ -91,6 +91,7 @@
 SIGNATURES = {
     "bya_abi_version": [],
     "bya_set_option": [_i32, _i32],
+    "bya_gemm_bf16_loader_rows": [_vp, _vp, _vp, _vp, _vp, _vp, _vp, _c.POINTER(GemmDesc), _c.POINTER(_i32)],
     "bya_get_option": [_i32, _c.POINTER(_i32)],
     "bya_mfma_calibration": [_vp, _i64, _vp, _i32, _vp],
     "bya_gemm_bf16": [_vp, _vp, _vp, _vp, _vp, _vp, _vp, _c.POINTER(GemmDesc), _vp],
@@ -200,7 +201,7 @@
     "BYA_GEMM_SPLITK": ("gemm_splitk", int),
     "BYA_GEMM_SPLITK_MIN": ("gemm_splitk_min", int),
     "BYA_GEMM_TILE": ("gemm_tile", int),
-    "BYA_GEMM_VARIANT": ("gemm_variant", lambda v: {"w8": 1, "no128": 2}.get(v, 0)),
+    "BYA_GEMM_VARIANT": ("gemm_variant", lambda v: {"w8": 1, "no128": 2, "tail96": 3}.get(v, 0)),
     "BYA_ATTN_STREAMK": ("attn_streamk", int),
     "BYA_FP8_KERNEL": ("fp8_kernel", lambda v: 1 if v.startswith("1") else 0),
     "BYA_P2P_GROUPS": ("p2p_groups", int),
diff --git a/bind_your_avatar_implementation_amd/csrc/gemm.hip b/bind_your_avatar_implementation_amd/csrc/gemm.hip
--- a/bind_your_avatar_implementation_amd/csrc/gemm.hip
+++ b/bind_your_avatar_implementation_amd/csrc/gemm.hip
@@ -255,7 +255,8 @@
         a.c_bs % 8 == 0 && a.res_bs % 8 == 0 && a.gate_bs % 8 == 0 && a.c_split_stride % 8 == 0;
 }
 
-inline bool p128_eligible(const GemmArgs& a) { return v4_eligible(a) && a.K >= 4 * BK && a.conv_cpg_log2 < 0 && bya_opt(BYA_OPT_GEMM_VARIANT) == 0; }
+inline bool p128_variant() { const int v = bya_opt(BYA_OPT_GEMM_VARIANT); return v == 0 || v == 3 || v == 4; }
+inline bool p128_eligible(const GemmArgs& a) { return v4_eligible(a) && a.K >= 4 * BK && a.conv_cpg_log2 < 0 && p128_variant(); }
 
 inline int path256(const GemmArgs& a) {
     return v4_eligible(a) && bya_opt(BYA_OPT_GEMM_VARIANT) != 1 ? BYA_GEMM_PATH_P256 : BYA_GEMM_PATH_W8_256;
@@ -287,6 +288,17 @@
 inline double rounds_128(int M, int N, int batch, double rel) {
     const long long t = (long long)((M + 127) / 128) * ((N + 255) / 256) * batch;
     return 0.5 * (double)((t + 255) / 256) / rel;
+}
+constexpr double REL_96S = 0.83;
+inline int tail_tile_rows(int rows, int N) {
+    const long long tn = (N + 255) / 256;
+    const double c128 = 128.0 * (double)((((rows + 127) / 128) * tn + 255) / 256);
+    const double c96 = 96.0 * (double)((((rows + 95) / 96) * tn + 255) / 256) / REL_96S;
+    return c96 < c128 ? 96 : 128;
+}
+inline int loader_tile_rows(bool is_tail, int rows, int N) {
+    const int opt = bya_opt(BYA_OPT_GEMM_VARIANT);
+    return opt == 4 ? 96 : (opt == 3 && is_tail) ? tail_tile_rows(rows, N) : 128;
 }
 inline double rounds_256_split(int M, int N, int K, int batch) {
     const long long tiles = (long long)((M + 255) / 256) * ((N + 255) / 256) * batch, full = tiles / 256, rem = tiles % 256;
@@ -390,6 +402,7 @@
 namespace {
 int dispatch_gemm(const GemmArgs& a, int nbatch, hipStream_t stream);
 void plan_gemm(const GemmArgs& a, int nbatch, bya_gemm_plan* p);
+int plan_loader_rows(const GemmArgs& a, const bya_gemm_plan& p);
 
 int bf16_args(const void* A, const void* W, const void* bias, const void* C, const void* res, const void* gate0,
               const void* gate1, const bya_gemm_desc* d, GemmArgs* out) {
@@ -470,6 +483,19 @@
     if (!chunks) return BYA_ERR_UNSUPPORTED;
     plan_gemm(piece, nb, plan);
     plan->row_chunks = chunks;
+    return BYA_OK;
+}
+
+extern "C" int bya_gemm_bf16_loader_rows(const void* A, const void* W, const void* bias, const void* C, const void* res,
+                                         const void* gate0, const void* gate1, const bya_gemm_desc* d, int32_t* rows) {
+    if (!rows) return BYA_ERR_SHAPE;
+    GemmArgs a, piece;
+    int rc = bf16_args(A, W, bias, C, res, gate0, gate1, d, &a), nb = 0;
+    if (rc != BYA_OK) return rc;
+    if (!gemm_first_chunk(a, d->batch, &piece, &nb)) return BYA_ERR_UNSUPPORTED;
+    bya_gemm_plan p;
+    plan_gemm(piece, nb, &p);
+    *rows = plan_loader_rows(piece, p);
     return BYA_OK;
 }
 
@@ -654,7 +680,13 @@
     if (p->path == BYA_GEMM_PATH_P256) p->split_k = bya_gemm256p_split(&a, nbatch);
 }
 
-int launch_path(int path, const GemmArgs& a, int batch, hipStream_t stream) {
+int plan_loader_rows(const GemmArgs& a, const bya_gemm_plan& p) {
+    if (p.m0 > 0) return p.tail == BYA_GEMM_PATH_P128S ? loader_tile_rows(true, a.M - p.m0, a.N) : 0;
+    return p.path == BYA_GEMM_PATH_P128S ? loader_tile_rows(false, a.M, a.N) : 0;
+}
+
+int launch_path(int path, const GemmArgs& a, int batch, hipStream_t stream, int loader_rows = 128) {
+    if (path == BYA_GEMM_PATH_P128S && loader_rows == 96) return bya_launch_gemm96s(&a, batch, stream);
     switch (path) {
         case BYA_GEMM_PATH_T128X64: return launch<128, 64, 2, 2>(a, batch, stream);
         case BYA_GEMM_PATH_T128X128: return launch<128, 128, 2, 2>(a, batch, stream);
@@ -681,9 +713,9 @@
         if (hi.bias_rowscale) hi.bias_rowscale += p.m0;
         hi.gate_split = a.gate_split > p.m0 ? a.gate_split - p.m0 : 0;
         const int rc = launch_path(p.path, lo, 1, stream);
-        return rc != BYA_OK ? rc : launch_path(p.tail, hi, 1, stream);
-    }
-    return launch_path(p.path, a, nbatch, stream);
+        return rc != BYA_OK ? rc : launch_path(p.tail, hi, 1, stream, plan_loader_rows(a, p));
+    }
+    return launch_path(p.path, a, nbatch, stream, plan_loader_rows(a, p));
 }
 }
 
diff --git a/bind_your_avatar_implementation_amd/csrc/gemm_common.h b/bind_your_avatar_implementation_amd/csrc/gemm_common.h
--- a/bind_your_avatar_implementation_amd/csrc/gemm_common.h
+++ b/bind_your_avatar_implementation_amd/csrc/gemm_common.h
@@ -215,3 +215,4 @@
 int bya_launch_gemm128p(const void* args, int batch, hipStream_t stream);
 int bya_launch_gemm128p_qkn(const void* args, int batch, hipStream_t stream);
 int bya_launch_gemm128s(const void* args, int batch, hipStream_t stream);
+int bya_launch_gemm96s(const void* args, int batch, hipStream_t stream);
diff --git a/bind_your_avatar_implementation_amd/csrc/gemm_persistent.h b/bind_your_avatar_implementation_amd/csrc/gemm_persistent.h
--- a/bind_your_avatar_implementation_amd/csrc/gemm_persistent.h
+++ b/bind_your_avatar_implementation_amd/csrc/gemm_persistent.h
@@ -96,6 +96,7 @@
 #define DMA_PIECE(Q, BASE, VO, RS, SOFF) dma_piece<(Q) * 1024>(BASE, VO[Q], RS, SOFF)
 #define ALL4(M, ...) M(0, __VA_ARGS__); M(1, __VA_ARGS__); M(2, __VA_ARGS__); M(3, __VA_ARGS__)
 #define ALL8(M, ...) ALL4(M, __VA_ARGS__); M(4, __VA_ARGS__); M(5, __VA_ARGS__); M(6, __VA_ARGS__); M(7, __VA_ARGS__)
+#define KEEP3(F) asm volatile("" :: "v"(F[0]), "v"(F[1]), "v"(F[2]))
 #define KEEP4(F) asm volatile("" :: "v"(F[0]), "v"(F[1]), "v"(F[2]), "v"(F[3]))
 #define KEEP8(F) asm volatile("" :: "v"(F[0]), "v"(F[1]), "v"(F[2]), "v"(F[3]), "v"(F[4]), "v"(F[5]), "v"(F[6]), "v"(F[7]))
 
diff --git a/bind_your_avatar_implementation_amd/csrc/gemm_v6.hip b/bind_your_avatar_implementation_amd/csrc/gemm_v6.hip
--- a/bind_your_avatar_implementation_amd/csrc/gemm_v6.hip
+++ b/bind_your_avatar_implementation_amd/csrc/gemm_v6.hip
@@ -7,10 +7,13 @@
 
 namespace {
 
-__global__ __launch_bounds__(512, 1) void gemm128s_kernel(GemmArgs p, int tiles_m, int tiles_n, int batch) {
+template <int NJ>
+__device__ __forceinline__ void gemm_s_body(const GemmArgs& p, int tiles_m, int tiles_n, int batch) {
     extern __shared__ __attribute__((aligned(16))) char smem[];
-    constexpr int BM = 128, BN = 256, TILE_A = BM * BK * 2, STAGE = (BM + BN) * BK * 2;
-    static_assert(TILE_A == 16384 && STAGE == 49152, "three stages fill 144 KiB");
+    constexpr int BM = 32 * NJ, BN = 256, TILE_A = BM * BK * 2, STAGE = (BM + BN) * BK * 2;
+    constexpr int PIECES = NJ + 8;
+    static_assert(NJ == 3 || NJ == 4, "the schedule tables of tools/gen_gemm_v6_schedule.py");
+    static_assert(3 * STAGE <= 147456, "three stages fill at most 144 KiB");
     const int tid = threadIdx.x, lane = tid & 63;
     const int wave = __builtin_amdgcn_readfirstlane(tid >> 6);
     const int nk = p.K / BK;
@@ -23,10 +26,10 @@
 
     if (wave >= 4) {
         const int lw = wave - 4;
-        uint32_t voA[4], voW[8];
+        uint32_t voA[NJ], voW[8];
 #pragma unroll
-        for (int q = 0; q < 4; ++q) {
-            const int rl = lw * 32 + q * 8 + (lane >> 3);
+        for (int q = 0; q < NJ; ++q) {
+            const int rl = lw * (8 * NJ) + q * 8 + (lane >> 3);
             voA[q] = stage_off(lane, rl, rl, (uint32_t)(p.lda * 2));
         }
 #pragma unroll
@@ -34,23 +37,25 @@
             const int rl = lw * 64 + q * 8 + (lane >> 3);
             voW[q] = stage_off(lane, rl, w_slot_col(rl), (uint32_t)(p.ldw * 2));
         }
-        uint32_t fillA = __builtin_amdgcn_readfirstlane(lds0 + lw * 32 * 128);
+        uint32_t fillA = __builtin_amdgcn_readfirstlane(lds0 + lw * (8 * NJ) * 128);
         uint32_t fillW = __builtin_amdgcn_readfirstlane(lds0 + TILE_A + lw * 64 * 128);
         int st = 0;
         i32x4 rsA = tile_rsrc_a(p, p.A, cur), rsW = tile_rsrc_w(p, p.W, cur);
 #define DMA_A(Q, BASE, RS, SOFF) DMA_PIECE(Q, BASE, voA, RS, SOFF)
 #define DMA_W(Q, BASE, RS, SOFF) DMA_PIECE(Q, BASE, voW, RS, SOFF)
-        ALL4(DMA_A, fillA, rsA, 0u);
+#define ALL_A(BASE, RS, SOFF) do { DMA_A(0, BASE, RS, SOFF); DMA_A(1, BASE, RS, SOFF); DMA_A(2, BASE, RS, SOFF); \
+            if constexpr (NJ > 3) DMA_A(3, BASE, RS, SOFF); } while (0)
+        ALL_A(fillA, rsA, 0u);
         ALL8(DMA_W, fillW, rsW, 0u);
-        ALL4(DMA_A, fillA + STAGE, rsA, (uint32_t)(BK * 2));
+        ALL_A(fillA + STAGE, rsA, (uint32_t)(BK * 2));
         ALL8(DMA_W, fillW + STAGE, rsW, (uint32_t)(BK * 2));
-        ALL4(DMA_A, fillA + 2 * STAGE, rsA, (uint32_t)(2 * BK * 2));
+        ALL_A(fillA + 2 * STAGE, rsA, (uint32_t)(2 * BK * 2));
         ALL8(DMA_W, fillW + 2 * STAGE, rsW, (uint32_t)(2 * BK * 2));
-        asm volatile("s_waitcnt vmcnt(24)\n\ts_barrier" ::: "memory");
+        asm volatile("s_waitcnt vmcnt(%0)\n\ts_barrier" :: "n"(2 * PIECES) : "memory");
         auto refill = [&](const i32x4& dA, const i32x4& dW, uint32_t soff) {
-            asm volatile("s_waitcnt vmcnt(12)\n\ts_barrier" ::: "memory");
+            asm volatile("s_waitcnt vmcnt(%0)\n\ts_barrier" :: "n"(PIECES) : "memory");
             if (!(BYA_GEMM6_ABLATE & 2)) {
-                ALL4(DMA_A, fillA, dA, (BYA_GEMM6_ABLATE & 16) ? 0u : soff);
+                ALL_A(fillA, dA, (BYA_GEMM6_ABLATE & 16) ? 0u : soff);
                 ALL8(DMA_W, fillW, dW, (BYA_GEMM6_ABLATE & 16) ? 0u : soff);
             }
             const uint32_t d = st == 2 ? (uint32_t)(-2 * STAGE) : (uint32_t)STAGE;
@@ -70,6 +75,7 @@
             rsA = rsAn;
             rsW = rsWn;
         }
+#undef ALL_A
 #undef DMA_A
 #undef DMA_W
         asm volatile("s_waitcnt vmcnt(0)" ::: "memory");
@@ -78,15 +84,15 @@
 
     const int wm = wave >> 1, wn = wave & 1;
     const int fr = lane & 15, fq = lane >> 4;
-    const int a_row = wm * 64 + fr, w_row = wn * 128 + fr;
+    const int a_row = wm * (16 * NJ) + fr, w_row = wn * 128 + fr;
     const uint32_t bA0 = frag_addr(lds0, a_row, fq), bA1 = frag_addr(lds0, a_row, 4 + fq);
     const uint32_t bW0 = frag_addr(lds0 + TILE_A, w_row, fq);
     const uint32_t bW1 = frag_addr(lds0 + TILE_A, w_row, 4 + fq);
     uint32_t off1 = 0u, off0 = (uint32_t)STAGE;
     uint32_t rA1 = bA1, rW1 = bW1, rA0 = bA0 + STAGE, rW0 = bW0 + STAGE;
 
-    f32x4 acc[8][4];
-    bf16x8 fa[2][4], fw[2][8];
+    f32x4 acc[8][NJ];
+    bf16x8 fa[2][NJ], fw[2][8];
     asm volatile("s_barrier" ::: "memory");
 
 #define RA(S, J) ds_read128<(J) * 2048>(fa[S][J], (S) ? rA1 : rA0)
@@ -95,7 +101,8 @@
         const PersistentTile nxt = walk.coord(seq + 1);
         {
             const uint32_t tA = bA0 + off1, tW = bW0 + off1;
-            ds_read128<0 * 2048>(fa[0][0], tA); ds_read128<1 * 2048>(fa[0][1], tA); ds_read128<2 * 2048>(fa[0][2], tA); ds_read128<3 * 2048>(fa[0][3], tA);
+            ds_read128<0 * 2048>(fa[0][0], tA); ds_read128<1 * 2048>(fa[0][1], tA); ds_read128<2 * 2048>(fa[0][2], tA);
+            if constexpr (NJ > 3) ds_read128<3 * 2048>(fa[0][NJ - 1], tA);
             ds_read128<0 * 2048>(fw[0][0], tW); ds_read128<1 * 2048>(fw[0][1], tW); ds_read128<2 * 2048>(fw[0][2], tW); ds_read128<3 * 2048>(fw[0][3], tW);
             ds_read128<4 * 2048>(fw[0][4], tW); ds_read128<5 * 2048>(fw[0][5], tW); ds_read128<6 * 2048>(fw[0][6], tW); ds_read128<7 * 2048>(fw[0][7], tW);
             asm volatile("s_waitcnt lgkmcnt(0)" ::: "memory");
@@ -113,6 +120,7 @@
                 off0 = off0 == (uint32_t)(2 * STAGE) ? 0u : off0 + (uint32_t)STAGE; \
                 rA1 = bA1 + off1; rW1 = bW1 + off1; rA0 = bA0 + off0; rW0 = bW0 + off0; \
             } while (0)
+        if constexpr (NJ == 4) {
         if constexpr (V == 'A') {
             MFZ(0, 0, 0);  RA(1, 0);
             MFZ(0, 0, 1);  RA(1, 1);
@@ -309,7 +317,158 @@
             MF(1, 7, 2);
             MF(1, 7, 3);  NEXT();
         }
-            KEEP4(fa[0]); KEEP8(fw[0]); KEEP4(fa[1]); KEEP8(fw[1]);
+        } else if constexpr (NJ == 3) {
+        if constexpr (V == 'A') {
+            MFZ(0, 0, 0);  RA(1, 0);
+            MFZ(0, 0, 1);  RA(1, 1);
+            MFZ(0, 0, 2);  RA(1, 2);
+            MFZ(0, 1, 0);  RW(1, 0);
+            MFZ(0, 1, 1);
+            MFZ(0, 1, 2);  RW(1, 1);
+            MFZ(0, 2, 0);
+            MFZ(0, 2, 1);  RW(1, 2);
+            MFZ(0, 2, 2);
+            MFZ(0, 3, 0);  RW(1, 3);
+            MFZ(0, 3, 1);
+            MFZ(0, 3, 2);  RW(1, 4);
+            MFZ(0, 4, 0);
+            MFZ(0, 4, 1);  RW(1, 5);
+            MFZ(0, 4, 2);
+            MFZ(0, 5, 0);  RW(1, 6);
+            MFZ(0, 5, 1);
+            MFZ(0, 5, 2);  RW(1, 7);
+            MFZ(0, 6, 0);
+            MFZ(0, 6, 1);
+            MFZ(0, 6, 2);  SYNC();
+            MFZ(0, 7, 0);
+            MFZ(0, 7, 1);  RW(0, 0);
+            MFZ(0, 7, 2);
+            MF(1, 0, 0);  RW(0, 1);
+            MF(1, 0, 1);
+            MF(1, 0, 2);  RW(0, 2);
+            MF(1, 1, 0);
+            MF(1, 1, 1);  RW(0, 3);
+            MF(1, 1, 2);
+            MF(1, 2, 0);  RW(0, 4);
+            MF(1, 2, 1);
+            MF(1, 2, 2);  RA(0, 0);
+            MF(1, 3, 0);
+            MF(1, 3, 1);  RA(0, 1);
+            MF(1, 3, 2);
+            MF(1, 4, 0);  RA(0, 2);
+            MF(1, 4, 1);
+            MF(1, 4, 2);  RW(0, 5);
+            MF(1, 5, 0);
+            MF(1, 5, 1);  RW(0, 6);
+            MF(1, 5, 2);
+            MF(1, 6, 0);  RW(0, 7);
+            MF(1, 6, 1);
+            MF(1, 6, 2);
+            MF(1, 7, 0);
+            MF(1, 7, 1);
+            MF(1, 7, 2);  NEXT();
+        } else if constexpr (V == 'B') {
+            MF(0, 0, 0);  RA(1, 0);
+            MF(0, 0, 1);  RA(1, 1);
+            MF(0, 0, 2);  RA(1, 2);
+            MF(0, 1, 0);  RW(1, 0);
+            MF(0, 1, 1);
+            MF(0, 1, 2);  RW(1, 1);
+            MF(0, 2, 0);
+            MF(0, 2, 1);  RW(1, 2);
+            MF(0, 2, 2);
+            MF(0, 3, 0);  RW(1, 3);
+            MF(0, 3, 1);
+            MF(0, 3, 2);  RW(1, 4);
+            MF(0, 4, 0);
+            MF(0, 4, 1);  RW(1, 5);
+            MF(0, 4, 2);
+            MF(0, 5, 0);  RW(1, 6);
+            MF(0, 5, 1);
+            MF(0, 5, 2);  RW(1, 7);
+            MF(0, 6, 0);
+            MF(0, 6, 1);
+            MF(0, 6, 2);  SYNC();
+            MF(0, 7, 0);
+            MF(0, 7, 1);  RW(0, 0);
+            MF(0, 7, 2);
+            MF(1, 0, 0);  RW(0, 1);
+            MF(1, 0, 1);
+            MF(1, 0, 2);  RW(0, 2);
+            MF(1, 1, 0);
+            MF(1, 1, 1);  RW(0, 3);
+            MF(1, 1, 2);
+            MF(1, 2, 0);  RW(0, 4);
+            MF(1, 2, 1);
+            MF(1, 2, 2);  RA(0, 0);
+            MF(1, 3, 0);
+            MF(1, 3, 1);  RA(0, 1);
+            MF(1, 3, 2);
+            MF(1, 4, 0);  RA(0, 2);
+            MF(1, 4, 1);
+            MF(1, 4, 2);  RW(0, 5);
+            MF(1, 5, 0);
+            MF(1, 5, 1);  RW(0, 6);
+            MF(1, 5, 2);
+            MF(1, 6, 0);  RW(0, 7);
+            MF(1, 6, 1);
+            MF(1, 6, 2);
+            MF(1, 7, 0);
+            MF(1, 7, 1);
+            MF(1, 7, 2);  NEXT();
+        } else if constexpr (V == 'L') {
+            MF(0, 0, 0);  RA(1, 0);
+            MF(0, 0, 1);  RA(1, 1);
+            MF(0, 0, 2);  RA(1, 2);
+            MF(0, 1, 0);  RW(1, 0);
+            MF(0, 1, 1);
+            MF(0, 1, 2);  RW(1, 1);
+            MF(0, 2, 0);
+            MF(0, 2, 1);  RW(1, 2);
+            MF(0, 2, 2);
+            MF(0, 3, 0);  RW(1, 3);
+            MF(0, 3, 1);
+            MF(0, 3, 2);  RW(1, 4);
+            MF(0, 4, 0);
+            MF(0, 4, 1);  RW(1, 5);
+            MF(0, 4, 2);
+            MF(0, 5, 0);  RW(1, 6);
+            MF(0, 5, 1);
+            MF(0, 5, 2);  RW(1, 7);
+            MF(0, 6, 0);
+            MF(0, 6, 1);
+            MF(0, 6, 2);  SYNC();
+            MF(0, 7, 0);
+            MF(0, 7, 1);
+            MF(0, 7, 2);
+            MF(1, 0, 0);
+            MF(1, 0, 1);
+            MF(1, 0, 2);
+            MF(1, 1, 0);
+            MF(1, 1, 1);
+            MF(1, 1, 2);
+            MF(1, 2, 0);
+            MF(1, 2, 1);
+            MF(1, 2, 2);
+            MF(1, 3, 0);
+            MF(1, 3, 1);
+            MF(1, 3, 2);
+            MF(1, 4, 0);
+            MF(1, 4, 1);
+            MF(1, 4, 2);
+            MF(1, 5, 0);
+            MF(1, 5, 1);
+            MF(1, 5, 2);
+            MF(1, 6, 0);
+            MF(1, 6, 1);
+            MF(1, 6, 2);
+            MF(1, 7, 0);
+            MF(1, 7, 1);
+            MF(1, 7, 2);  NEXT();
+        }
+        }
+            if constexpr (NJ > 3) { KEEP4(fa[0]); KEEP8(fw[0]); KEEP4(fa[1]); KEEP8(fw[1]); }
+            else { KEEP3(fa[0]); KEEP8(fw[0]); KEEP3(fa[1]); KEEP8(fw[1]); }
 #undef MF
 #undef MFZ
 #undef SYNC
@@ -322,10 +481,10 @@
 
         if constexpr (BYA_GEMM6_ABLATE & 1) {
 #pragma unroll
-            for (int i = 0; i < 8; ++i) asm volatile("" :: "a"(acc[i][0]), "a"(acc[i][1]), "a"(acc[i][2]), "a"(acc[i][3]));
+            for (int i = 0; i < 8; ++i) asm volatile("" :: "a"(acc[i][0]), "a"(acc[i][1]), "a"(acc[i][2]), "a"(acc[i][NJ - 1]));
         } else {
             auto run = [&](auto act_tag) {
-                epilogue_wide<decltype(act_tag)::value, 1, false, false, 4>(p, cur.z, cur.m0 + wm * 64, cur.n0 + wn * 128, fr, fq, acc, wave, lane);
+                epilogue_wide<decltype(act_tag)::value, 1, false, false, NJ>(p, cur.z, cur.m0 + wm * (16 * NJ), cur.n0 + wn * 128, fr, fq, acc, wave, lane);
             };
             dispatch_act_big(p.act, run);
         }
@@ -338,16 +497,27 @@
 #undef RW
 }
 
+__global__ __launch_bounds__(512, 1) void gemm128s_kernel(GemmArgs p, int tiles_m, int tiles_n, int batch) {
+    gemm_s_body<4>(p, tiles_m, tiles_n, batch);
 }
-
-int bya_launch_gemm128s(const void* args, int batch, hipStream_t s) {
+__global__ __launch_bounds__(512, 1) void gemm96s_kernel(GemmArgs p, int tiles_m, int tiles_n, int batch) {
+    gemm_s_body<3>(p, tiles_m, tiles_n, batch);
+}
+
+template <int BM, auto KERNEL>
+int launch_s(const void* args, int batch, hipStream_t s) {
     GemmArgs a = *static_cast<const GemmArgs*>(args);
 #ifdef BYA_GEMM6_GM
     a.gm = BYA_GEMM6_GM;
 #else
-    a.gm = 2 * gemm_group_m(a);
+    a.gm = 256 * gemm_group_m(a) / BM;
 #endif
-    const int tiles_m = (a.M + 127) / 128, tiles_n = (a.N + 255) / 256;
-    const size_t lds = 3 * (128 + 256) * BK * 2;
-    return launch_persistent<gemm128s_kernel>(persistent_grid((long long)tiles_m * tiles_n * batch), 512, lds, s, a, tiles_m, tiles_n, batch);
+    const int tiles_m = (a.M + BM - 1) / BM, tiles_n = (a.N + 255) / 256;
+    const size_t lds = 3 * (BM + 256) * BK * 2;
+    return launch_persistent<KERNEL>(persistent_grid((long long)tiles_m * tiles_n * batch), 512, lds, s, a, tiles_m, tiles_n, batch);
 }
+
+}
+
+int bya_launch_gemm128s(const void* args, int batch, hipStream_t s) { return launch_s<128, gemm128s_kernel>(args, batch, s); }
+int bya_launch_gemm96s(const void* args, int batch, hipStream_t s) { return launch_s<96, gemm96s_kernel>(args, batch, s); }
diff --git a/bind_your_avatar_implementation_amd/csrc/misc.hip b/bind_your_avatar_implementation_amd/csrc/misc.hip
--- a/bind_your_avatar_implementation_amd/csrc/misc.hip
+++ b/bind_your_avatar_implementation_amd/csrc/misc.hip
@@ -320,7 +320,7 @@
 
 extern "C" int bya_set_option(int32_t key, int32_t value) {
     static const int32_t lo[BYA_OPT_COUNT] = {0, 0, -1, 0, 0, 0, 0, 0, 0};
-    static const int32_t hi[BYA_OPT_COUNT] = {2, 1 << 20, 6, 2, 1, 1, 1024, 31, 2};
+    static const int32_t hi[BYA_OPT_COUNT] = {2, 1 << 20, 6, 4, 1, 1, 1024, 31, 2};
     if (key < 0 || key >= BYA_OPT_COUNT || value < lo[key] || value > hi[key]) return BYA_ERR_SHAPE;
     if (key == BYA_OPT_P2P_GROUPS && value != 0 && value < 16) return BYA_ERR_SHAPE;
     g_bya_options[key].store(value, std::memory_order_relaxed);
diff --git a/bind_your_avatar_implementation_amd/engine.py b/bind_your_avatar_implementation_amd/engine.py
--- a/bind_your_avatar_implementation_amd/engine.py
+++ b/bind_your_avatar_implementation_amd/engine.py
@@ -76,6 +76,7 @@
         self.side_stream_conditioning = os.environ.get("BYA_INVARIANTS_SIDE_STREAM", "1") != "0"
         self.sp_allgather = os.environ.get("BYA_SP_ALLGATHER", "0") == "1"
         self.router_fused_attn = os.environ.get("BYA_ROUTER_FUSED_ATTN", "1") != "0"
+        self.gemm_tail_tile = os.environ.get("BYA_GEMM_TAIL_TILE", "1") != "0"
         self.router_chain = os.environ.get("BYA_ROUTER_CHAIN", "1")
         self.verify_exchanges = os.environ.get("BYA_SP_VERIFY", "0") == "1"
         self.sp_overlap_v = os.environ.get("BYA_SP_OVERLAP_V", "1") != "0"
@@ -520,7 +521,8 @@
     @torch.no_grad()
     def step(self, *args, **kwargs):
         self.refresh_if_stale()
-        with ops.pinned_stream():
+        tail = self.gemm_tail_tile and ops.get_option("gemm_variant") == 0
+        with ops.pinned_stream(), (ops.options(gemm_variant=3) if tail else contextlib.nullcontext()):
             return self._step(*args, **kwargs)
 
     def _step(self, hidden_states, encoder_hidden_states, timestep, image_rotary_emb, id_cond, id_vit_hidden,
diff --git a/bind_your_avatar_implementation_amd/ops.py b/bind_your_avatar_implementation_amd/ops.py
--- a/bind_your_avatar_implementation_amd/ops.py
+++ b/bind_your_avatar_implementation_amd/ops.py
@@ -382,11 +382,16 @@
     if a.is_cuda and a.device.index not in _GEMM_WS:
         ensure_gemm_workspace(a.device)
     if _takes_skinny(d, gate0, bias_rowscale, split):
-        return {"path": "skinny", "m0": 0, "tail": None, "split_k": 0, "row_chunks": 1}
+        return {"path": "skinny", "m0": 0, "tail": None, "split_k": 0, "row_chunks": 1, "loader_rows": 0}
     p, q = _hip.GemmPlan(), _plan_p
     check(lib.bya_gemm_bf16_plan(q(a), q(w), q(bias), q(out), q(res), q(gate0), q(gate1), ctypes.byref(d),
                                  ctypes.byref(p)), "bya_gemm_bf16_plan")
-    return _plan_dict(p)
+    plan = _plan_dict(p)
+    rows = _hip._i32(0)
+    check(lib.bya_gemm_bf16_loader_rows(q(a), q(w), q(bias), q(out), q(res), q(gate0), q(gate1), ctypes.byref(d),
+                                        ctypes.byref(rows)), "bya_gemm_bf16_loader_rows")
+    plan["loader_rows"] = rows.value
+    return plan
 
 
 def _qkn_descs(a, w, out, split, qw, qb, kw, kb, cos, sin, text_rows, eps, k_scale, tensors, plan=False):
diff --git a/include/bya.h b/include/bya.h
--- a/include/bya.h
+++ b/include/bya.h
@@ -95,6 +95,8 @@
 } bya_gemm_plan;
 int bya_gemm_bf16_plan(const void* A, const void* W, const void* bias, const void* C, const void* res,
                        const void* gate0, const void* gate1, const bya_gemm_desc* desc, bya_gemm_plan* plan);
+int bya_gemm_bf16_loader_rows(const void* A, const void* W, const void* bias, const void* C, const void* res,
+                              const void* gate0, const void* gate1, const bya_gemm_desc* desc, int32_t* rows);
 int bya_gemm_qkv_norm_rope_plan(const void* A, const void* W, const void* bias, const void* C, const bya_gemm_desc* desc,
                                 const bya_qknorm_desc* norm, bya_gemm_plan* plan);
 
```

Result: no change. 2.882 steps/s (median of 2 runs) (+0.0%).
